# AshutoshNirkhe/KubernetesClusterCapacity

Measured on AMD Instinct MI355X. Metric: node×spec fit evals/sec at 1M nodes × 4K specs; % of HBM roofline, higher is better.
Workload: dtype int64; 1 GPU; C4: 1000000 nodes x 20000000 pods x 4096 specs; reduce + fit prepare + fit + finalize; nodes=1000000, pods=20000000, containers_rank0=39602467, nodes_rank0=1000000, pods_rank0=19801877, pods_per_node=poisson, mean 20, specs=4096, parallelism=node-sharded x1

## Files before the change

### include/kcc.h

```cpp
#ifndef KCC_H
#define KCC_H

#include <stdint.h>

#ifdef __cplusplus
extern "C" {
#endif

#define KCC_ABI_VERSION 2

enum {
  KCC_OK = 0,
  KCC_EINVAL = -1,
  KCC_ENOMEM = -2,
  KCC_EHIP = -3,
  KCC_ENODEV = -4,
  KCC_ERCCL = -5,
  KCC_EFAULT = -6
};

enum {
  KCC_SPEC_OK = 0,
  KCC_SPEC_DIVZERO = 1,
  KCC_SPEC_FAULT = 2
// ... 56 lines not shown
int kcc_fit_run_async(kcc_ctx* ctx, int64_t n_nodes, int64_t n_specs, int64_t* d_partial,
                      void* stream);

int kcc_fit_async(kcc_ctx* ctx, int64_t n_nodes, const uint64_t* d_alloc_cpu,
                  const int64_t* d_alloc_mem, const int64_t* d_alloc_pods,
                  const int64_t* d_pod_count, const uint64_t* d_used_cpu,
                  const int64_t* d_used_mem, int64_t n_specs, const uint64_t* d_spec_cpu,
                  const int64_t* d_spec_mem, int64_t* d_totals, int32_t* d_spec_err,
                  void* stream);

int kcc_capacity_partial_async(kcc_ctx* ctx, int64_t n_nodes, int64_t n_containers,
                               const int64_t* h_node_ptr, const int64_t* d_node_ptr,
                               const uint64_t* d_cpu_req, const int64_t* d_mem_req,
                               const uint64_t* d_alloc_cpu, const int64_t* d_alloc_mem,
                               const int64_t* d_alloc_pods, const int64_t* d_pod_count,
                               uint64_t* d_used_cpu, int64_t* d_used_mem, int64_t n_specs,
                               const uint64_t* d_spec_cpu, const int64_t* d_spec_mem,
                               int64_t* d_partial, int n_chunks, void* stream);
int kcc_capacity_async(kcc_ctx* ctx, int64_t n_nodes, int64_t n_containers,
                       const int64_t* h_node_ptr, const int64_t* d_node_ptr,
                       const uint64_t* d_cpu_req, const int64_t* d_mem_req,
                       const uint64_t* d_alloc_cpu, const int64_t* d_alloc_mem,
                       const int64_t* d_alloc_pods, const int64_t* d_pod_count,
                       uint64_t* d_used_cpu, int64_t* d_used_mem, int64_t n_specs,
                       const uint64_t* d_spec_cpu, const int64_t* d_spec_mem, int64_t* d_totals,
                       int32_t* d_spec_err, void* stream);

#define KCC_COMM_ID_BYTES 128
int kcc_set_node_shards(kcc_ctx* ctx, int n_shards);
int kcc_comm_unique_id(uint8_t* id );
int kcc_comm_init(kcc_ctx* ctx, const uint8_t* id, int n_ranks, int rank);
int kcc_allreduce_partial_async(kcc_ctx* ctx, int64_t n_specs, int64_t* d_partial, void* stream);

#define KCC_P2P_HANDLE_BYTES 64
#define KCC_P2P_MAX_SPECS (1 << 20)
int kcc_p2p_export(kcc_ctx* ctx, int n_ranks, int64_t max_specs,
                   uint8_t* handle );
int kcc_p2p_open(kcc_ctx* ctx, int rank, const uint8_t* handles );
int kcc_exchange_finalize_async(kcc_ctx* ctx, int64_t n_specs, const int64_t* d_partial,
                                int64_t* d_totals, int32_t* d_spec_err, void* stream);
int kcc_p2p_faults(kcc_ctx* ctx, int64_t* faults);

int kcc_profile_enable(kcc_ctx* ctx, int on);
int kcc_profile_read(kcc_ctx* ctx, double* reduce_ms, int64_t* reduce_launches, double* fit_ms,
                     int64_t* fit_launches);

int kcc_reduce_faults(kcc_ctx* ctx, int64_t* faults);
int kcc_clear_faults(kcc_ctx* ctx);

int kcc_set_fit_dense(kcc_ctx* ctx, int dense);
int kcc_set_clamp_in_fit(kcc_ctx* ctx, int mode);
int kcc_clamp_in_fit_used(kcc_ctx* ctx, int* used);
int kcc_fit_stream_rows(kcc_ctx* ctx, int64_t* streamed);

double kcc_last_slow_fraction(const kcc_ctx* ctx);

int kcc_fit_slow_pairs(kcc_ctx* ctx, int64_t* slow_pairs, int64_t* pairs);

enum {
  KCC_PARSE_OK = 1,
  KCC_PARSE_ERR = 0,
  KCC_PARSE_UNSUPPORTED = -1,
  KCC_PARSE_BADOFF = -2
};
int kcc_parse_cpu_millis(kcc_ctx* ctx, int64_t n, const char* bytes, int64_t n_bytes,
                         const int64_t* offsets, uint64_t* out, int8_t* status);
int kcc_parse_bytes(kcc_ctx* ctx, int64_t n, const char* bytes, int64_t n_bytes,
                    const int64_t* offsets, int64_t* out, int8_t* status);
int kcc_parse_quantity(kcc_ctx* ctx, int64_t n, const char* bytes, int64_t n_bytes,
                       const int64_t* offsets, int64_t* out, int8_t* status);
int kcc_parse_quantity_async(kcc_ctx* ctx, int64_t n, const char* d_bytes, int64_t n_bytes,
                             const int64_t* d_offsets, int64_t* d_out, int8_t* d_status,
                             void* stream);
int kcc_parse_cpu_millis_async(kcc_ctx* ctx, int64_t n, const char* d_bytes, int64_t n_bytes,
                               const int64_t* d_offsets, uint64_t* d_out, int8_t* d_status,
                               void* stream);
int kcc_parse_bytes_async(kcc_ctx* ctx, int64_t n, const char* d_bytes, int64_t n_bytes,
                          const int64_t* d_offsets, int64_t* d_out, int8_t* d_status,
                          void* stream);

int kcc_reduce_requests_keyed(kcc_ctx* ctx, int64_t n_keys, int64_t n_containers,
                              const int32_t* key, const uint64_t* cpu_req, const int64_t* mem_req,
                              const uint64_t* cpu_lim, const int64_t* mem_lim,
                              uint64_t* used_cpu, int64_t* used_mem, uint64_t* lim_cpu,
                              int64_t* lim_mem);
int kcc_reduce_requests_keyed_async(kcc_ctx* ctx, int64_t n_keys, int64_t n_containers,
                                    const int32_t* d_key, const uint64_t* d_cpu_req,
                                    const int64_t* d_mem_req, const uint64_t* d_cpu_lim,
                                    const int64_t* d_mem_lim, uint64_t* d_used_cpu,
                                    int64_t* d_used_mem, uint64_t* d_lim_cpu, int64_t* d_lim_mem,
                                    void* stream);
int kcc_count_by_key(kcc_ctx* ctx, int64_t n_keys, int64_t n, const int32_t* key, int64_t* count);
int kcc_count_by_key_async(kcc_ctx* ctx, int64_t n_keys, int64_t n, const int32_t* d_key,
                           int64_t* d_count, void* stream);

int kcc_fit_rows(kcc_ctx* ctx, int64_t n_nodes, const uint64_t* alloc_cpu,
                 const int64_t* alloc_mem, const int64_t* alloc_pods, const int64_t* pod_count,
                 const uint64_t* used_cpu, const int64_t* used_mem, uint64_t spec_cpu,
                 int64_t spec_mem, int64_t* q, int32_t* row_err);

int kcc_fit_grouped(kcc_ctx* ctx, int64_t n_nodes, const uint64_t* alloc_cpu,
                    const int64_t* alloc_mem, const int64_t* alloc_pods, const int64_t* pod_count,
                    const uint64_t* used_cpu, const int64_t* used_mem, const int32_t* group,
                    int64_t n_groups, int64_t n_specs, const uint64_t* spec_cpu,
                    const int64_t* spec_mem, int64_t* totals ,
                    int32_t* spec_err );
// ... 49 lines not shown
```

### kubernetesclustercapacity_amd/_lib.py

```python
from __future__ import annotations

import ctypes as C
import os
import re

_HERE = os.path.dirname(os.path.abspath(__file__))
LIB_PATH = os.path.join(_HERE, "libkcc.so")
HEADER_PATH = os.path.join(os.path.dirname(_HERE), "include", "kcc.h")

KCC_OK = 0
KCC_EINVAL = -1
KCC_ENOMEM = -2
KCC_EHIP = -3
KCC_ENODEV = -4
KCC_ERCCL = -5
KCC_EFAULT = -6
ERROR_NAMES = {
    KCC_EINVAL: "KCC_EINVAL", KCC_ENOMEM: "KCC_ENOMEM", KCC_EHIP: "KCC_EHIP",
    KCC_ENODEV: "KCC_ENODEV", KCC_ERCCL: "KCC_ERCCL", KCC_EFAULT: "KCC_EFAULT",
}
KCC_SPEC_OK = 0
KCC_SPEC_DIVZERO = 1
KCC_SPEC_FAULT = 2
KCC_EXT_MAX = 4

_i64, _i32, _int, _vp, _dbl = C.c_int64, C.c_int32, C.c_int, C.c_void_p, C.c_double

SIGNATURES = {
    "kcc_abi_version": (_int, []),
    "kcc_set_allreduce_verify": (_int, [_vp, _int]),
    "kcc_build_info": (C.c_char_p, []),
    "kcc_create": (_int, [C.POINTER(_vp), _int, _int]),
    "kcc_destroy": (None, [_vp]),
    "kcc_last_error": (C.c_char_p, [_vp]),
    "kcc_create_error": (C.c_char_p, []),
    "kcc_reserve": (_int, [_vp, _i64, _i64, _i64]),
    "kcc_reduce_requests": (_int, [_vp, _i64, _i64] + [_vp] * 9),
    "kcc_reduce_requests_async": (_int, [_vp, _i64, _i64] + [_vp] * 10),
    "kcc_fit": (_int, [_vp, _i64] + [_vp] * 6 + [_i64] + [_vp] * 4),
    "kcc_capacity": (_int, [_vp, _i64, _i64] + [_vp] * 7 + [_i64] + [_vp] * 4),
    "kcc_fit_partial_async": (_int, [_vp, _i64] + [_vp] * 6 + [_i64] + [_vp] * 4),
    "kcc_fit_prepare_async": (_int, [_vp, _i64] + [_vp] * 6 + [_i64] + [_vp] * 4),
    "kcc_fit_run_async": (_int, [_vp, _i64, _i64, _vp, _vp]),
    "kcc_fit_finalize_async": (_int, [_vp, _i64, _vp, _vp, _vp, _vp]),
    "kcc_fit_async": (_int, [_vp, _i64] + [_vp] * 6 + [_i64] + [_vp] * 5),
    "kcc_capacity_partial_async": (_int, [_vp, _i64, _i64] + [_vp] * 10 + [_i64] + [_vp] * 3
                                   + [_int, _vp]),
    "kcc_capacity_async": (_int, [_vp, _i64, _i64] + [_vp] * 10 + [_i64] + [_vp] * 5),
    "kcc_set_node_shards": (_int, [_vp, _int]),
    "kcc_set_fit_dense": (_int, [_vp, _int]),
    "kcc_set_clamp_in_fit": (_int, [_vp, _int]),
    "kcc_clamp_in_fit_used": (_int, [_vp, C.POINTER(C.c_int)]),
    "kcc_fit_stream_rows": (_int, [_vp, C.POINTER(_i64)]),
    "kcc_reduce_faults": (_int, [_vp, C.POINTER(_i64)]),
    "kcc_clear_faults": (_int, [_vp]),
    "kcc_comm_unique_id": (_int, [_vp]),
    "kcc_comm_init": (_int, [_vp, _vp, _int, _int]),
    "kcc_allreduce_partial_async": (_int, [_vp, _i64, _vp, _vp]),
    "kcc_p2p_export": (_int, [_vp, _int, _i64, _vp]),
    "kcc_p2p_open": (_int, [_vp, _int, _vp]),
    "kcc_exchange_finalize_async": (_int, [_vp, _i64, _vp, _vp, _vp, _vp]),
    "kcc_p2p_faults": (_int, [_vp, C.POINTER(_i64)]),
    "kcc_profile_enable": (_int, [_vp, _int]),
    "kcc_profile_read": (_int, [_vp] + [C.POINTER(_dbl), C.POINTER(_i64)] * 2),
    "kcc_last_slow_fraction": (_dbl, [_vp]),
    "kcc_fit_slow_pairs": (_int, [_vp, C.POINTER(_i64), C.POINTER(_i64)]),
    "kcc_parse_cpu_millis": (_int, [_vp, _i64, _vp, _i64, _vp, _vp, _vp]),
    "kcc_parse_bytes": (_int, [_vp, _i64, _vp, _i64, _vp, _vp, _vp]),
    "kcc_parse_quantity": (_int, [_vp, _i64, _vp, _i64, _vp, _vp, _vp]),
    "kcc_parse_quantity_async": (_int, [_vp, _i64, _vp, _i64, _vp, _vp, _vp, _vp]),
    "kcc_parse_cpu_millis_async": (_int, [_vp, _i64, _vp, _i64, _vp, _vp, _vp, _vp]),
    "kcc_parse_bytes_async": (_int, [_vp, _i64, _vp, _i64, _vp, _vp, _vp, _vp]),
    "kcc_reduce_requests_keyed": (_int, [_vp, _i64, _i64] + [_vp] * 9),
    "kcc_reduce_requests_keyed_async": (_int, [_vp, _i64, _i64] + [_vp] * 10),
    "kcc_count_by_key": (_int, [_vp, _i64, _i64, _vp, _vp]),
    "kcc_count_by_key_async": (_int, [_vp, _i64, _i64, _vp, _vp, _vp]),
    "kcc_fit_rows": (_int, [_vp, _i64] + [_vp] * 6 + [C.c_uint64, _i64, _vp, _vp]),
    "kcc_fit_grouped": (_int, [_vp, _i64] + [_vp] * 7 + [_i64, _i64] + [_vp] * 4),
    "kcc_fit_grouped_async": (_int, [_vp, _i64] + [_vp] * 7 + [_i64, _i64] + [_vp] * 5),
    "kcc_fit_ext": (_int, [_vp, _i64] + [_vp] * 6 + [_i64] + [_vp] * 3 + [_i64, _i64] + [_vp] * 5),
    "kcc_fit_ext_async": (_int, [_vp, _i64] + [_vp] * 6 + [_i64] + [_vp] * 3 + [_i64, _i64]
                          + [_vp] * 6),
    "kcc_pod_requests": (_int, [_vp, _i64, _i64, _i64] + [_vp] * 11),
    "kcc_pod_requests_async": (_int, [_vp, _i64, _i64, _i64] + [_vp] * 12),
    "kcc_reduce_requests_pods": (_int, [_vp, _i64, _i64, _i64, _i64] + [_vp] * 12),
}

KCC_PARSE_OK = 1
KCC_PARSE_ERR = 0
KCC_PARSE_UNSUPPORTED = -1
KCC_PARSE_BADOFF = -2


def header_symbols(path: str = HEADER_PATH) -> list[str]:
    text = open(path).read()
    text = re.sub(r"/\*.*?\*/", "", text, flags=re.S)
    return sorted(set(re.findall(r"\b(kcc_[a-z0-9_]+)\s*\(", text)))


def header_arities(path: str = HEADER_PATH) -> dict[str, int]:
    text = re.sub(r"/\*.*?\*/", "", open(path).read(), flags=re.S)
    out = {}
    for m in re.finditer(r"\b(kcc_[a-z0-9_]+)\s*\(([^;{]*?)\)\s*;", text, flags=re.S):
        params = m.group(2).strip()
        out[m.group(1)] = 0 if params in ("", "void") else params.count(",") + 1
    return out


def load(path: str = LIB_PATH) -> C.CDLL:
    if not os.path.exists(path):
        raise ImportError(
            f"libkcc.so not found at {path}: build it with "
            "`make -C kubernetesclustercapacity_amd/csrc` (or __graft_entry__.build()). "
            "There is no CPU fallback.")
    lib = C.CDLL(path)
    for name, (res, args) in SIGNATURES.items():
        fn = getattr(lib, name)
        fn.restype = res
        fn.argtypes = args
    return lib


_LIBS: dict[str, C.CDLL] = {}


def lib(path: str | None = None) -> C.CDLL:
    p = os.path.abspath(path or LIB_PATH)
    if p not in _LIBS:
        _LIBS[p] = load(p)
    return _LIBS[p]
```

### kubernetesclustercapacity_amd/csrc/kcc_abi.cpp

```cpp
#include "kcc.h"

#include <hip/hip_runtime.h>
#include <rccl/rccl.h>

#include <cstdio>
#include <cstdlib>
#include <cstring>
#include <string>
#include <vector>

#include "kcc_internal.h"

namespace {

struct DevBuf {
  void* p = nullptr;
  size_t bytes = 0;
};

hipError_t ensure(DevBuf& b, size_t bytes) {
  if (bytes == 0) bytes = 16;
  if (b.bytes >= bytes) return hipSuccess;
  if (b.p) (void)hipFree(b.p);
  b.p = nullptr;
  b.bytes = 0;
  hipError_t e = hipMalloc(&b.p, bytes);
  if (e == hipSuccess) b.bytes = bytes;
  return e;
}

hipError_t ensure_uncached(DevBuf& b, size_t bytes) {
  if (bytes == 0) bytes = 16;
  if (b.bytes >= bytes) return hipSuccess;
  if (b.p) (void)hipFree(b.p);
  b.p = nullptr;
  b.bytes = 0;
  hipError_t e = hipExtMallocWithFlags(&b.p, bytes, hipDeviceMallocUncached);
  if (e == hipSuccess) b.bytes = bytes;
  return e;
}

template <class T>
T* as(DevBuf& b) {
  return static_cast<T*>(b.p);
}

struct ProfPair {
  hipEvent_t a, b;
  int kind;
};

struct Dev {
  int device = 0;
  hipStream_t stream = nullptr;
  hipStream_t side = nullptr;
  hipEvent_t ev_fork = nullptr;
  hipEvent_t ev_red[kcc::FIT_MAX_CHUNKS] = {};
  bool prof_on = false;
  std::vector<ProfPair> prof_pending;
  std::vector<hipEvent_t> prof_free;
  double prof_ms[2] = {0.0, 0.0};
  int64_t prof_n[2] = {0, 0};
  DevBuf fast_a, fast_b, slow, slow_list, srec, sperm, counters;
  DevBuf red_tail;
  DevBuf faults;
  DevBuf rank_arrive;
  DevBuf fit_q;
  bool fitq_dirty = true;
  DevBuf c_rank, c_bcnt, c_cs, c_ms, c_mrc, c_crm, c_dperm;
  DevBuf c_C, c_H2, c_H3, c_Crow, c_rec, c_dir;
  bool clamp_dirty = true;
  int64_t last_pairs = 0;
  int64_t c_stride = 0;
  int64_t h_stride = 0;
  int64_t d_stride = 0;
  bool fit_dense = false;
  int clamp_in_fit = -1;
  bool last_nc = false;
  DevBuf fast_cl;
  int stream_chunks = 0;
  int64_t prep_nodes = -1, prep_specs = -1;
  DevBuf ptr, cpu, mem, cpul, meml, used_cpu, used_mem, lim_cpu, lim_mem;
  DevBuf alloc_cpu, alloc_mem, alloc_pods, pod_count, spec_cpu, spec_mem, partial, totals, err;
  DevBuf p_bytes, p_off, p_out, p_st;
  DevBuf k_key;
  DevBuf g_group;
  DevBuf g_count, g_cursor, g_total, g_rec, g_rg, g_acc;
  DevBuf x_alloc, x_used, x_spec;
  DevBuf x_rec;
  DevBuf kb_counts, kb_tot, kb_sr, kb_sv;
  DevBuf kb_part, kb_arrive;
  DevBuf kb_esc_n, kb_esc_row, kb_esc_cpu, kb_esc_mem;
  DevBuf q_ptr, q_iptr, q_icpu, q_imem, q_rst, q_ocpu, q_omem, q_pcpu, q_pmem;
  DevBuf p2p_mbox, p2p_arrive;
  DevBuf clamp_arrive;
  DevBuf np_sync;
  unsigned char* p2p_peer[kcc::P2P_MAX_RANKS] = {};
  int p2p_W = 0, p2p_rank = -1;
  int64_t p2p_smax = 0;
  bool p2p_ready = false;
};

}

struct kcc_ctx {
  std::vector<Dev> devs;
  std::vector<ncclComm_t> comms;
  ncclComm_t proc_comm = nullptr;
  int proc_ranks = 0, proc_rank = 0;
  int node_shards = 0;
  std::string err;
  double slow_frac = -1.0;
  unsigned long long* host_cnt = nullptr;
  size_t host_cnt_n = 0;
  int64_t host_stream_rows = -1;
  bool allreduce_verified = false;
  bool allreduce_verify_every = false;
};

namespace {

thread_local std::string g_create_error;

int fail(kcc_ctx* ctx, int code, const std::string& msg) {
  if (ctx) ctx->err = msg;
  return code;
}

#define KCC_HIP(ctx, expr)                                                              \
  do {                                                                                  \
// ... 71 lines not shown
    KCC_HIP(ctx, hipSetDevice(dv.device));
    KCC_HIP(ctx, hipMemcpy(f, dv.faults.p, sizeof(f), hipMemcpyDeviceToHost));
    red += f[kcc::FAULT_RED];
    p2p += f[kcc::FAULT_P2P];
  }
  if (red == 0 && p2p == 0) return KCC_OK;
  return fail(ctx, KCC_EFAULT,
              "device fault: " + std::to_string(red) + " reduce-side wait(s) (look-back, node prep, keyed gather) and " +
                  std::to_string(p2p) +
                  " exchange flag wait(s) gave up; results are not valid (every spec is marked "
                  "KCC_SPEC_FAULT) until kcc_clear_faults");
}

int reduce_async_dev(kcc_ctx* ctx, Dev& dv, int64_t n_nodes, int64_t n_cont, const int64_t* ptr,
                     const uint64_t* cpu, const int64_t* mem, const uint64_t* cpul,
                     const int64_t* meml, uint64_t* used_cpu, int64_t* used_mem,
                     uint64_t* lim_cpu, int64_t* lim_mem, hipStream_t s) {
  if (n_nodes < 0 || n_cont < 0) return fail(ctx, KCC_EINVAL, "negative size");
  if (n_nodes == 0) return n_cont == 0 ? KCC_OK : fail(ctx, KCC_EINVAL, "containers without nodes");
  if (n_nodes >= kcc::RED_MAX_NODES)
    return fail(ctx, KCC_EINVAL, "too many nodes per device (max 2^28 - 1)");
  if (!ptr || !used_cpu || !used_mem) return fail(ctx, KCC_EINVAL, "NULL node_ptr/output");
  if (n_cont > 0 && (!cpu || !mem)) return fail(ctx, KCC_EINVAL, "NULL cpu_req/mem_req");
  const bool lim = cpul != nullptr || meml != nullptr;
  if (lim && (!cpul || !meml || !lim_cpu || !lim_mem))
    return fail(ctx, KCC_EINVAL, "limits need cpu_lim, mem_lim, lim_cpu and lim_mem");
  if (!aligned16(cpu) || !aligned16(mem) || (lim && (!aligned16(cpul) || !aligned16(meml))))
    return fail(ctx, KCC_EINVAL, "container arrays must be 16-byte aligned");
  int rc = reduce_ws(ctx, dv, s);
  if (rc) return rc;
  KCC_HIP(ctx, kcc::launch_reduce(n_nodes, 0, n_cont, ptr, cpu, mem, lim ? cpul : nullptr,
                                  lim ? meml : nullptr, used_cpu, used_mem, lim ? lim_cpu : nullptr,
                                  lim ? lim_mem : nullptr, as<uint64_t>(dv.red_tail),
                                  as<unsigned long long>(dv.faults), s));
  return KCC_OK;
}

kcc::SpecPrep spec_prep_of(Dev& dv) {
  kcc::SpecPrep sp;
  sp.rec = as<kcc::SpecRec>(dv.srec);
  sp.perm = as<int32_t>(dv.sperm);
  return sp;
}

int reserve_dev(kcc_ctx* ctx, Dev& dv, int64_t n_nodes, int64_t n_cont, int64_t n_specs) {
  KCC_HIP(ctx, hipSetDevice(dv.device));
  const size_t N = (size_t)(n_nodes > 0 ? n_nodes : 1);
  const size_t S = (size_t)(n_specs > 0 ? n_specs : 1);
  (void)n_cont;
  {
    int rc = reduce_ws(ctx, dv, dv.stream);
    if (rc) return rc;
  }
  KCC_HIP(ctx, ensure(dv.fast_a, sizeof(kcc::FitGroupA) * (size_t)kcc::fit_groups((int64_t)N)));
  KCC_HIP(ctx, ensure(dv.fast_b, sizeof(kcc::FitGroup) * (size_t)kcc::fit_groups((int64_t)N)));
  KCC_HIP(ctx, ensure(dv.fast_cl, sizeof(int32_t) * kcc::FIT_GROUP * (size_t)kcc::fit_groups((int64_t)N)));
  KCC_HIP(ctx, ensure(dv.slow, sizeof(kcc::SlowNode) * N));
  KCC_HIP(ctx, ensure(dv.slow_list, sizeof(int64_t) * N));
  KCC_HIP(ctx, ensure(dv.srec, sizeof(kcc::SpecRec) * S));
  KCC_HIP(ctx, ensure(dv.sperm, 4 * S));
  KCC_HIP(ctx, ensure(dv.counters, sizeof(unsigned long long) * kcc::CNT_N));
  if (!dv.np_sync.p) {
    const size_t bytes = 4 * (kcc::NP_FLAGS + (size_t)kcc::reduce_tail_records());
    KCC_HIP(ctx, ensure(dv.np_sync, bytes));
    KCC_HIP(ctx, hipMemsetAsync(dv.np_sync.p, 0, bytes, dv.stream));
    KCC_HIP(ctx, hipStreamSynchronize(dv.stream));
  }
  if (!dv.clamp_arrive.p) {
    KCC_HIP(ctx, ensure(dv.clamp_arrive, 64));
    KCC_HIP(ctx, hipMemsetAsync(dv.clamp_arrive.p, 0, 64, dv.stream));
    KCC_HIP(ctx, hipStreamSynchronize(dv.stream));
  }
  const size_t q_before = dv.fit_q.bytes;
  KCC_HIP(ctx, ensure(dv.fit_q, 4 * (size_t)kcc::fit_queue_words((int64_t)S)));
  if (dv.fit_q.bytes != q_before) dv.fitq_dirty = true;
  const size_t S64 = (S + 63) / 64 * 64;
  KCC_HIP(ctx, ensure(dv.c_bcnt, 8 * (S64 / 64)));
  KCC_HIP(ctx, ensure(dv.c_cs, 8 * S));
  KCC_HIP(ctx, ensure(dv.c_ms, 8 * S));
  KCC_HIP(ctx, ensure(dv.c_mrc, 4 * S64));
  KCC_HIP(ctx, ensure(dv.c_crm, 4 * S64));
  KCC_HIP(ctx, ensure(dv.c_dperm, 4 * S));
  const int64_t cs_ = kcc::clamp_c_cells((int64_t)S), hs = kcc::clamp_h_cells((int64_t)S);
  const size_t before[3] = {dv.c_C.bytes, dv.c_H2.bytes, dv.c_H3.bytes};
  KCC_HIP(ctx, ensure(dv.c_rank, 4 * (size_t)kcc::rank_words((int64_t)S)));
  if (dv.rank_arrive.bytes < 4 * (S64 / 64)) {
    KCC_HIP(ctx, ensure(dv.rank_arrive, 4 * (S64 / 64)));
    KCC_HIP(ctx, hipMemsetAsync(dv.rank_arrive.p, 0, dv.rank_arrive.bytes, dv.stream));
    KCC_HIP(ctx, hipStreamSynchronize(dv.stream));
  }
  KCC_HIP(ctx, ensure(dv.c_C, 8 * (size_t)kcc::C_COPIES * (size_t)cs_));
  KCC_HIP(ctx, ensure(dv.c_H2, 8 * (size_t)kcc::H2_COPIES * (size_t)hs));
  KCC_HIP(ctx, ensure(dv.c_H3, 8 * (size_t)kcc::H2_COPIES * (size_t)hs));
  KCC_HIP(ctx, ensure(dv.c_Crow, 8 * (size_t)cs_));
  if (kcc::clamp_binned((int64_t)S)) {
    const size_t passes = (size_t)((N + kcc::CLAMP_PASS_ROWS_MIN - 1) / kcc::CLAMP_PASS_ROWS_MIN);
    const size_t recs = (size_t)((N + kcc::CLAMP_PASS_ROWS_MAX - 1) / kcc::CLAMP_PASS_ROWS_MAX) *
                        2 * kcc::CLAMP_PASS_ROWS_MAX;
    KCC_HIP(ctx, ensure(dv.c_rec, 8 * recs));
    KCC_HIP(ctx, ensure(dv.c_dir, 4 * (size_t)kcc::clamp_d_stride((int64_t)S) * passes));
  }
  if (dv.c_C.bytes != before[0] || dv.c_H2.bytes != before[1] || dv.c_H3.bytes != before[2] ||
      dv.c_stride != cs_ || dv.h_stride != hs)
    dv.clamp_dirty = true;
  dv.c_stride = cs_;
  dv.h_stride = hs;
  dv.d_stride = kcc::clamp_d_stride((int64_t)S);
  return KCC_OK;
}

int clamp_clean(kcc_ctx* ctx, Dev& dv, hipStream_t s) {
  if (dv.fitq_dirty) {
    KCC_HIP(ctx, hipMemsetAsync(dv.fit_q.p, 0, dv.fit_q.bytes, s));
    dv.fitq_dirty = false;
  }
  if (!dv.clamp_dirty) return KCC_OK;
  KCC_HIP(ctx, hipMemsetAsync(dv.c_C.p, 0, dv.c_C.bytes, s));
  KCC_HIP(ctx, hipMemsetAsync(dv.c_H2.p, 0, dv.c_H2.bytes, s));
  KCC_HIP(ctx, hipMemsetAsync(dv.c_H3.p, 0, dv.c_H3.bytes, s));
  dv.clamp_dirty = false;
  return KCC_OK;
}

kcc::ClampWork clamp_of(Dev& dv) {
  kcc::ClampWork cw;
  cw.rank = as<uint32_t>(dv.c_rank);
  cw.bcnt = as<uint32_t>(dv.c_bcnt);
  cw.cs = as<uint64_t>(dv.c_cs);
  cw.ms = as<int64_t>(dv.c_ms);
  cw.mr_c = as<uint32_t>(dv.c_mrc);
  cw.cr_m = as<uint32_t>(dv.c_crm);
  cw.dperm = as<int32_t>(dv.c_dperm);
  cw.C = as<int64_t>(dv.c_C);
  cw.H2 = as<int64_t>(dv.c_H2);
  cw.H3 = as<int64_t>(dv.c_H3);
  cw.Crow = as<int64_t>(dv.c_Crow);
  cw.rec = as<uint64_t>(dv.c_rec);
  cw.dir = as<uint32_t>(dv.c_dir);
  cw.c_stride = dv.c_stride;
  cw.h_stride = dv.h_stride;
  cw.d_stride = dv.d_stride;
  cw.n_pass = 0;
  return cw;
}

int check_spec_ws(kcc_ctx* ctx, Dev& dv, int64_t S) {
  const size_t S64 = (size_t)(S + 63) / 64 * 64;
  const bool ok = dv.c_rank.bytes >= 4 * (size_t)kcc::rank_words(S) &&
                  dv.c_bcnt.bytes >= 8 * (S64 / 64) && dv.c_mrc.bytes >= 4 * S64 &&
                  dv.rank_arrive.bytes >= 4 * (S64 / 64) &&
                  dv.c_crm.bytes >= 4 * S64 && dv.c_cs.bytes >= 8 * (size_t)S &&
                  dv.c_ms.bytes >= 8 * (size_t)S && dv.c_dperm.bytes >= 4 * (size_t)S &&
                  dv.srec.bytes >= sizeof(kcc::SpecRec) * (size_t)S &&
                  dv.sperm.bytes >= 4 * (size_t)S &&
                  dv.counters.bytes >= sizeof(unsigned long long) * kcc::CNT_N &&
                  dv.c_C.bytes >= 8 * (size_t)kcc::C_COPIES * (size_t)dv.c_stride &&
                  dv.c_stride >= kcc::clamp_c_cells(S);
  return ok ? KCC_OK : fail(ctx, KCC_EINVAL, "internal: spec workspace smaller than the call");
}

kcc::PlaceArgs place_args(Dev& dv, int64_t n_specs, const uint64_t* spec_cpu,
                          const int64_t* spec_mem, int64_t* partial) {
  return kcc::PlaceArgs{n_specs, spec_cpu, spec_mem, spec_prep_of(dv), clamp_of(dv), partial,
                        as<unsigned long long>(dv.counters), 0,
                        as<const unsigned long long>(dv.faults), 0};
}

int fit_prepare_dev(kcc_ctx* ctx, Dev& dv, int64_t n_nodes, const uint64_t* alloc_cpu,
                    const int64_t* alloc_mem, const int64_t* alloc_pods,
                    const int64_t* pod_count, const uint64_t* used_cpu,
                    const int64_t* used_mem, int64_t n_specs, const uint64_t* spec_cpu,
                    const int64_t* spec_mem, int64_t* partial, hipStream_t s) {
  ctx->host_stream_rows = -1;
  if (n_nodes < 0 || n_specs < 0) return fail(ctx, KCC_EINVAL, "negative size");
  if (n_specs >= kcc::MAX_SPECS) return fail(ctx, KCC_EINVAL, "too many specs (max 2^26 - 1)");
  if (n_specs > 0 && (!spec_cpu || !spec_mem || !partial))
    return fail(ctx, KCC_EINVAL, "NULL spec array / partial");
  if (n_nodes > 0 && (!alloc_cpu || !alloc_mem || !alloc_pods || !pod_count || !used_cpu || !used_mem))
    return fail(ctx, KCC_EINVAL, "NULL node array");
  int rc = reserve_dev(ctx, dv, n_nodes, 0, n_specs);
  if (rc) return rc;
  dv.last_pairs = n_nodes * n_specs;
  dv.prep_nodes = n_nodes;
  dv.prep_specs = n_specs;
  if (n_specs == 0) return KCC_OK;
  if ((rc = check_spec_ws(ctx, dv, n_specs))) return rc;
  rc = clamp_clean(ctx, dv, s);
  if (rc) return rc;
  dv.clamp_dirty = true;
  KCC_HIP(ctx, kcc::launch_spec_rank(kcc::rank_args(n_specs, spec_cpu, spec_mem, clamp_of(dv),
                                                    as<unsigned long long>(dv.counters),
                                                    as<uint32_t>(dv.rank_arrive)),
                                     s));
  const kcc::PlaceArgs pa = place_args(dv, n_specs, spec_cpu, spec_mem, partial);
  KCC_HIP(ctx, kcc::launch_node_prep(n_nodes, alloc_cpu, alloc_mem, alloc_pods, pod_count,
                                       used_cpu, used_mem, as<kcc::FitGroupA>(dv.fast_a),
                                       as<kcc::FitGroup>(dv.fast_b), as<kcc::SlowNode>(dv.slow),
                                       as<int64_t>(dv.slow_list), n_specs, clamp_of(dv),
                                       as<unsigned long long>(dv.counters), 0, 0,
                                       n_nodes, s, dv.fit_dense, &pa));
  if (n_nodes == 0) {
    dv.clamp_dirty = false;
    return KCC_OK;
  }
  dv.stream_chunks = 1;
  KCC_HIP(ctx, kcc::launch_clamp_apply(n_specs, n_nodes, clamp_of(dv),
                                       as<unsigned long long>(dv.counters), partial, s));
  dv.clamp_dirty = false;
  return KCC_OK;
}

int fit_run_dev(kcc_ctx* ctx, Dev& dv, int64_t n_nodes, int64_t n_specs, int64_t* partial,
                hipStream_t s) {
  if (n_nodes != dv.prep_nodes || n_specs != dv.prep_specs)
    return fail(ctx, KCC_EINVAL, "fit_run sizes differ from the preceding fit_prepare");
  if (n_nodes == 0 || n_specs == 0) return KCC_OK;
  if (!partial) return fail(ctx, KCC_EINVAL, "NULL partial");
  KCC_HIP(ctx, kcc::launch_fit(n_nodes, as<kcc::FitGroupA>(dv.fast_a), as<kcc::FitGroup>(dv.fast_b),
                               as<kcc::SlowNode>(dv.slow),
                               as<int64_t>(dv.slow_list), n_specs, spec_prep_of(dv), partial,
                               as<unsigned long long>(dv.counters), as<uint32_t>(dv.fit_q), 0,
                               n_nodes, s, as<const unsigned long long>(dv.faults)));
  return KCC_OK;
}

int fit_partial_dev(kcc_ctx* ctx, Dev& dv, int64_t n_nodes, const uint64_t* alloc_cpu,
                    const int64_t* alloc_mem, const int64_t* alloc_pods,
                    const int64_t* pod_count, const uint64_t* used_cpu,
                    const int64_t* used_mem, int64_t n_specs, const uint64_t* spec_cpu,
                    const int64_t* spec_mem, int64_t* partial, hipStream_t s) {
  int rc = fit_prepare_dev(ctx, dv, n_nodes, alloc_cpu, alloc_mem, alloc_pods, pod_count,
                           used_cpu, used_mem, n_specs, spec_cpu, spec_mem, partial, s);
  if (rc) return rc;
  return fit_run_dev(ctx, dv, n_nodes, n_specs, partial, s);
}

int fit_finalize_dev(kcc_ctx* ctx, Dev& dv, int64_t n_specs, const int64_t* partial,
                     int64_t* totals, int32_t* spec_err, hipStream_t s) {
  if (n_specs < 0) return fail(ctx, KCC_EINVAL, "negative size");
  if (n_specs == 0) return KCC_OK;
  if (!partial || !totals || !spec_err) return fail(ctx, KCC_EINVAL, "NULL partial/totals/err");
  if (dv.sperm.bytes < sizeof(int32_t) * (size_t)n_specs)
    return fail(ctx, KCC_EINVAL, "finalize without a matching fit_partial");
  KCC_HIP(ctx, kcc::launch_fit_finalize(n_specs, partial, as<int32_t>(dv.sperm), totals,
                                        spec_err, as<const unsigned long long>(dv.faults), s));
  return KCC_OK;
}



hipError_t prof_event(Dev& dv, hipEvent_t* ev) {
  if (!dv.prof_free.empty()) {
    *ev = dv.prof_free.back();
    dv.prof_free.pop_back();
    return hipSuccess;
  }
  return hipEventCreateWithFlags(ev, hipEventDisableSystemFence);
}

constexpr int64_t CHUNK_ALIGN = kcc::CLAMP_PASS_ROWS_MAX;
int plan_chunks(int64_t n_nodes, int want, int64_t min_nodes, std::vector<int64_t>& lo,
                std::vector<int64_t>& hi) {
  int k = want;
  if (k > kcc::FIT_MAX_CHUNKS) k = kcc::FIT_MAX_CHUNKS;
  while (k > 1 && n_nodes / k < min_nodes) --k;
  if (k < 1) k = 1;
  lo.assign(k, 0);
  hi.assign(k, 0);
  for (int c = 0; c < k; ++c) {
    lo[c] = c == 0 ? 0 : hi[c - 1];
    hi[c] = c == k - 1 ? n_nodes : (n_nodes * (c + 1) / k) / CHUNK_ALIGN * CHUNK_ALIGN;
    if (hi[c] < lo[c]) hi[c] = lo[c];
  }
  return k;
}
// ... 8 lines not shown
                         int64_t* used_mem, int64_t n_specs, const uint64_t* spec_cpu,
                         const int64_t* spec_mem, int64_t* partial, int n_chunks, hipStream_t s,
                         int64_t* totals = nullptr, int32_t* spec_err = nullptr) {
  ctx->host_stream_rows = -1;
  if (n_nodes < 0 || n_cont < 0 || n_specs < 0) return fail(ctx, KCC_EINVAL, "negative size");
  if (n_nodes >= kcc::RED_MAX_NODES)
    return fail(ctx, KCC_EINVAL, "too many nodes per device (max 2^28 - 1)");
  if (n_specs >= kcc::MAX_SPECS) return fail(ctx, KCC_EINVAL, "too many specs (max 2^26 - 1)");
  if (n_nodes == 0 && n_cont != 0) return fail(ctx, KCC_EINVAL, "containers without nodes");
  if (n_nodes > 0 && (!ptr || !used_cpu || !used_mem || !alloc_cpu || !alloc_mem || !alloc_pods ||
                      !pod_count))
    return fail(ctx, KCC_EINVAL, "NULL node array");
  if (n_cont > 0 && (!cpu || !mem)) return fail(ctx, KCC_EINVAL, "NULL cpu_req/mem_req");
  if (!aligned16(cpu) || !aligned16(mem))
    return fail(ctx, KCC_EINVAL, "container arrays must be 16-byte aligned");
  if (n_specs > 0 && (!spec_cpu || !spec_mem || !partial))
    return fail(ctx, KCC_EINVAL, "NULL spec array / partial");
  std::vector<int64_t> lo, hi;
  const int k = plan_chunks(n_nodes, h_ptr ? (n_chunks > 0 ? n_chunks : KCC_DEFAULT_CHUNKS) : 1,
                            KCC_MIN_CHUNK_NODES, lo, hi);
  std::vector<int64_t> c0(k), c1(k);
  for (int c = 0; c < k; ++c) {
    if (k == 1) {
      c0[c] = 0;
      c1[c] = n_cont;
    } else {
      c0[c] = h_ptr[lo[c]];
      c1[c] = h_ptr[hi[c]];
      if (c0[c] < 0 || c1[c] < c0[c] || c1[c] > n_cont)
        return fail(ctx, KCC_EINVAL, "h_node_ptr is not a CSR of n_containers");
    }
  }
  int rc = reserve_dev(ctx, dv, n_nodes, n_cont, n_specs);
  if (rc) return rc;
  if (n_specs > 0 && (rc = check_spec_ws(ctx, dv, n_specs))) return rc;
  for (int c = 0; c < k; ++c)
    if (!dv.ev_red[c]) KCC_HIP(ctx, hipEventCreateWithFlags(&dv.ev_red[c], hipEventDisableTiming));
  dv.last_pairs = n_nodes * n_specs;
  dv.stream_chunks = k;
  dv.prep_nodes = -1;
  dv.prep_specs = -1;
  hipStream_t rs = k > 1 ? dv.side : s;
  if (k > 1) {
    KCC_HIP(ctx, hipEventRecord(dv.ev_fork, s));
    KCC_HIP(ctx, hipStreamWaitEvent(dv.side, dv.ev_fork, 0));
  }
  const bool fuse_place = n_specs > 0;
  const bool fuse_rank = k == 1 && fuse_place && n_nodes > 0 && n_cont > 0;
  const bool nc = fuse_rank && n_specs <= kcc::CLAMP_LDS_SPECS && !dv.fit_dense &&
                  (dv.clamp_in_fit == 1 ||
                   (dv.clamp_in_fit < 0 && kcc::clamp_in_fit_auto(n_nodes, n_specs)));
  int32_t* const fast_cl = nc ? as<int32_t>(dv.fast_cl) : nullptr;
  dv.last_nc = nc;
  kcc::RankArgs ra = kcc::rank_args(n_specs, spec_cpu, spec_mem, clamp_of(dv),
                                    as<unsigned long long>(dv.counters),
                                    as<uint32_t>(dv.rank_arrive), nc);
  kcc::PlaceArgs pa = place_args(dv, n_specs, spec_cpu, spec_mem, partial);
  pa.no_ranks = nc ? 1 : 0;
  kcc::NpArgs np{};
  if (nc) {
    ra.done_flag = as<uint32_t>(dv.np_sync);
    np.n_place = (int32_t)((n_specs + 255) / 256);
    np.n_rows = (int32_t)((n_nodes + kcc::NP_ROWS_PER_WG - 1) / kcc::NP_ROWS_PER_WG);
    np.sync = as<uint32_t>(dv.np_sync);
    np.pa = pa;
    np.n = n_nodes;
    np.alloc_cpu = alloc_cpu;
    np.alloc_mem = alloc_mem;
    np.alloc_pods = alloc_pods;
    np.pod_count = pod_count;
    np.used_cpu = used_cpu;
    np.used_mem = used_mem;
    np.fast_a = as<kcc::FitGroupA>(dv.fast_a);
    np.fast_b = as<kcc::FitGroup>(dv.fast_b);
    np.slow = as<kcc::SlowNode>(dv.slow);
    np.slow_list = as<int64_t>(dv.slow_list);
    np.fast_cl = fast_cl;
    np.counters = as<unsigned long long>(dv.counters);
    np.bcnt = clamp_of(dv).bcnt;
    np.S = n_specs;
    np.faults = as<unsigned long long>(dv.faults);
  }
  if (n_specs > 0) {
    rc = clamp_clean(ctx, dv, s);
    if (rc) return rc;
    dv.clamp_dirty = true;
    if (!fuse_rank) KCC_HIP(ctx, kcc::launch_spec_rank(ra, s));
  }
  for (int c = 0; c < k; ++c) {
    const int64_t n = hi[c] - lo[c];
    ProfPair pp{};
    if (dv.prof_on) {
      KCC_HIP(ctx, prof_event(dv, &pp.a));
      KCC_HIP(ctx, prof_event(dv, &pp.b));
    }
    KCC_HIP(ctx, kcc::launch_reduce(n, c0[c], c1[c] - c0[c], ptr + lo[c], cpu, mem, nullptr, nullptr,
                                    used_cpu + lo[c], used_mem + lo[c], nullptr, nullptr,
                                    as<uint64_t>(dv.red_tail),
                                    as<unsigned long long>(dv.faults), rs,
                                    fuse_rank ? &ra : nullptr, nc ? &np : nullptr,
                                    dv.prof_on ? pp.a : nullptr, dv.prof_on ? pp.b : nullptr));
    if (dv.prof_on) {
      pp.kind = 0;
      dv.prof_pending.push_back(pp);
    }
    if (k > 1) KCC_HIP(ctx, hipEventRecord(dv.ev_red[c], dv.side));
  }
  const bool fuse_fin = totals && n_nodes > 0;
  const kcc::FinArgs fin{as<int32_t>(dv.sperm), totals, spec_err, as<uint32_t>(dv.clamp_arrive),
                         as<const unsigned long long>(dv.faults)};
  for (int c = 0; c < k; ++c) {
    if (k > 1) KCC_HIP(ctx, hipStreamWaitEvent(s, dv.ev_red[c], 0));
    const int64_t n = hi[c] - lo[c];
    const bool place_here = fuse_place && c == 0;
    if (n_specs == 0 || (n == 0 && !place_here)) continue;
    if (!nc)
    KCC_HIP(ctx, kcc::launch_node_prep(n, alloc_cpu + lo[c], alloc_mem + lo[c], alloc_pods + lo[c],
                                       pod_count + lo[c], used_cpu + lo[c], used_mem + lo[c],
                                       as<kcc::FitGroupA>(dv.fast_a) + lo[c] / kcc::FIT_GROUP,
                                       as<kcc::FitGroup>(dv.fast_b) + lo[c] / kcc::FIT_GROUP,
                                       as<kcc::SlowNode>(dv.slow) + lo[c],
                                       as<int64_t>(dv.slow_list) + lo[c], n_specs, clamp_of(dv),
                                       as<unsigned long long>(dv.counters),
                                       c, lo[c], n_nodes, s, dv.fit_dense,
                                       place_here ? &pa : nullptr));
    if (n == 0) continue;
    ProfPair pp{};
    if (dv.prof_on) {
      KCC_HIP(ctx, prof_event(dv, &pp.a));
      KCC_HIP(ctx, prof_event(dv, &pp.b));
    }
    KCC_HIP(ctx, kcc::launch_fit(n, as<kcc::FitGroupA>(dv.fast_a) + lo[c] / kcc::FIT_GROUP,
                                 as<kcc::FitGroup>(dv.fast_b) + lo[c] / kcc::FIT_GROUP,
                                 as<kcc::SlowNode>(dv.slow) + lo[c],
                                 as<int64_t>(dv.slow_list) + lo[c], n_specs, spec_prep_of(dv),
                                 partial, as<unsigned long long>(dv.counters),
                                 as<uint32_t>(dv.fit_q), c, n_nodes, s,
                                 as<const unsigned long long>(dv.faults), fast_cl,
                                 dv.prof_on ? pp.a : nullptr, dv.prof_on ? pp.b : nullptr));
    if (dv.prof_on) {
      pp.kind = 1;
      dv.prof_pending.push_back(pp);
    }
  }
  if (n_specs > 0 && nc) {
    dv.clamp_dirty = false;
    if (totals) return fit_finalize_dev(ctx, dv, n_specs, partial, totals, spec_err, s);
    return KCC_OK;
  }
  if (n_specs > 0) {
    if (n_nodes > 0)
      KCC_HIP(ctx, kcc::launch_clamp_apply(n_specs, n_nodes, clamp_of(dv),
                                           as<unsigned long long>(dv.counters), partial, s,
                                           fuse_fin ? &fin : nullptr));
    dv.clamp_dirty = false;
    if (totals && !fuse_fin)
      return fit_finalize_dev(ctx, dv, n_specs, partial, totals, spec_err, s);
  }
  return KCC_OK;
}

int run_host(kcc_ctx* ctx, bool with_reduce, int64_t n_nodes, int64_t n_cont,
             const int64_t* node_ptr, const uint64_t* cpu_req, const int64_t* mem_req,
             const uint64_t* alloc_cpu, const int64_t* alloc_mem, const int64_t* alloc_pods,
             const int64_t* pod_count, const uint64_t* used_cpu_in, const int64_t* used_mem_in,
             int64_t n_specs, const uint64_t* spec_cpu, const int64_t* spec_mem,
             int64_t* totals, int32_t* spec_err) {
  if (n_nodes < 0 || n_specs < 0) return fail(ctx, KCC_EINVAL, "negative size");
  if (n_specs > 0 && (!spec_cpu || !spec_mem || !totals || !spec_err))
    return fail(ctx, KCC_EINVAL, "NULL spec array / output");
  if (n_nodes > 0 && (!alloc_cpu || !alloc_mem || !alloc_pods || !pod_count))
    return fail(ctx, KCC_EINVAL, "NULL node array");
  if (with_reduce) {
    int rc = check_csr(ctx, n_nodes, n_cont, node_ptr);
    if (rc) return rc;
    if (n_cont > 0 && (!cpu_req || !mem_req)) return fail(ctx, KCC_EINVAL, "NULL container array");
  } else if (n_nodes > 0 && (!used_cpu_in || !used_mem_in)) {
    return fail(ctx, KCC_EINVAL, "NULL used array");
  }
  if (n_specs == 0) return KCC_OK;
  const int nd = (int)ctx->devs.size();
  const int ns = ctx->node_shards > nd ? ctx->node_shards : nd;
  const int slots = (ns + nd - 1) / nd;
  std::vector<int64_t> lo, hi;
  shard_nodes(n_nodes, ns, lo, hi);
  std::vector<std::vector<int64_t>> rebased(ns);
  if (ctx->host_cnt_n < (size_t)ns * kcc::CNT_N) {
    if (ctx->host_cnt) (void)hipHostFree(ctx->host_cnt);
    ctx->host_cnt = nullptr;
    ctx->host_cnt_n = 0;
    KCC_HIP(ctx, hipHostMalloc(reinterpret_cast<void**>(&ctx->host_cnt),
                               sizeof(unsigned long long) * (size_t)ns * kcc::CNT_N, hipHostMallocDefault));
// ... 66 lines not shown
    }
    KCC_NCCL(ctx, ncclGroupStart());
    for (int d = 0; d < nd; ++d) {
      Dev& dv = ctx->devs[d];
      KCC_NCCL(ctx, ncclAllReduce(dv.partial.p, dv.partial.p, words, ncclInt64,
                                  ncclSum, ctx->comms[d], dv.stream));
    }
    KCC_NCCL(ctx, ncclGroupEnd());
#ifdef KCC_DIAG_INLIB_COMM
    if (std::getenv("KCC_DRILL_CORRUPT_ALLREDUCE")) {
      Dev& dv = ctx->devs[nd - 1];
      KCC_HIP(ctx, hipSetDevice(dv.device));
      KCC_HIP(ctx, hipMemsetAsync(dv.partial.p, 0x5a, 8, dv.stream));
    }
#endif
    if (verify) {
      for (int d = 0; d < nd; ++d) {
        Dev& dv = ctx->devs[d];
        KCC_HIP(ctx, hipSetDevice(dv.device));
        KCC_HIP(ctx, hipMemcpyAsync(got.data(), dv.partial.p, 8 * words, hipMemcpyDeviceToHost,
                                    dv.stream));
        KCC_HIP(ctx, hipStreamSynchronize(dv.stream));
        for (size_t i = 0; i < words; ++i)
          if (got[i] != expect[i])
            return fail(ctx, KCC_ERCCL,
                        "in-library all-reduce verification failed on device " +
                            std::to_string(dv.device) + ": word " + std::to_string(i) + " is " +
                            std::to_string(got[i]) + ", the host sum of the devices' partials " +
                            std::to_string(expect[i]) + "; results not returned");
      }
      ctx->allreduce_verified = true;
    }
  }
  Dev& d0 = ctx->devs[0];
  KCC_HIP(ctx, hipSetDevice(d0.device));
  KCC_HIP(ctx, ensure(d0.totals, 8 * (size_t)n_specs));
  KCC_HIP(ctx, ensure(d0.err, 4 * (size_t)n_specs));
  int rc = fit_finalize_dev(ctx, d0, n_specs, as<int64_t>(d0.partial), as<int64_t>(d0.totals),
                            as<int32_t>(d0.err), d0.stream);
  if (rc) return rc;
  KCC_HIP(ctx, hipMemcpyAsync(totals, d0.totals.p, 8 * (size_t)n_specs, hipMemcpyDeviceToHost,
                              d0.stream));
  KCC_HIP(ctx, hipMemcpyAsync(spec_err, d0.err.p, 4 * (size_t)n_specs, hipMemcpyDeviceToHost,
                              d0.stream));
  unsigned long long slow_pairs = 0;
  for (int d = 0; d < nd; ++d) {
    Dev& dv = ctx->devs[d];
    KCC_HIP(ctx, hipSetDevice(dv.device));
    KCC_HIP(ctx, hipStreamSynchronize(dv.stream));
  }
  int64_t streamed = 0;
  for (int sh = 0; sh < ns; ++sh) {
    slow_pairs += ctx->host_cnt[(size_t)sh * kcc::CNT_N + kcc::CNT_SLOW_PAIRS];
    streamed += (int64_t)ctx->host_cnt[(size_t)sh * kcc::CNT_N + kcc::CNT_STREAM];
  }
  ctx->host_stream_rows = streamed;
  const double pairs = (double)n_nodes * (double)n_specs;
  ctx->slow_frac = pairs > 0 ? (double)slow_pairs / pairs : 0.0;
  return check_faults(ctx);
}

}

extern "C" {

int kcc_abi_version(void) { return KCC_ABI_VERSION; }

int kcc_set_allreduce_verify(kcc_ctx* ctx, int every_call) {
  if (!ctx) return KCC_EINVAL;
  ctx->allreduce_verify_every = every_call != 0;
  return KCC_OK;
}

#ifdef KCC_VARIANT_BUILD
const char* kcc_build_info(void) { return "variant: " KCC_VARIANT_FLAGS; }
#else
const char* kcc_build_info(void) { return "release"; }
#endif

const char* kcc_create_error(void) { return g_create_error.c_str(); }

int kcc_create(kcc_ctx** out, int first_device, int n_gpus) {
  g_create_error.clear();
  if (!out) { g_create_error = "out is NULL"; return KCC_EINVAL; }
  *out = nullptr;
  if (n_gpus <= 0 || first_device < 0) {
    g_create_error = "n_gpus must be >= 1 and first_device >= 0 (there is no CPU backend)";
    return KCC_EINVAL;
  }
  int count = 0;
  hipError_t e = hipGetDeviceCount(&count);
  if (e != hipSuccess || count <= 0) {
    g_create_error = std::string("no HIP device: ") + hipGetErrorString(e);
    return KCC_ENODEV;
  }
  if (first_device + n_gpus > count) {
    g_create_error = "requested devices [" + std::to_string(first_device) + ", " +
                     std::to_string(first_device + n_gpus) + ") but only " +
                     std::to_string(count) + " visible";
    return KCC_ENODEV;
  }
  kcc_ctx* ctx = new kcc_ctx();
  ctx->devs.resize(n_gpus);
  std::vector<int> ids(n_gpus);
  for (int d = 0; d < n_gpus; ++d) {
    Dev& dv = ctx->devs[d];
    dv.device = first_device + d;
// ... 7 lines not shown
                       "): libkcc is built for MI355X only";
      kcc_destroy(ctx);
      return KCC_ENODEV;
    }
    if ((e = hipSetDevice(dv.device)) != hipSuccess ||
        (e = hipStreamCreateWithFlags(&dv.stream, hipStreamNonBlocking)) != hipSuccess ||
        (e = hipStreamCreateWithFlags(&dv.side, hipStreamNonBlocking)) != hipSuccess ||
        (e = hipEventCreateWithFlags(&dv.ev_fork, hipEventDisableTiming)) != hipSuccess) {
      g_create_error = std::string("stream creation failed: ") + hipGetErrorString(e);
      kcc_destroy(ctx);
      return KCC_EHIP;
    }
  }
#ifdef KCC_DIAG_INLIB_COMM
  const bool inlib_comm = true;
#else
  const bool inlib_comm = n_gpus > 1;
#endif
  if (inlib_comm) {
    ctx->comms.resize(n_gpus);
    ncclResult_t r = ncclCommInitAll(ctx->comms.data(), n_gpus, ids.data());
    if (r != ncclSuccess) {
      ctx->comms.clear();
      g_create_error = std::string("ncclCommInitAll: ") + ncclGetErrorString(r);
      kcc_destroy(ctx);
      return KCC_ERCCL;
    }
  }
  *out = ctx;
  return KCC_OK;
}

void kcc_destroy(kcc_ctx* ctx) {
  if (!ctx) return;
  for (auto& c : ctx->comms) ncclCommDestroy(c);
  if (ctx->proc_comm) {
    (void)hipSetDevice(ctx->devs[0].device);
    (void)hipDeviceSynchronize();
    ncclCommDestroy(ctx->proc_comm);
  }
  for (Dev& dv : ctx->devs) {
    (void)hipSetDevice(dv.device);
    if (dv.stream) (void)hipStreamSynchronize(dv.stream);
    if (dv.p2p_W > 0) {
      (void)hipDeviceSynchronize();
      for (int p = 0; p < dv.p2p_W; ++p)
        if (p != dv.p2p_rank && dv.p2p_peer[p]) (void)hipIpcCloseMemHandle(dv.p2p_peer[p]);
      DevBuf* pb[] = {&dv.p2p_mbox, &dv.p2p_arrive};
      for (DevBuf* b : pb)
        if (b->p) (void)hipFree(b->p);
    }
    if (dv.clamp_arrive.p) (void)hipFree(dv.clamp_arrive.p);
    if (dv.np_sync.p) (void)hipFree(dv.np_sync.p);
    DevBuf* bufs[] = {&dv.c_rank, &dv.c_bcnt, &dv.c_cs, &dv.c_ms,
                      &dv.c_mrc, &dv.c_crm, &dv.c_dperm, &dv.c_C, &dv.c_H2, &dv.c_H3,
                      &dv.c_Crow, &dv.c_rec, &dv.c_dir,
                      &dv.red_tail,  &dv.faults, &dv.rank_arrive, &dv.fast_cl, &dv.slow_list, &dv.fast_a, &dv.fast_b, &dv.slow, &dv.srec,
                      &dv.sperm,     &dv.fit_q,
                      &dv.counters,  &dv.ptr,       &dv.cpu,       &dv.mem,       &dv.cpul,
                      &dv.meml,      &dv.used_cpu,  &dv.used_mem,  &dv.lim_cpu,   &dv.lim_mem,
                      &dv.alloc_cpu, &dv.alloc_mem, &dv.alloc_pods, &dv.pod_count, &dv.spec_cpu,
                      &dv.spec_mem,  &dv.partial,   &dv.totals,    &dv.err,
                      &dv.p_bytes,   &dv.p_off,     &dv.p_out,     &dv.p_st,      &dv.k_key,
                      &dv.kb_counts, &dv.kb_tot,    &dv.kb_sr,     &dv.kb_sv,     &dv.q_ptr,
                      &dv.kb_part,   &dv.kb_arrive,
                      &dv.kb_esc_n,  &dv.kb_esc_row, &dv.kb_esc_cpu, &dv.kb_esc_mem,
                      &dv.q_iptr,    &dv.q_icpu,    &dv.q_imem,    &dv.q_rst,     &dv.q_ocpu,
                      &dv.q_omem,    &dv.q_pcpu,    &dv.q_pmem,
                      &dv.g_group,   &dv.g_count,   &dv.g_cursor,  &dv.g_total,   &dv.g_rec,
                      &dv.g_rg,      &dv.g_acc,     &dv.x_alloc,   &dv.x_used,    &dv.x_spec,
                      &dv.x_rec};
    for (DevBuf* b : bufs)
      if (b->p) (void)hipFree(b->p);
    if (dv.stream) (void)hipStreamDestroy(dv.stream);
    if (dv.side) {
      (void)hipStreamSynchronize(dv.side);
      (void)hipStreamDestroy(dv.side);
    }
    if (dv.ev_fork) (void)hipEventDestroy(dv.ev_fork);
    for (hipEvent_t ev : dv.ev_red)
      if (ev) (void)hipEventDestroy(ev);
    for (const ProfPair& pp : dv.prof_pending) {
      (void)hipEventDestroy(pp.a);
      (void)hipEventDestroy(pp.b);
    }
    for (hipEvent_t ev : dv.prof_free) (void)hipEventDestroy(ev);
  }
  if (ctx->host_cnt) (void)hipHostFree(ctx->host_cnt);
  delete ctx;
}

const char* kcc_last_error(const kcc_ctx* ctx) { return ctx ? ctx->err.c_str() : "NULL context"; }

int kcc_reserve(kcc_ctx* ctx, int64_t max_nodes, int64_t max_containers, int64_t max_specs) {
  if (!ctx) return KCC_EINVAL;
  if (max_nodes < 0 || max_containers < 0 || max_specs < 0)
    return fail(ctx, KCC_EINVAL, "negative size");
  return reserve_dev(ctx, ctx->devs[0], max_nodes, max_containers, max_specs);
}

int kcc_reduce_requests_async(kcc_ctx* ctx, int64_t n_nodes, int64_t n_containers,
                              const int64_t* d_node_ptr, const uint64_t* d_cpu_req,
                              const int64_t* d_mem_req, const uint64_t* d_cpu_lim,
                              const int64_t* d_mem_lim, uint64_t* d_used_cpu,
                              int64_t* d_used_mem, uint64_t* d_lim_cpu, int64_t* d_lim_mem,
                              void* stream) {
  if (!ctx) return KCC_EINVAL;
// ... 206 lines not shown
  *reduce_launches = dv.prof_n[0];
  *fit_ms = dv.prof_ms[1];
  *fit_launches = dv.prof_n[1];
  return KCC_OK;
}

double kcc_last_slow_fraction(const kcc_ctx* ctx) { return ctx ? ctx->slow_frac : -1.0; }

int kcc_fit_slow_pairs(kcc_ctx* ctx, int64_t* slow_pairs, int64_t* pairs) {
  if (!ctx || !slow_pairs || !pairs) return ctx ? fail(ctx, KCC_EINVAL, "NULL output") : KCC_EINVAL;
  Dev& dv = ctx->devs[0];
  KCC_HIP(ctx, hipSetDevice(dv.device));
  KCC_HIP(ctx, hipDeviceSynchronize());
  unsigned long long c = 0;
  if (dv.counters.p) KCC_HIP(ctx, hipMemcpy(&c, dv.counters.p, sizeof(c), hipMemcpyDeviceToHost));
  *slow_pairs = (int64_t)c;
  *pairs = dv.last_pairs;
  return KCC_OK;
}

int kcc_set_fit_dense(kcc_ctx* ctx, int dense) {
  if (!ctx) return KCC_EINVAL;
  for (Dev& dv : ctx->devs) dv.fit_dense = dense != 0;
  return KCC_OK;
}

int kcc_clamp_in_fit_used(kcc_ctx* ctx, int* used) {
  if (!ctx || !used) return KCC_EINVAL;
  *used = 0;
  for (const Dev& dv : ctx->devs) *used |= dv.last_nc ? 1 : 0;
  return KCC_OK;
}

int kcc_set_clamp_in_fit(kcc_ctx* ctx, int mode) {
  if (!ctx) return KCC_EINVAL;
  if (mode < -1 || mode > 1) return fail(ctx, KCC_EINVAL, "mode: -1 (by size), 0 or 1");
  for (Dev& dv : ctx->devs) dv.clamp_in_fit = mode;
  return KCC_OK;
}

int kcc_fit_stream_rows(kcc_ctx* ctx, int64_t* streamed) {
  if (!ctx || !streamed) return ctx ? fail(ctx, KCC_EINVAL, "NULL output") : KCC_EINVAL;
  if (ctx->host_stream_rows >= 0) {
    *streamed = ctx->host_stream_rows;
    return KCC_OK;
  }
  Dev& dv = ctx->devs[0];
  KCC_HIP(ctx, hipSetDevice(dv.device));
  KCC_HIP(ctx, hipDeviceSynchronize());
  unsigned long long c[kcc::CNT_N] = {};
  if (dv.counters.p)
    KCC_HIP(ctx, hipMemcpy(c, dv.counters.p, sizeof(c), hipMemcpyDeviceToHost));
  int64_t t = 0;
  for (int k = 0; k < dv.stream_chunks && k < kcc::FIT_MAX_CHUNKS; ++k) t += (int64_t)c[kcc::CNT_STREAM + k];
  *streamed = t;
  return KCC_OK;
}

int kcc_reduce_faults(kcc_ctx* ctx, int64_t* faults) {
  if (!ctx || !faults) return ctx ? fail(ctx, KCC_EINVAL, "NULL output") : KCC_EINVAL;
  int64_t t = 0;
  for (Dev& dv : ctx->devs) {
    if (!dv.faults.p) continue;
    KCC_HIP(ctx, hipSetDevice(dv.device));
    KCC_HIP(ctx, hipDeviceSynchronize());
    unsigned long long f = 0;
    KCC_HIP(ctx, hipMemcpy(&f, as<unsigned long long>(dv.faults) + kcc::FAULT_RED, sizeof(f),
                           hipMemcpyDeviceToHost));
    t += (int64_t)f;
  }
  *faults = t;
  return KCC_OK;
}

int kcc_clear_faults(kcc_ctx* ctx) {
  if (!ctx) return KCC_EINVAL;
  for (Dev& dv : ctx->devs) {
    KCC_HIP(ctx, hipSetDevice(dv.device));
    KCC_HIP(ctx, hipDeviceSynchronize());
    if (dv.faults.p) KCC_HIP(ctx, hipMemset(dv.faults.p, 0, dv.faults.bytes));
    if (dv.red_tail.p) KCC_HIP(ctx, hipMemset(dv.red_tail.p, 0, dv.red_tail.bytes));
    for (DevBuf* b : {&dv.kb_arrive, &dv.rank_arrive, &dv.fit_q, &dv.clamp_arrive})
      if (b->p) KCC_HIP(ctx, hipMemset(b->p, 0, b->bytes));
    KCC_HIP(ctx, hipDeviceSynchronize());
  }
  return KCC_OK;
}

int kcc_set_node_shards(kcc_ctx* ctx, int n_shards) {
  if (!ctx) return KCC_EINVAL;
  if (n_shards < 0) return fail(ctx, KCC_EINVAL, "n_shards must be >= 0");
  ctx->node_shards = n_shards;
  return KCC_OK;
}


int kcc_comm_unique_id(uint8_t* id) {
  if (!id) return KCC_EINVAL;
  static_assert(sizeof(ncclUniqueId) == KCC_COMM_ID_BYTES, "ncclUniqueId size");
  ncclUniqueId u;
  if (ncclGetUniqueId(&u) != ncclSuccess) return KCC_ERCCL;
  std::memcpy(id, &u, sizeof(u));
  return KCC_OK;
}

int kcc_comm_init(kcc_ctx* ctx, const uint8_t* id, int n_ranks, int rank) {
  if (!ctx) return KCC_EINVAL;
  if (!id || n_ranks < 1 || rank < 0 || rank >= n_ranks)
// ... 842 lines not shown
```

### kubernetesclustercapacity_amd/csrc/kcc_internal.h

```cpp
#pragma once
#include <hip/hip_runtime.h>
#include <stdint.h>

#if !defined(KCC_VARIANT_BUILD) &&                                                       \
    (defined(KCC_DIAG_RED_NOSTORE) || defined(KCC_DIAG_RED_LOADONLY) ||                  \
     defined(KCC_TIMELINE) || defined(KCC_DIAG_RED_GIVEUP) || defined(KCC_DIAG_P2P_GIVEUP) || \
     defined(KCC_DIAG_INLIB_COMM) || defined(KCC_DIAG_GA_NOATOM) ||                     \
     defined(KCC_DIAG_NP_NOSC1))
#error "a diagnostic KCC_* knob in a release build: use `make variant` (KCC_VARIANT_BUILD)"
#endif

namespace kcc {

struct RankArgs;
struct NpArgs;

constexpr int RED_PREFETCH = 1;
constexpr int RED_IPL = 8;
constexpr int RED_TILE = 64 * RED_IPL;
constexpr int RED_WAVES_PER_BLOCK = 4;
constexpr int64_t RED_MAX_NODES = (int64_t)1 << 28;
constexpr int RED_TAIL_WORDS = 8;
constexpr int RED_TAIL_TAG = 7;
constexpr uint64_t RED_TAG_READY = 1;
// ... 22 lines not shown
};
hipError_t launch_reduce(int64_t n_nodes, int64_t c0, int64_t n_containers, const int64_t* node_ptr,
                         const uint64_t* cpu_req, const int64_t* mem_req,
                         const uint64_t* cpu_lim, const int64_t* mem_lim,
                         uint64_t* used_cpu, int64_t* used_mem, uint64_t* lim_cpu, int64_t* lim_mem,
                         uint64_t* tail, unsigned long long* faults, hipStream_t s,
                         const RankArgs* rank = nullptr, const NpArgs* np = nullptr,
                         hipEvent_t ev_start = nullptr, hipEvent_t ev_stop = nullptr);

constexpr int FIT_GROUP = 8;
struct __attribute__((aligned(32))) FitGroupA {
  uint64_t fm[FIT_GROUP];
  uint32_t fc[FIT_GROUP];
  uint32_t P[FIT_GROUP];
};
static_assert(sizeof(FitGroupA) == 128, "FitGroupA must be 128 B");
constexpr double FIT_BIAS = 4503599627370496.0;
struct __attribute__((aligned(32))) FitGroup {
  double fc[FIT_GROUP];
  double fm[FIT_GROUP];
  double Pb[FIT_GROUP];
};
static_assert(sizeof(FitGroup) == 192, "FitGroup must be 192 B");
__host__ __device__ inline int64_t fit_groups(int64_t n_nodes) { return (n_nodes + FIT_GROUP - 1) / FIT_GROUP; }

struct __attribute__((aligned(32))) SlowNode {
  uint64_t fc;
  int64_t fm;
  int64_t P;
  int64_t cl;
};
static_assert(sizeof(SlowNode) == 32, "SlowNode must be 32 B");

enum SpecClass : int32_t { SPEC_A = 0, SPEC_B = 1, SPEC_EXACT = 2 };
struct __attribute__((aligned(16))) SpecRec {
  uint64_t c;
  int64_t m;
  double rc;
  double rm;
  float rcf;
  int32_t cls;
  int64_t pad;
};
static_assert(sizeof(SpecRec) == 48, "SpecRec must be 48 B");

struct SpecPrep {
  SpecRec* rec;
  int32_t* perm;
};

struct ClampWork {
  uint32_t* rank;
  uint32_t* bcnt;
  uint64_t* cs;
  int64_t* ms;
  uint32_t* mr_c;
  uint32_t* cr_m;
  int32_t* dperm;
  int64_t* C;
  int64_t* H2;
  int64_t* H3;
  int64_t* Crow;
  uint64_t* rec;
  uint32_t* dir;
  int64_t c_stride;
  int64_t h_stride;
  int64_t d_stride;
  int64_t n_pass;
  int64_t pass_recs;
};
constexpr int64_t MAX_SPECS = (int64_t)1 << 26;
__host__ __device__ inline int64_t clamp_c_cells(int64_t S) { return (S / 64 + 3) * (S / 64 + 3); }
inline int64_t clamp_h_cells(int64_t S) { return (S / 64 + 1) * 65 * 64; }
constexpr int C_COPIES = 2;
constexpr int H2_COPIES = 2;
constexpr int CLAMP_PASS_ROWS_MIN = 1024;
constexpr int CLAMP_PASS_ROWS_MAX = 4096;
inline int64_t clamp_pass_rows(int64_t n_nodes) {
  return n_nodes >= (int64_t)200 * CLAMP_PASS_ROWS_MAX ? CLAMP_PASS_ROWS_MAX : CLAMP_PASS_ROWS_MIN;
}
constexpr int64_t CLAMP_BIN_T_MAX = 256;
__host__ __device__ inline bool clamp_binned(int64_t S) { return (S + 63) / 64 <= CLAMP_BIN_T_MAX; }
inline int64_t clamp_d_stride(int64_t S) { return 2 * ((S + 63) / 64) + 1; }
inline int64_t clamp_passes(int64_t n_nodes) {
  const int64_t pr = clamp_pass_rows(n_nodes);
  return (n_nodes + pr - 1) / pr;
}
constexpr int64_t CLAMP_LDS_SPECS = 4096;

constexpr int64_t RANK_L = 1024;
constexpr int64_t RANK_FULL_MAX = 4096;
__host__ __device__ inline int64_t rank_slices(int64_t S) { return (S + RANK_L - 1) / RANK_L; }
__host__ __device__ inline int64_t rank_words(int64_t S) { return 2 * S + 2 * S * rank_slices(S); }
struct RankArgs {
  int64_t S;
  const uint64_t* c_in;
  const int64_t* m_in;
  uint32_t* part;
  uint32_t* arrive;
  uint32_t* bcnt;
  uint64_t* cs;
  int64_t* ms;
  uint32_t* mr_c;
  uint32_t* cr_m;
  int64_t* C;
  int64_t c_stride, c_cells;
  unsigned long long* counters;
  int32_t n_blocks;
  int32_t zero_only;
  uint32_t* done_flag;
};
RankArgs rank_args(int64_t n_specs, const uint64_t* spec_cpu, const int64_t* spec_mem,
                   const ClampWork& cw, unsigned long long* counters, uint32_t* arrive,
                   bool zero_only = false);
hipError_t launch_spec_rank(const RankArgs& ra, hipStream_t s);

struct PlaceArgs {
  int64_t S;
  const uint64_t* c_in;
  const int64_t* m_in;
  SpecPrep sp;
  ClampWork cw;
  int64_t* partial;
  unsigned long long* counters;
  int32_t n_blocks;
  const unsigned long long* faults;
  int32_t no_ranks;
};


struct NpArgs {
  int32_t n_place, n_rows;
  uint32_t* sync;
  const int64_t* ptr;
  int64_t c0;
  int32_t range, red_waves;
  PlaceArgs pa;
  int64_t n;
  const uint64_t* alloc_cpu;
  const int64_t* alloc_mem;
  const int64_t* alloc_pods;
  const int64_t* pod_count;
  const uint64_t* used_cpu;
  const int64_t* used_mem;
  FitGroupA* fast_a;
  FitGroup* fast_b;
  SlowNode* slow;
  int64_t* slow_list;
  int32_t* fast_cl;
  unsigned long long* counters;
  const uint32_t* bcnt;
  int64_t S;
  unsigned long long* faults;
};
constexpr int NP_ROWS_PER_WG = 1024;
constexpr int NP_EPOCH = 0, NP_DONE = 16, NP_ARRIVE = 32, NP_FLAGS = 64;

constexpr int FIT_MAX_CHUNKS = 16;
enum {
  CNT_SLOW_PAIRS = 0,
  CNT_SPECS_A = 1,
  CNT_SPECS_B = 2,
  CNT_CLAMP_ALL = 3,
  CNT_SLOW_ROWS = 4,
  CNT_STREAM = 4 + FIT_MAX_CHUNKS,
  CNT_N = 4 + 2 * FIT_MAX_CHUNKS
};
struct FinArgs {
  const int32_t* perm;
  int64_t* totals;
  int32_t* spec_err;
  uint32_t* arrive;
  const unsigned long long* faults;
};
hipError_t launch_clamp_apply(int64_t n_specs, int64_t n_nodes, ClampWork cw,
                              const unsigned long long* counters, int64_t* partial, hipStream_t s,
                              const FinArgs* fin = nullptr);
int64_t clamp_apply_blocks(int64_t n_specs);
constexpr int64_t RED_RANKS_LAST_MIN = (int64_t)16 << 20;

hipError_t launch_node_prep(int64_t n_nodes, const uint64_t* alloc_cpu,
                            const int64_t* alloc_mem, const int64_t* alloc_pods,
                            const int64_t* pod_count, const uint64_t* used_cpu,
                            const int64_t* used_mem, FitGroupA* fast_a, FitGroup* fast_b,
                            SlowNode* slow, int64_t* slow_list, int64_t n_specs, ClampWork cw,
                            unsigned long long* counters, int chunk, int64_t row0,
                            int64_t call_nodes, hipStream_t s, bool dense = false,
                            const PlaceArgs* place = nullptr);
constexpr int64_t CLAMP_IN_FIT_PAIRS = 1100000000LL;
inline bool clamp_in_fit_auto(int64_t n_nodes, int64_t n_specs) {
  return n_specs <= CLAMP_LDS_SPECS && n_nodes * n_specs <= CLAMP_IN_FIT_PAIRS;
}

hipError_t launch_fit(int64_t n_nodes, const FitGroupA* fast_a, const FitGroup* fast_b,
                      const SlowNode* slow,
                      const int64_t* slow_list, int64_t n_specs, SpecPrep sp, int64_t* partial,
                      unsigned long long* counters, uint32_t* queue, int chunk,
                      int64_t grid_nodes, hipStream_t s, const unsigned long long* faults,
                      const int32_t* fast_cl = nullptr, hipEvent_t ev_start = nullptr,
                      hipEvent_t ev_stop = nullptr);
constexpr int64_t FIT_QSUBS_MAX = 32;
inline int64_t fit_queue_words(int64_t S) { return (S + 255) / 256 * FIT_QSUBS_MAX * 16; }

hipError_t launch_fit_finalize(int64_t n_specs, const int64_t* partial,
                               const int32_t* perm, int64_t* totals, int32_t* spec_err,
                               const unsigned long long* faults, hipStream_t s);
hipError_t launch_partial_add(int64_t n, int64_t* dst, const int64_t* src, hipStream_t s);

constexpr int P2P_MAX_RANKS = 8;
__host__ __device__ inline size_t p2p_flag_words(int W) { return (size_t)2 * W * 8; }
inline size_t p2p_mbox_bytes(int W, int64_t smax) {
  return 8 * (p2p_flag_words(W) + (size_t)2 * W * 2 * (size_t)smax);
}
struct P2PArgs {
  int64_t S, smax;
  int32_t W, rank;
  uint64_t* epoch;
  const int64_t* partial;
  unsigned char* mbox[P2P_MAX_RANKS];
  const int32_t* perm;
  int64_t* totals;
  int32_t* spec_err;
  uint32_t* arrive;
  unsigned long long* faults;
};
hipError_t launch_exchange_finalize(const P2PArgs& a, hipStream_t s);

enum ParseMode : int { PARSE_MODE_CPU_MILLIS = 0, PARSE_MODE_BYTES = 1, PARSE_MODE_QUANTITY = 2 };
enum ParseStatus : int8_t {
  PARSE_OK = 1,
  PARSE_ERR = 0,
  PARSE_UNSUPPORTED = -1,
  PARSE_BADOFF = -2
};
int64_t parse_grid(int64_t n);
hipError_t launch_parse(int mode, int64_t n, const uint8_t* bytes, int64_t n_bytes,
                        const int64_t* offsets, int64_t* out, int8_t* status, hipStream_t s);

constexpr int KB_SHIFT = 12;
constexpr int KB_ROWS = 1 << KB_SHIFT;
constexpr int KB_TILE = 65536;
constexpr int64_t KB_NB_MAX = 4096;
struct KeyedWork {
  uint32_t* counts;
  uint32_t* tot;
  uint64_t* sr;
  uint64_t* sv;
  uint32_t* esc_n;
  int32_t* esc_row;
  uint64_t* esc_cpu;
  uint64_t* esc_mem;
  uint64_t* part_acc;
  uint32_t* arrive;
  unsigned long long* faults;
};
// ... 111 lines not shown
```

### kubernetesclustercapacity_amd/csrc/kcc_kernels.hip

```cpp

#include <hip/hip_ext.h>
#include <hip/hip_runtime.h>
#include <stdint.h>

#include <atomic>

#include "kcc_internal.h"

namespace kcc {

namespace {

#ifdef KCC_TIMELINE
__device__ uint64_t kcc_tl[8192][8];
#define KCC_TL(slot, k) \
  do { if (threadIdx.x == 0) kcc_tl[(slot)][(k)] = __builtin_amdgcn_s_memrealtime(); } while (0)
#define KCC_TLV(slot, k, v) \
  do { if (threadIdx.x == 0) kcc_tl[(slot)][(k)] = (v); } while (0)
#else
#define KCC_TL(slot, k) do { } while (0)
#define KCC_TLV(slot, k, v) do { } while (0)
#endif

typedef __attribute__((address_space(3))) unsigned long long lds_ull;
// ... 735 lines not shown
    if (a[mid] <= v) lo = mid + 1;
    else hi = mid;
  }
  return (uint32_t)lo;
}

__device__ __forceinline__ uint32_t count_lt64(const uint32_t* __restrict__ a, uint32_t v, uint32_t lim) {
  const uint4* q = reinterpret_cast<const uint4*>(a);
  uint32_t n = 0;
#pragma unroll 4
  for (uint32_t u = 0; u < 16; ++u) {
    const uint4 w = q[u];
    n += (w.x < v && 4 * u + 0 < lim ? 1u : 0u) + (w.y < v && 4 * u + 1 < lim ? 1u : 0u) +
         (w.z < v && 4 * u + 2 < lim ? 1u : 0u) + (w.w < v && 4 * u + 3 < lim ? 1u : 0u);
  }
  return n;
}

#define KCC_NODE_PREP_BLOCK 1024
static_assert(CLAMP_PASS_ROWS_MIN == KCC_NODE_PREP_BLOCK, "a pass is 1, 2 or 4 rows per thread");
static_assert(2 * CLAMP_PASS_ROWS_MAX <= 0xffff, "record ranks packed in 16 bits");
__device__ __forceinline__ void np_atomic(int64_t* p, int64_t w) {
  atomic_add_u64(reinterpret_cast<uint64_t*>(p), (uint64_t)w);
}
static_assert(CLAMP_LDS_SPECS % KCC_NODE_PREP_BLOCK == 0, "node_prep table fill");
constexpr int64_t NODE_PREP_GRID = 1024;
constexpr int NP_C_CELLS = (int)((CLAMP_LDS_SPECS / 64 + 2) * (CLAMP_LDS_SPECS / 64 + 2));
static_assert(CLAMP_LDS_SPECS == 4096, "node_prep's LDS member tables are 64 x 64");
constexpr size_t NP_OFF_CS = 8 * (size_t)CLAMP_LDS_SPECS;
constexpr size_t NP_OFF_MK = NP_OFF_CS + 4 * (size_t)CLAMP_LDS_SPECS;
constexpr size_t NP_OFF_CK = NP_OFF_MK + 8 * 64 * 64;
constexpr size_t NP_OFF_CJ = NP_OFF_CK + 64 * 65;
constexpr size_t NP_OFF_C = (NP_OFF_CJ + 64 * 65 + 15) / 16 * 16;
constexpr size_t NODE_PREP_LDS = NP_OFF_C + 8 * (size_t)NP_C_CELLS;
constexpr int NP_BINS = 2 * (int)CLAMP_BIN_T_MAX;
constexpr uint32_t NP_ST_MAX = 16;
constexpr size_t NODE_PREP_LDS_SRCH = NP_OFF_MK;
__host__ __device__ inline uint32_t np_stride(int64_t S) {
  uint32_t st = 1;
  while (st < NP_ST_MAX && (int64_t)st * CLAMP_LDS_SPECS < S) st *= 2;
  return st;
}
template <int MODE, int SUB>
__global__ __launch_bounds__(KCC_NODE_PREP_BLOCK) void node_prep_kernel(int64_t n, const uint64_t* __restrict__ alloc_cpu,
                                 const int64_t* __restrict__ alloc_mem,
                                 const int64_t* __restrict__ alloc_pods,
                                 const int64_t* __restrict__ pod_count,
                                 const uint64_t* __restrict__ used_cpu,
                                 const int64_t* __restrict__ used_mem,
                                 FitGroupA* __restrict__ fast_a, FitGroup* __restrict__ fast_b,
                                 SlowNode* __restrict__ slow, int64_t* __restrict__ slow_list,
                                 int64_t S, ClampWork cw,
                                 unsigned long long* __restrict__ counters,
                                 int32_t chunk, int32_t dense, int64_t pass0, PlaceArgs pa) {
  if ((int32_t)blockIdx.x < pa.n_blocks) {
    spec_place_body(pa, blockIdx.x);
    return;
  }
  const int32_t bid = (int32_t)blockIdx.x - pa.n_blocks, nbid = (int32_t)gridDim.x - pa.n_blocks;
  KCC_TL(bid % 1024, 2);
  constexpr int64_t PR = (int64_t)KCC_NODE_PREP_BLOCK * SUB;
  const int lane = threadIdx.x & 63, wv = threadIdx.x >> 6;
  const int64_t stride = (int64_t)nbid * PR;
  uint64_t ld_ac, ld_uc;
  int64_t ld_am, ld_um, ld_P, ld_pc;
  auto load_row = [&](int64_t i) {
    ld_ac = ld_uc = 0;
    ld_am = ld_um = ld_P = ld_pc = 0;
    if (i < n) {
      ld_ac = alloc_cpu[i];
      ld_uc = used_cpu[i];
      ld_am = alloc_mem[i];
      ld_um = used_mem[i];
      ld_P = alloc_pods[i];
      ld_pc = pod_count[i];
    }
  };
  load_row((int64_t)bid * PR + threadIdx.x);
  __shared__ uint32_t np_wc[KCC_NODE_PREP_BLOCK / 64];
  __shared__ uint64_t np_base;
  __shared__ uint32_t np_tot;
  __shared__ uint32_t np_bcnt[NP_BINS];
  __shared__ uint32_t np_bstart[NP_BINS];
  const NpClasses cls = np_classes<false>(cw.bcnt, S, lane);
  const bool want_b = cls.want_b, slow_all = cls.slow_all;
  const int64_t nN = cls.nN;
  const int64_t T = (nN + 63) / 64, W = T + 2;
  const bool binned = MODE == 2 || clamp_binned(S);
  const int NB = (int)(2 * T);
  int64_t* Cc = cw.C + (int64_t)(bid % C_COPIES) * cw.c_stride;
  int64_t* H2c = cw.H2 + (int64_t)(bid % H2_COPIES) * cw.h_stride;
  int64_t* H3c = cw.H3 + (int64_t)(bid % H2_COPIES) * cw.h_stride;
  extern __shared__ __attribute__((aligned(16))) unsigned char np_lds[];
  int64_t* ms_l = reinterpret_cast<int64_t*>(np_lds);
  uint32_t* cs_l = reinterpret_cast<uint32_t*>(np_lds + NP_OFF_CS);
  unsigned long long* mk_l = reinterpret_cast<unsigned long long*>(np_lds + NP_OFF_MK);
  uint8_t* ck_l = np_lds + NP_OFF_CK;
  uint8_t* cj_l = np_lds + NP_OFF_CJ;
  unsigned long long* c_l = reinterpret_cast<unsigned long long*>(np_lds + NP_OFF_C);
  constexpr bool lds = MODE == 2;
  constexpr bool cpriv = lds;
  constexpr bool srch = MODE >= 1;
  const uint32_t st = lds ? 1u : np_stride(S);
  for (int b = threadIdx.x; b < NP_BINS; b += KCC_NODE_PREP_BLOCK) np_bcnt[b] = 0;
  constexpr int PER = (int)(CLAMP_LDS_SPECS / KCC_NODE_PREP_BLOCK);
  uint32_t yv[PER];
  if (srch) {
    uint64_t cv[PER], mv[PER];
#pragma unroll
    for (int u = 0; u < PER; ++u) {
      const int64_t k = threadIdx.x + (int64_t)KCC_NODE_PREP_BLOCK * u;
      const int64_t e = (k + 1) * st - 1;
      cv[u] = e < S ? cw.cs[e] : ~0ull;
      mv[u] = e < S ? (uint64_t)cw.ms[e] : (uint64_t)INT64_MAX;
      yv[u] = lds && k < S ? cw.mr_c[k] : 0xffffffffu;
    }
#pragma unroll
    for (int u = 0; u < PER; ++u) {
      const int64_t k = threadIdx.x + (int64_t)KCC_NODE_PREP_BLOCK * u;
      const bool in = (k + 1) * st - 1 < nN;
      cs_l[np_slot((uint32_t)k)] = in && cv[u] < FAST_FC_MAX ? (uint32_t)cv[u] : 0xffffffffu;
      ms_l[np_slot((uint32_t)k)] = in ? (int64_t)mv[u] : INT64_MAX;
      if (!in) yv[u] = 0xffffffffu;
      if (lds) mk_l[k] = 0ull;
    }
    if (cpriv)
      for (int64_t e = threadIdx.x; e < W * W; e += KCC_NODE_PREP_BLOCK) c_l[e] = 0ull;
  }
  __syncthreads();
  KCC_TL(bid % 1024, 6);
  if (lds) {
#pragma unroll
    for (int u = 0; u < PER; ++u) {
      const int64_t x = threadIdx.x + (int64_t)KCC_NODE_PREP_BLOCK * u;
      if (x < nN)
        __hip_atomic_fetch_or((lds_ull*)(mk_l + mk_at((uint32_t)x >> 6, yv[u] >> 6)), 1ull << (yv[u] & 63),
                              __ATOMIC_RELAXED, __HIP_MEMORY_SCOPE_WORKGROUP);
    }
  }
  __syncthreads();
  KCC_TL(bid % 1024, 7);
  const uint32_t cmin = lds ? cs_l[np_slot(0u)]
                            : (nN > 0 ? (cw.cs[0] < FAST_FC_MAX ? (uint32_t)cw.cs[0] : 0xffffffffu)
                                      : 0xffffffffu);
  const int64_t mmin = lds ? ms_l[np_slot(0u)] : (nN > 0 ? cw.ms[0] : INT64_MAX);
  if (lds) {
    static_assert(KCC_NODE_PREP_BLOCK == 1024, "16 waves: rows wv, wv + 16, wv + 32, wv + 48");
    for (int g = wv; g < 64; g += 32) {
      const uint32_t pk = (uint32_t)__popcll(mk_l[mk_at(g, lane)]) |
                          (uint32_t)__popcll(mk_l[mk_at(lane, g)]) << 8 |
                          (uint32_t)__popcll(mk_l[mk_at(g + 16, lane)]) << 16 |
                          (uint32_t)__popcll(mk_l[mk_at(lane, g + 16)]) << 24;
      const uint32_t inc = wave_incl_scan_u32(pk), exc = inc - pk;
      ck_l[g * 65 + lane] = (uint8_t)exc;
      cj_l[g * 65 + lane] = (uint8_t)(exc >> 8);
      ck_l[(g + 16) * 65 + lane] = (uint8_t)(exc >> 16);
      cj_l[(g + 16) * 65 + lane] = (uint8_t)(exc >> 24);
      if (lane == 63) {
        ck_l[g * 65 + 64] = (uint8_t)inc;
        cj_l[g * 65 + 64] = (uint8_t)(inc >> 8);
        ck_l[(g + 16) * 65 + 64] = (uint8_t)(inc >> 16);
        cj_l[(g + 16) * 65 + 64] = (uint8_t)(inc >> 24);
      }
    }
  }
  auto c_add = [&](int64_t cell, int64_t w) {
    if (cpriv) lds_add_u64(c_l + cell, (uint64_t)w);
    else np_atomic(&Cc[cell], w);
  };
  __syncthreads();
  KCC_TL(bid % 1024, 0);
  for (int64_t i0 = (int64_t)bid * PR; i0 < n; i0 += stride) {
    const int64_t pass = pass0 + i0 / PR;
    uint64_t r_fm[SUB];
    uint32_t r_fc[SUB];
    int32_t r_P[SUB];
    unsigned long long sbal[SUB];
    uint32_t pk1[SUB], pk2[SUB], pk3[SUB];
    uint64_t always_sum = 0;
    uint64_t base_ret = 0;
    uint32_t t_pass = 0;
#pragma unroll
    for (int q = 0; q < SUB; ++q) {
      const int64_t i = i0 + q * KCC_NODE_PREP_BLOCK + threadIdx.x;
      const bool valid = i < n;
      int32_t cl_q;
      const bool ok = np_classify(valid, i, ld_ac, ld_uc, ld_am, ld_um, ld_P, ld_pc, slow_all, slow,
                                  r_fm[q], r_fc[q], r_P[q], cl_q);
      np_slow_append(valid && !ok, i, lane, &counters[CNT_SLOW_ROWS + chunk], slow_list);
      load_row(q + 1 < SUB ? i + KCC_NODE_PREP_BLOCK : i0 + stride + threadIdx.x);
      sbal[q] = __ballot(dense ? valid : (r_fc[q] > 0 && r_fm[q] > 0 && r_P[q] > 0));
      if (q == SUB - 1) {
        if (lane == 0) np_wc[wv] = np_wave_streamed(sbal);
        __syncthreads();
        if (threadIdx.x == 0) {
          t_pass = np_wc_sum(np_wc, KCC_NODE_PREP_BLOCK / 64);
          base_ret = np_stream_claim(t_pass, &counters[CNT_STREAM + chunk]);
        }
        KCC_TL(bid % 1024, 3);
      }
      const int64_t P = r_P[q], Penc = P > 0 ? P : 0;
      const int64_t wfull = Penc - (int64_t)cl_q;
      if (ok && nN > 0 && P <= 0) always_sum += (uint64_t)wfull;
      const double rP = recip_up_f64(P > 0 ? (uint64_t)P : 1ull);
      const int64_t V0 = (int64_t)((double)r_fm[q] * rP);
      const uint32_t U0 = (uint32_t)((double)r_fc[q] * rP);
      const bool act = ok && nN > 0 && P > 0 && wfull != 0 && U0 >= cmin && V0 >= mmin;
      const int64_t w = act ? wfull : 0;
      const uint32_t U = act ? U0 : 0u;
      const int64_t V = act ? V0 : 0;
      uint32_t L = 0, b = 0;
      if (srch) {
        uint32_t iL = 1, ib = 1;
#pragma unroll
        for (int lv = 0; lv < 12; ++lv) {
          iL = 2 * iL + (cs_l[iL] <= U ? 1u : 0u);
          ib = 2 * ib + (ms_l[ib] <= V ? 1u : 0u);
        }
        L = iL - 4096u;
        b = ib - 4096u;
        L += L == 4095u && cs_l[0] <= U ? 1u : 0u;
        b += b == 4095u && ms_l[0] <= V ? 1u : 0u;
        if (!lds) {
          L *= st;
          b *= st;
          uint32_t addL = 0, addb = 0;
#pragma unroll 4
          for (uint32_t j = 0; j + 1 < st; ++j) {
            addL += w && L + j < (uint64_t)nN && cw.cs[L + j] <= (uint64_t)U ? 1u : 0u;
            addb += w && b + j < (uint64_t)nN && cw.ms[b + j] <= V ? 1u : 0u;
          }
          L += addL;
          b += addb;
        }
      } else {
        L = w ? upper_bound_count(cw.cs, nN, (uint64_t)U) : 0u;
        b = w ? upper_bound_count(cw.ms, nN, V) : 0u;
      }
      const uint32_t GX = L >> 6, rx = L & 63u, GY = b >> 6, ry = b & 63u;
      uint32_t k, j;
      if (lds) {
        const uint32_t gx = GX < 63u ? GX : 63u, yb = GY < 63u ? GY : 63u;
        const uint64_t mk = mk_l[mk_at(gx, yb)];
        k = (uint32_t)ck_l[gx * 65 + GY] + (uint32_t)__popcll(mk & ((1ull << ry) - 1ull));
        j = cj_l[yb * 65 + GX];
      } else {
        const int64_t mx = nN - 64 * (int64_t)GX, my = nN - 64 * (int64_t)GY;
        k = w && rx ? count_lt64(cw.mr_c + 64 * GX, b, (uint32_t)(mx < 64 ? mx : 64)) : 0u;
        j = w && ry && GX > 0 ? count_lt64(cw.cr_m + 64 * GY, GX << 6, (uint32_t)(my < 64 ? my : 64)) : 0u;
      }
      if (w && GX > 0 && GY > 0) c_add((int64_t)GX * W + GY, w);
      const bool has2 = w && rx > 0 && k > 0;
      const bool has3 = w && ry > 0 && GX > 0 && j > 0;
      if (!binned) {
        if (has2) np_atomic(&H2c[((int64_t)GX * 65 + k) * 64 + rx], w);
        if (has3) np_atomic(&H3c[((int64_t)GY * 65 + j) * 64 + ry], w);
      }
      const bool rec2 = binned && has2, rec3 = binned && has3;
      const uint32_t bin2 = rec2 ? GX : 0u, bin3 = rec3 ? (uint32_t)T + GY : 0u;
      const uint32_t rk2 = rec2 ? atomicAdd(&np_bcnt[bin2], 1u) : 0u;
      const uint32_t rk3 = rec3 ? atomicAdd(&np_bcnt[bin3], 1u) : 0u;
      const uint32_t wu = (uint32_t)(int32_t)w;
      pk1[q] = (rec2 ? k * 64 + rx : 0u) | (rec3 ? j * 64 + ry : 0u) << 13 | (wu & 63u) << 26;
      pk2[q] = rk2 | rk3 << 13 | ((wu >> 6) & 63u) << 26;
      pk3[q] = bin2 | bin3 << 9 | (uint32_t)((int32_t)wu >> 12) << 18;
      __builtin_amdgcn_sched_barrier(0);
    }
    {
      const uint64_t v = np_always_sum(always_sum);
      if (lane == 0 && v) c_add((T + 1) * W + T + 1, (int64_t)v);
    }
    if (threadIdx.x == 0) {
      np_base = base_ret;
      np_tot = t_pass;
    }
    __syncthreads();
    KCC_TL(bid % 1024, 4);
    if (binned && wv == 1) {
      const int per = (NB + 63) / 64;
      const int b0 = lane * per, b1 = min(b0 + per, NB);
      uint32_t ls = 0;
      for (int bb = b0; bb < b1; ++bb) ls += np_bcnt[bb];
      uint32_t li = ls;
#pragma unroll
      for (int d = 1; d < 64; d <<= 1) {
        const uint32_t t = __shfl_up(li, d, 64);
        if (lane >= d) li += t;
      }
      uint32_t* drow = cw.dir + pass * cw.d_stride;
      uint32_t run = li - ls;
      for (int bb = b0; bb < b1; ++bb) {
        const uint32_t c = np_bcnt[bb];
        np_bstart[bb] = run;
        drow[bb] = run;
        np_bcnt[bb] = 0;
        run += c;
      }
      if (lane == 63) drow[NB] = li;
    }
    __syncthreads();
    {
      const uint64_t sb0 = np_base + np_wc_sum(np_wc, wv);
      const uint32_t tot = np_tot;
      uint32_t done = 0;
      uint64_t* prec = cw.rec + pass * (2 * PR);
#pragma unroll
      for (int q = 0; q < SUB; ++q) {
        if ((sbal[q] >> lane) & 1ull)
          np_put<false>(sb0 + done + (uint32_t)__popcll(sbal[q] & ((1ull << lane) - 1ull)), r_fm[q], r_fc[q],
                        r_P[q] > 0 ? (uint32_t)r_P[q] : 0u, 0, fast_a, fast_b, want_b, nullptr);
        done += (uint32_t)__popcll(sbal[q]);
        const uint32_t c2 = pk1[q] & 0x1fffu, c3 = (pk1[q] >> 13) & 0x1fffu;
        if (c2 | c3) {
          const int32_t wr = (int32_t)pk3[q] >> 18 << 12 | (int32_t)((pk2[q] >> 26) << 6 | pk1[q] >> 26);
          const uint64_t wbits = (uint64_t)(uint32_t)wr << 32;
          if (c2) NP_ST(prec[np_bstart[pk3[q] & 0x1ffu] + (pk2[q] & 0x1fffu)], wbits | c2);
          if (c3) NP_ST(prec[np_bstart[(pk3[q] >> 9) & 0x1ffu] + ((pk2[q] >> 13) & 0x1fffu)], wbits | c3);
        }
      }
      if (threadIdx.x < np_padded(tot) - tot)
        np_put<false>(np_base + tot + threadIdx.x, 0ull, 0u, 0u, 0, fast_a, fast_b, want_b, nullptr);
    }
    __syncthreads();
    KCC_TL(bid % 1024, 5);
  }
  if (cpriv) {
    for (int64_t e = threadIdx.x; e < W * W; e += KCC_NODE_PREP_BLOCK) {
      const unsigned long long v = c_l[e];
      if (v) np_atomic(&Cc[e], (int64_t)v);
    }
  }
  KCC_TL(bid % 1024, 1);
}

__device__ __forceinline__ float recip_up_f32(uint64_t v) {
  const double vd = (double)v;
  float r = (float)(1.0 / vd);
  if (fma((double)r, vd, -1.0) < 0.0) r = __uint_as_float(__float_as_uint(r) + 1u);
  return r;
}



__device__ void spec_rank_count(const RankArgs& ra, int64_t blk, uint64_t* lds) {
  const int64_t S = ra.S;
  const uint64_t* __restrict__ c_in = ra.c_in;
  const int64_t* __restrict__ m_in = ra.m_in;
  const int tid = threadIdx.x, lane = tid & 63, wv = tid >> 6;
  typedef uint64_t u64x2_t __attribute__((ext_vector_type(2)));
  u64x2_t* key_l = reinterpret_cast<u64x2_t*>(lds);
  uint32_t* part = reinterpret_cast<uint32_t*>(lds);
  const int64_t ns = rank_slices(S);
  const int64_t qb = blk / ns, sl = blk % ns;
  const int64_t i = qb * 64 + lane;
  const bool qv = i < S;
  const uint64_t c = qv ? c_in[i] : 0;
  const int64_t m = qv ? m_in[i] : 0;
  const int32_t ci = qv ? spec_class(c, m) : SPEC_EXACT;
  if (sl == 0 && wv == 0) {
    const uint32_t na = (uint32_t)__popcll(__ballot(ci == SPEC_A));
    const uint32_t nb = (uint32_t)__popcll(__ballot(ci == SPEC_B));
    if (lane == 0) {
      ra.bcnt[2 * qb] = na;
      ra.bcnt[2 * qb + 1] = nb;
    }
  }
  const int64_t j0 = sl * RANK_L, j1 = j0 + RANK_L < S ? j0 + RANK_L : S;
  for (int64_t j = j0 + tid; j < j1; j += 256) {
    const uint64_t cj = c_in[j];
    const int64_t mj = m_in[j];
    const bool nj = spec_class(cj, mj) != SPEC_EXACT;
    u64x2_t k;
    k.x = nj ? cj << 13 | (uint64_t)(j & 8191) : ~0ull;
    k.y = nj ? (uint64_t)mj << 13 | (uint64_t)(j & 8191) : ~0ull;
    key_l[j - j0] = k;
  }
  __syncthreads();
  const int64_t chq = i >> 13, chs = j0 >> 13;
  const uint64_t tc = chs < chq ? (c + 1) << 13 : (chs == chq ? c << 13 | (uint64_t)(i & 8191) : c << 13);
  const uint64_t tm = chs < chq ? ((uint64_t)m + 1) << 13
                                : (chs == chq ? (uint64_t)m << 13 | (uint64_t)(i & 8191) : (uint64_t)m << 13);
  const int n = (int)(j1 - j0);
  const int w0 = n * wv / 4, w1 = n * (wv + 1) / 4;
  uint32_t rc = 0, rm = 0;
#pragma unroll 4
  for (int j = w0; j < w1; ++j) {
    const u64x2_t k = key_l[j];
    rc += k.x < tc ? 1u : 0u;
    rm += k.y < tm ? 1u : 0u;
  }
  __syncthreads();
  part[(wv * 2 + 0) * 64 + lane] = rc;
  part[(wv * 2 + 1) * 64 + lane] = rm;
  __syncthreads();
  uint32_t* const slices = ra.part + 2 * S;
  if (wv < 2) {
    const uint32_t t = part[(0 * 2 + wv) * 64 + lane] + part[(1 * 2 + wv) * 64 + lane] +
                       part[(2 * 2 + wv) * 64 + lane] + part[(3 * 2 + wv) * 64 + lane];
    if (qv) __hip_atomic_store(slices + (sl * 2 + wv) * S + i, t, __ATOMIC_RELAXED, __HIP_MEMORY_SCOPE_AGENT);
    asm volatile("s_waitcnt vmcnt(0)" ::: "memory");
  }
  __syncthreads();
  uint32_t& last_s = rank_small(lds)[0];
  if (tid == 0)
    last_s = ns == 1 ? 1u
                     : (uint32_t)(__hip_atomic_fetch_add(ra.arrive + qb, 1u, __ATOMIC_RELAXED,
                                                         __HIP_MEMORY_SCOPE_AGENT) == (uint32_t)ns - 1u);
  __syncthreads();
  if (!last_s || wv != 0) return;
  asm volatile("" ::: "memory");
  if (ns > 1 && lane == 0) ra.arrive[qb] = 0;
  if (!qv || ci == SPEC_EXACT) return;
  uint32_t x = 0, y = 0;
  for (int64_t k = 0; k < ns; ++k) {
    x += __hip_atomic_load(slices + (k * 2 + 0) * S + i, __ATOMIC_RELAXED, __HIP_MEMORY_SCOPE_AGENT);
    y += __hip_atomic_load(slices + (k * 2 + 1) * S + i, __ATOMIC_RELAXED, __HIP_MEMORY_SCOPE_AGENT);
  }
  ra.cs[x] = c;
  ra.ms[y] = m;
  ra.mr_c[x] = y;
  ra.cr_m[y] = x;
  ra.part[i] = x;
  ra.part[S + i] = y;
}

__device__ void spec_rank_sort(const RankArgs& ra, int64_t blk, uint64_t* lds) {
  const int64_t S = ra.S;
  const uint64_t* __restrict__ c_in = ra.c_in;
  const int64_t* __restrict__ m_in = ra.m_in;
  const int tid = threadIdx.x, lane = tid & 63, wv = tid >> 6;
  const int64_t ns = rank_slices(S);
  const int64_t qb = blk / ns, sl = blk % ns;
  const int64_t j0 = sl * RANK_L;
  uint64_t kx[4], ky[4];
  uint32_t nrm = 0;
#pragma unroll
  for (int q = 0; q < 4; ++q) {
    const int64_t j = j0 + 4 * tid + q;
    const uint64_t cj = j < S ? c_in[j] : 0;
    const int64_t mj = j < S ? m_in[j] : 0;
    const bool nj = j < S && spec_class(cj, mj) != SPEC_EXACT;
    kx[q] = nj ? cj << 13 | (uint64_t)(j & 8191) : ~0ull;
    ky[q] = nj ? (uint64_t)mj << 13 | (uint64_t)(j & 8191) : ~0ull;
    nrm += nj ? 1u : 0u;
  }
  uint64_t* const lx = lds;
  uint64_t* const ly = lds + RANK_L;
  auto cx = [](uint64_t& a, uint64_t& b, bool asc) {
    const uint64_t lo = a < b ? a : b, hi = a < b ? b : a;
    a = asc ? lo : hi;
    b = asc ? hi : lo;
  };
  typedef uint64_t u64x2_t __attribute__((ext_vector_type(2)));
  auto xlane = [&](uint32_t v, int msk) -> uint32_t {
    switch (msk) {
      case 1: return (uint32_t)__builtin_amdgcn_mov_dpp((int)v, 0xB1, 0xf, 0xf, false);
      case 2: return (uint32_t)__builtin_amdgcn_mov_dpp((int)v, 0x4E, 0xf, 0xf, false);
      case 4: return (uint32_t)__builtin_amdgcn_ds_swizzle((int)v, 0x1F | (4 << 10));
      case 8: return (uint32_t)__builtin_amdgcn_ds_swizzle((int)v, 0x1F | (8 << 10));
      case 16: return (uint32_t)__builtin_amdgcn_ds_swizzle((int)v, 0x1F | (16 << 10));
      default: return (uint32_t)__builtin_amdgcn_ds_bpermute((lane ^ 32) << 2, (int)v);
    }
  };
  auto xlane64 = [&](uint64_t v, int msk) -> uint64_t {
    return (uint64_t)xlane((uint32_t)(v >> 32), msk) << 32 | xlane((uint32_t)v, msk);
  };
#pragma unroll
  for (int k = 2; k <= RANK_L; k <<= 1) {
#pragma unroll
    for (int jj = k >> 1; jj > 0; jj >>= 1) {
// ... 91 lines not shown
  for (int e = 0; e < 4; ++e) {
    const int64_t i = qb * RANK_L + 256 * e + tid;
    if (i >= S) continue;
    uint32_t rx = 0, ry = 0;
    if (ci[e] != SPEC_EXACT) {
      const uint64_t own = (uint64_t)(i & 8191);
      if (sl < qb) {
        rx = c[e] == V_TOP ? n_norm : lower_bound(lx, (c[e] + 1) << 13);
        ry = (uint64_t)m[e] == V_TOP ? n_norm : lower_bound(ly, ((uint64_t)m[e] + 1) << 13);
      } else if (sl > qb) {
        rx = lower_bound(lx, c[e] << 13);
        ry = lower_bound(ly, (uint64_t)m[e] << 13);
      } else {
        rx = lower_bound(lx, c[e] << 13 | own);
        ry = lower_bound(ly, (uint64_t)m[e] << 13 | own);
      }
    }
    __hip_atomic_store(slices + (sl * 2 + 0) * S + i, rx, __ATOMIC_RELAXED, __HIP_MEMORY_SCOPE_AGENT);
    __hip_atomic_store(slices + (sl * 2 + 1) * S + i, ry, __ATOMIC_RELAXED, __HIP_MEMORY_SCOPE_AGENT);
  }
  asm volatile("s_waitcnt vmcnt(0)" ::: "memory");
  __syncthreads();
  uint32_t& last_s = rank_small(lds)[0];
  if (tid == 0)
    last_s = ns == 1 ? 1u
                     : (uint32_t)(__hip_atomic_fetch_add(ra.arrive + qb, 1u, __ATOMIC_RELAXED,
                                                         __HIP_MEMORY_SCOPE_AGENT) == (uint32_t)ns - 1u);
  __syncthreads();
  if (!last_s) return;
  asm volatile("" ::: "memory");
  if (ns > 1 && tid == 0) ra.arrive[qb] = 0;
#pragma unroll
  for (int e = 0; e < 4; ++e) {
    const int64_t i = qb * RANK_L + 256 * e + tid;
    if (i >= S || ci[e] == SPEC_EXACT) continue;
    uint32_t x = 0, y = 0;
    for (int64_t k = 0; k < ns; ++k) {
      x += __hip_atomic_load(slices + (k * 2 + 0) * S + i, __ATOMIC_RELAXED, __HIP_MEMORY_SCOPE_AGENT);
      y += __hip_atomic_load(slices + (k * 2 + 1) * S + i, __ATOMIC_RELAXED, __HIP_MEMORY_SCOPE_AGENT);
    }
    ra.cs[x] = c[e];
    ra.ms[y] = m[e];
    ra.mr_c[x] = y;
    ra.cr_m[y] = x;
    ra.part[i] = x;
    ra.part[S + i] = y;
  }
}

__device__ void spec_rank_body(const RankArgs& ra, int64_t blk, uint64_t* lds) {
  const int tid = threadIdx.x;
  if (ra.zero_only) {
    const bool wt = ra.done_flag != nullptr;
    if (tid < CNT_N && tid != CNT_SPECS_A && tid != CNT_SPECS_B) {
      if (wt) __hip_atomic_store(ra.counters + tid, 0ull, __ATOMIC_RELAXED, __HIP_MEMORY_SCOPE_AGENT);
      else ra.counters[tid] = 0;
    }
    const int lane = tid & 63;
    const int64_t nqb = (ra.S + 63) / 64;
    int32_t cls[CLAMP_LDS_SPECS / 256];
#pragma unroll
    for (int u = 0; u < (int)(CLAMP_LDS_SPECS / 256); ++u) {
      const int64_t j = ((int64_t)(tid >> 6) + 4 * u) * 64 + lane;
      cls[u] = j < ra.S ? spec_class(ra.c_in[j], ra.m_in[j]) : SPEC_EXACT;
    }
#pragma unroll
    for (int u = 0; u < (int)(CLAMP_LDS_SPECS / 256); ++u) {
      const int64_t qb = (tid >> 6) + 4 * u;
      const uint32_t na = (uint32_t)__popcll(__ballot(cls[u] == SPEC_A));
      const uint32_t nb = (uint32_t)__popcll(__ballot(cls[u] == SPEC_B));
      if (qb < nqb && lane == 0) {
        if (wt) {
          __hip_atomic_store(ra.bcnt + 2 * qb, na, __ATOMIC_RELAXED, __HIP_MEMORY_SCOPE_AGENT);
          __hip_atomic_store(ra.bcnt + 2 * qb + 1, nb, __ATOMIC_RELAXED, __HIP_MEMORY_SCOPE_AGENT);
        } else {
          ra.bcnt[2 * qb] = na;
          ra.bcnt[2 * qb + 1] = nb;
        }
      }
    }
    if (wt) {
      asm volatile("s_waitcnt vmcnt(0)" ::: "memory");
      __syncthreads();
      if (tid == 0)
        __hip_atomic_store(ra.done_flag + NP_DONE,
                           __hip_atomic_load(ra.done_flag + NP_EPOCH, __ATOMIC_RELAXED, __HIP_MEMORY_SCOPE_AGENT) + 1u,
                           __ATOMIC_RELAXED, __HIP_MEMORY_SCOPE_AGENT);
    }
    return;
  }
  {
    const int64_t gt = blk * 256 + tid, nt = (int64_t)ra.n_blocks * 256;
    if (gt < CNT_N && gt != CNT_SPECS_A && gt != CNT_SPECS_B) ra.counters[gt] = 0;
    for (int64_t e = gt; e < C_COPIES * ra.c_cells; e += nt)
      ra.C[(e / ra.c_cells) * ra.c_stride + e % ra.c_cells] = 0;
  }
  if (ra.S <= RANK_FULL_MAX) spec_rank_count(ra, blk, lds);
  else spec_rank_sort(ra, blk, lds);
}

__global__ __launch_bounds__(256) void spec_rank_kernel(RankArgs ra) {
  __shared__ __attribute__((aligned(16))) uint64_t lds[RANK_LDS_WORDS];
  spec_rank_body(ra, blockIdx.x, lds);
}


__device__ void spec_place_body(const PlaceArgs& pa, int64_t blk) {
  const int64_t S = pa.S;
  const uint64_t* __restrict__ c_in = pa.c_in;
  const int64_t* __restrict__ m_in = pa.m_in;
  const SpecPrep& sp = pa.sp;
  const ClampWork& cw = pa.cw;
  int64_t* __restrict__ partial = pa.partial;
  unsigned long long* __restrict__ counters = pa.counters;
  const int64_t i = blk * blockDim.x + threadIdx.x;
  const int lane = threadIdx.x & 63;
  const int64_t nqb = (S + 63) / 64, qb = i >> 6;
  const bool in = i < S;
  const uint64_t c = in ? c_in[i] : 0;
  const int64_t m = in ? m_in[i] : 0;
  const int32_t cls = in ? spec_class(c, m) : SPEC_EXACT;
  const bool normal = cls != SPEC_EXACT;
  const uint32_t x = in && normal && !pa.no_ranks ? cw.rank[i] : 0u;
  uint64_t tot = 0, pre = 0;
  const unsigned long long* bc = reinterpret_cast<const unsigned long long*>(cw.bcnt);
  for (int64_t b = lane; b < nqb; b += 64) {
    const uint64_t v = __hip_atomic_load(bc + b, __ATOMIC_RELAXED, __HIP_MEMORY_SCOPE_AGENT);
    tot += v;
    pre += b < qb ? v : 0ull;
  }
  tot = readlane_u64(wave_incl_scan_u64(tot), 63);
  pre = readlane_u64(wave_incl_scan_u64(pre), 63);
  const uint32_t nA = (uint32_t)tot, nB = (uint32_t)(tot >> 32);
  const uint32_t pA = (uint32_t)pre, pB = (uint32_t)(pre >> 32);
  const int64_t nN = (int64_t)nA + nB;
  const unsigned long long mA = __ballot(cls == SPEC_A && in), mB = __ballot(cls == SPEC_B && in);
  const unsigned long long below = (1ull << lane) - 1ull;
  const uint32_t rA = (uint32_t)__popcll(mA & below), rB = (uint32_t)__popcll(mB & below);
  if (!pa.no_ranks && i >= nN && i < (nN + 63) / 64 * 64) {
    cw.mr_c[i] = 0xffffffffu;
    cw.cr_m[i] = 0xffffffffu;
  }
  if (i == 0) {
    counters[CNT_SPECS_A] = nA;
    counters[CNT_SPECS_B] = nB;
  }
  if (!in) return;
  const int64_t pos = cls == SPEC_A ? (int64_t)pA + rA
                    : cls == SPEC_B ? (int64_t)nA + pB + rB
                                    : nN + (qb * 64 - pA - pB) + (lane - rA - rB);
  SpecRec rec;
  rec.c = c;
  rec.m = m;
  rec.rc = normal ? recip_up_f64(c) : 0.0;
  rec.rm = normal ? recip_up_f64((uint64_t)m) : 0.0;
  rec.rcf = cls == SPEC_A ? recip_up_f32(c) : 0.0f;
  rec.cls = cls;
  rec.pad = 0;
  sp.rec[pos] = rec;
  sp.perm[pos] = (int32_t)i;
  partial[i] = 0;
  partial[S + i] = device_faulted(pa.faults) ? (int64_t)SPEC_FAULT_MARK : 0;
  if (!normal || pa.no_ranks) return;
  cw.dperm[x] = (int32_t)pos;
}


constexpr int CP_THREADS = 1024;
constexpr int CP_WAVES = CP_THREADS / 64;
constexpr int64_t C_FULL_CELLS = 4624;
constexpr int H_CELLS = 65 * 64;
__host__ __device__ inline bool clamp_c_full(int64_t T) { return (T + 2) * (T + 2) <= C_FULL_CELLS; }

constexpr int CP_PW = 4096;
constexpr int64_t CP_SPLIT = 4;
constexpr int CP_RB = 8;
__device__ __forceinline__ void clamp_consume_bin(const ClampWork& cw, int64_t bin, uint64_t* tab,
                                                  uint32_t* w_lo, uint32_t* w_off, uint64_t* scratch,
                                                  uint32_t h, uint32_t G) {
  constexpr int PPT = CP_PW / CP_THREADS;
  const int tid = threadIdx.x, lane = tid & 63, wv = tid >> 6;
  uint32_t* wsum = reinterpret_cast<uint32_t*>(scratch);
  for (int64_t p0 = 0; p0 < cw.n_pass; p0 += CP_PW) {
    const int np = (int)(cw.n_pass - p0 < CP_PW ? cw.n_pass - p0 : CP_PW);
    uint32_t lo[PPT], cnt[PPT];
#pragma unroll
    for (int u = 0; u < PPT; ++u) {
      const int p = tid * PPT + u;
      lo[u] = 0;
      cnt[u] = 0;
      if (p < np) {
        const uint32_t* d = cw.dir + (p0 + p) * cw.d_stride + bin;
        lo[u] = d[0];
        cnt[u] = d[1];
      }
    }
    uint32_t ts = 0;
#pragma unroll
    for (int u = 0; u < PPT; ++u) {
      cnt[u] -= lo[u];
      ts += cnt[u];
// ... 25 lines not shown
    __syncthreads();
    int top = 1;
    while (2 * top <= np) top *= 2;
    auto search = [&](uint32_t j) {
      int p = 0;
      for (int st = top; st >= 1; st >>= 1)
        if (w_off[p + st] <= j) p += st;
      return p;
    };
    const uint32_t s0 = (uint32_t)((uint64_t)total * h / G), s1 = (uint32_t)((uint64_t)total * (h + 1) / G);
    const uint32_t per_w = (s1 - s0 + CP_WAVES * 64 - 1) / (CP_WAVES * 64) * 64;
    const uint32_t J0 = s0 + (uint32_t)wv * per_w;
    const uint32_t J1 = J0 + per_w < s1 ? J0 + per_w : s1;
    int p = J0 + lane < J1 ? search(J0 + lane) : 0;
    uint32_t nxt = w_off[p + 1], gb = w_lo[p] - w_off[p];
    const uint64_t* rec0 = cw.rec + p0 * cw.pass_recs;
    auto load_batch = [&](uint64_t (&rv)[CP_RB], uint32_t jb) {
#pragma unroll
      for (int u = 0; u < CP_RB; ++u) {
        const uint32_t j = jb + (uint32_t)(64 * u + lane);
        rv[u] = 0;
        if (j < J1) {
          if (j >= nxt) {
            p = w_off[p + 2] <= j ? search(j) : p + 1;
            nxt = w_off[p + 1];
            gb = w_lo[p] - w_off[p];
          }
          rv[u] = rec0[(int64_t)p * cw.pass_recs + (uint32_t)(j + gb)];
        }
      }
    };
    auto add_batch = [&](const uint64_t (&rv)[CP_RB], uint32_t jb) {
#pragma unroll
      for (int u = 0; u < CP_RB; ++u)
        if (jb + (uint32_t)(64 * u + lane) < J1)
          atomicAdd(reinterpret_cast<unsigned long long*>(&tab[(uint32_t)rv[u]]),
                    (unsigned long long)(int64_t)(int32_t)(rv[u] >> 32));
    };
    const uint32_t step = 64u * CP_RB;
    uint64_t ra[CP_RB], rb[CP_RB];
    load_batch(ra, J0);
    for (uint32_t jb = J0; jb < J1; jb += 2 * step) {
      load_batch(rb, jb + step);
      add_batch(ra, jb);
      load_batch(ra, jb + 2 * step);
      add_batch(rb, jb + step);
    }
    __syncthreads();
  }
}

__device__ __forceinline__ void clamp_apply_bin(const ClampWork& cw, int64_t S,
                                                int64_t* __restrict__ partial, int64_t nN,
                                                int64_t u, uint32_t G, uint32_t h) {
  __shared__ uint64_t tab[H_CELLS];
  __shared__ uint64_t ctot[CP_WAVES][64];
  __shared__ uint64_t colsum[128];
  __shared__ uint32_t pos_s[64];
  __shared__ uint32_t cp_lo[CP_PW];
  __shared__ uint32_t cp_off[CP_PW + 1];
  const int64_t T = (nN + 63) / 64, W = T + 2;
  KCC_TL(1024 + blockIdx.x % 1024, 0);
  const int tid = threadIdx.x, lane = tid & 63, wv = tid >> 6;
  const bool x_side = u < T;
  const int64_t g = x_side ? u : u - T;
  const bool full = clamp_c_full(T);
  const int64_t q = 64 * g + lane;
  uint32_t other = 0xffffffffu;
  if (wv == 0 || wv == CP_WAVES - 1) other = (x_side ? cw.mr_c : cw.cr_m)[q];
  if (tid < 128) colsum[tid] = 0;
  const bool binned = clamp_binned(S);
  int64_t* H = (x_side ? cw.H2 : cw.H3) + g * H_CELLS;
  constexpr int PER = (H_CELLS + CP_THREADS - 1) / CP_THREADS;
  uint64_t v[PER];
#pragma unroll
  for (int k = 0; k < PER; ++k) {
    const int e = tid + CP_THREADS * k;
    v[k] = 0;
    if (!binned) {
#pragma unroll
      for (int c = 0; c < H2_COPIES; ++c) v[k] += e < H_CELLS ? (uint64_t)H[c * cw.h_stride + e] : 0ull;
    }
  }
  constexpr int CPER = (int)((C_FULL_CELLS + CP_THREADS - 1) / CP_THREADS);
  uint64_t cv[CPER];
  const int64_t c0 = (g + 1) * W, c1 = W * W;
  const bool do_c = x_side && full && h == 0;
#pragma unroll
  for (int k = 0; k < CPER; ++k) {
    const int64_t e = c0 + tid + CP_THREADS * k;
    cv[k] = 0;
    if (do_c && e < c1) {
#pragma unroll
      for (int c = 0; c < C_COPIES; ++c) cv[k] += (uint64_t)cw.C[c * cw.c_stride + e];
    }
  }
#pragma unroll
  for (int k = 0; k < PER; ++k) {
    const int e = tid + CP_THREADS * k;
    if (e < H_CELLS) {
      tab[e] = v[k];
      if (!binned) {
#pragma unroll
        for (int c = 0; c < H2_COPIES; ++c) H[c * cw.h_stride + e] = 0;
      }
    }
  }
// ... 10 lines not shown
  }
  int32_t p = 0x7fffffff;
  if (wv == 0 && q < nN) p = cw.dperm[x_side ? q : (int64_t)other];
  for (int k = wv; k < 65; k += CP_WAVES) {
    const uint64_t sr = wave_incl_scan_u64(tab[k * 64 + 63 - lane]);
    tab[k * 64 + 63 - lane] = sr;
  }
  if (wv == CP_WAVES - 1) {
    uint32_t pos = 0;
    for (int l = 0; l < 64; ++l) pos += (uint32_t)__builtin_amdgcn_readlane((int)other, l) < other ? 1u : 0u;
    pos_s[lane] = pos;
  }
  __syncthreads();
  constexpr int KCH = (65 + CP_WAVES - 1) / CP_WAVES;
  const int k0 = wv * KCH, k1 = k0 + KCH < 65 ? k0 + KCH : 65;
  {
    const uint32_t posl = pos_s[lane];
    uint64_t part = 0;
    for (int k = k0; k < k1; ++k)
      part += (lane < 63 && (uint32_t)k > posl) ? tab[k * 64 + lane + 1] : 0ull;
    ctot[wv][lane] = part;
  }
  __syncthreads();
  if (wv != 0) return;
  KCC_TL(1024 + blockIdx.x % 1024, 3);
  uint64_t csuf = 0;
  if (do_c) {
    uint64_t carry = 0;
    for (int ch = 1; ch >= 0; --ch) {
      const int col = ch * 64 + 63 - lane;
      uint64_t sv = col < W ? colsum[col] : 0ull;
      sv = wave_incl_scan_u64(sv) + carry;
      carry = readlane_u64(sv, 63);
      if (col < W) colsum[col] = sv;
    }
    const uint32_t gy1 = other == 0xffffffffu ? 0xffffffffu : (other >> 6) + 1;
    csuf = gy1 < W ? colsum[gy1] : 0ull;
  }
  if (q >= nN) return;
  uint64_t d = csuf;
#pragma unroll
  for (int w2 = 0; w2 < CP_WAVES; ++w2) d += ctot[w2][lane];
  if (x_side && !full && h == 0) {
    const int64_t gy = other >> 6;
    uint64_t part[8] = {};
    for (int64_t G = g + 1; G <= T + 1; G += 8) {
#pragma unroll
      for (int r = 0; r < 8; ++r)
        part[r] += G + r <= T + 1 ? (uint64_t)cw.Crow[(G + r) * W + gy + 1] : 0ull;
    }
#pragma unroll
    for (int r = 0; r < 8; ++r) d += part[r];
  }
  if (d && p < clamp_n_pure(nN, S)) atomic_add_u64(reinterpret_cast<uint64_t*>(&partial[p]), 0ull - d);
  KCC_TL(1024 + blockIdx.x % 1024, 4);
}

__device__ void fused_finalize(const FinArgs& fin, int64_t S, const int64_t* partial,
                               uint32_t* ctr, uint32_t expect, int64_t s0, int64_t s1) {
  asm volatile("s_waitcnt vmcnt(0)" ::: "memory");
  __syncthreads();
  __shared__ uint32_t last_s;
  if (threadIdx.x == 0) {
    last_s = __hip_atomic_fetch_add(ctr, 1u, __ATOMIC_RELAXED, __HIP_MEMORY_SCOPE_AGENT) ==
             expect - 1u;
    if (last_s) __hip_atomic_store(ctr, 0u, __ATOMIC_RELAXED, __HIP_MEMORY_SCOPE_AGENT);
  }
  __syncthreads();
  if (!last_s) return;
  const bool faulted = device_faulted(fin.faults);
  constexpr int FIN_PER = 4;
  const int64_t nt = blockDim.x;
  for (int64_t i0 = s0 + threadIdx.x; i0 < s1; i0 += (int64_t)FIN_PER * nt) {
    int64_t t[FIN_PER], e[FIN_PER];
    int32_t dst[FIN_PER];
#pragma unroll
    for (int k = 0; k < FIN_PER; ++k) {
      const int64_t i = min(i0 + (int64_t)k * nt, s1 - 1);
      t[k] = __hip_atomic_load(partial + i, __ATOMIC_RELAXED, __HIP_MEMORY_SCOPE_AGENT);
      e[k] = __hip_atomic_load(partial + S + i, __ATOMIC_RELAXED, __HIP_MEMORY_SCOPE_AGENT);
      dst[k] = fin.perm[i];
    }
#pragma unroll
    for (int k = 0; k < FIN_PER; ++k) {
      if (i0 + (int64_t)k * nt >= s1) break;
      const bool fk = faulted || (uint64_t)e[k] >= SPEC_FAULT_MARK;
      fin.totals[dst[k]] = e[k] != 0 || fk ? 0 : t[k];
      fin.spec_err[dst[k]] = fk ? SPEC_ERR_FAULT : e[k] != 0 ? SPEC_ERR_DIV0 : 0;
    }
  }
}

__global__ __launch_bounds__(CP_THREADS) void clamp_apply_kernel(ClampWork cw,
                                                                 const unsigned long long* __restrict__ counters,
                                                                 int64_t S, int64_t* __restrict__ partial,
                                                                 FinArgs fin) {
  const int64_t nN = clamp_n_normal(counters);
  const int64_t T = (nN + 63) / 64;
  const int64_t Tm = (S + 63) / 64;
  const uint32_t G = gridDim.x / (uint32_t)(2 * Tm), h = blockIdx.x / (uint32_t)(2 * Tm);
  const int64_t u = blockIdx.x % (uint32_t)(2 * Tm);
  if (u < 2 * T) clamp_apply_bin(cw, S, partial, nN, u, G, h);
  if (fin.totals) fused_finalize(fin, S, partial, fin.arrive, gridDim.x, 0, S);
}

__global__ __launch_bounds__(256) void clamp_crows_kernel(ClampWork cw,
                                                          const unsigned long long* __restrict__ counters) {
  const int64_t nN = clamp_n_normal(counters);
  const int64_t T = (nN + 63) / 64, W = T + 2;
  const int64_t G = (int64_t)blockIdx.x * 4 + (threadIdx.x >> 6);
  const int lane = threadIdx.x & 63;
  if (nN == 0 || clamp_c_full(T) || G >= W) return;
  uint64_t carry = 0;
  for (int64_t ch = (W + 63) / 64 - 1; ch >= 0; --ch) {
    const int64_t gy = ch * 64 + 63 - lane;
    uint64_t v = 0;
#pragma unroll
    for (int c = 0; c < C_COPIES; ++c) v += gy < W ? (uint64_t)cw.C[c * cw.c_stride + G * W + gy] : 0ull;
    v = wave_incl_scan_u64(v) + carry;
    carry = readlane_u64(v, 63);
    if (gy < W) cw.Crow[G * W + gy] = (int64_t)v;
  }
}

typedef int32_t i32x4 __attribute__((ext_vector_type(4)));
typedef int32_t i32x8 __attribute__((ext_vector_type(8)));
typedef int32_t i32x16 __attribute__((ext_vector_type(16)));
typedef float f32x2 __attribute__((ext_vector_type(2)));

__device__ __forceinline__ void set_round_down() {
  asm volatile("s_setreg_imm32_b32 hwreg(HW_REG_MODE, 0, 4), 10\n\ts_nop 1" ::: "memory");
}
__device__ __forceinline__ void set_round_nearest() {
  asm volatile("s_setreg_imm32_b32 hwreg(HW_REG_MODE, 0, 4), 0\n\ts_nop 1" ::: "memory");
}
__device__ __forceinline__ double min_f64_s(double x, double p) {
  double d;
  asm("v_min_f64 %0, %1, %2" : "=v"(d) : "v"(x), "s"(p));
  return d;
}

constexpr int FIT_SPW = 256;
constexpr int FIT_CHUNK_GROUPS = 128;
constexpr uint32_t FIT_QCHUNK = 32;
static_assert(FIT_QCHUNK >= 2 && FIT_QCHUNK <= FIT_CHUNK_GROUPS, "claims sum in i32");
constexpr uint32_t FIT_QDIV = 2;
constexpr uint32_t FIT_QMIN = 2;
constexpr uint32_t FIT_Q1_DIV = 8;
constexpr uint32_t FIT_Q_HALVE = 128;
constexpr uint32_t FIT_WG_PER_SUB = 24;
constexpr uint32_t FIT_QSUBS = (uint32_t)FIT_QSUBS_MAX;

__device__ __forceinline__ double f64_at(const i32x16& v, int k) {
  return __longlong_as_double(((int64_t)(uint32_t)v[2 * k + 1] << 32) | (uint32_t)v[2 * k]);
}

#define KCC_FIT_ATTR __attribute__((amdgpu_waves_per_eu(8)))
template <bool CL>
__device__ __forceinline__ void fit_body(
    int64_t n_nodes, uint32_t* __restrict__ queue, const FitGroupA* __restrict__ fast_a,
    const FitGroup* __restrict__ fast_b, const SlowNode* __restrict__ slow,
    const int64_t* __restrict__ slow_list, int64_t S, const SpecRec* __restrict__ specs,
    int64_t* __restrict__ partial, unsigned long long* __restrict__ counters, int32_t chunk,
    int32_t gx, int32_t gy, const int32_t* __restrict__ fast_cl,
    const unsigned long long* __restrict__ faults, const int32_t b, uint32_t* q_slot) {
  const int32_t xcd = b & 7, r = b >> 3;
  const int32_t bx = r % gx, by = (r / gx) * 8 + xcd;
  if (by >= gy) return;
  __builtin_amdgcn_s_setprio(3);
  KCC_TL(2048 + b % 4096, 0);
  const int32_t wv = __builtin_amdgcn_readfirstlane((int32_t)(threadIdx.x >> 6));
  const int lane = threadIdx.x & 63;
  const int64_t s = (int64_t)bx * FIT_SPW + threadIdx.x;
  const bool active = s < S;
  const bool idle = !__any(active);
  SpecRec sr;
  if (active) {
    sr = specs[s];
  } else {
    sr.c = 1;
    sr.m = CLASS_A_M_MIN;
    sr.rc = 1.0;
    sr.rm = 1.0 / (double)CLASS_A_M_MIN;
    sr.rcf = 1.0f;
    sr.cls = SPEC_A;
  }
  const uint64_t c = sr.c;
  const int64_t m = sr.m;
  const double rm = sr.rm, rc = sr.rc;
  const bool wave_exact = __any(sr.cls == SPEC_EXACT);
  const bool wave_b = __any(sr.cls == SPEC_B);
  const bool wave_fast = !wave_exact && !idle;
  KCC_TL(2048 + b % 4096, 5);

  const uint32_t n_groups = (uint32_t)(counters[CNT_STREAM + chunk] / FIT_GROUP);
  uint32_t lim = n_groups;
  uint32_t base = 0;
  uint32_t nxt = 0;
  uint32_t nsub = (uint32_t)gy / FIT_WG_PER_SUB;
  nsub = nsub <= 8u ? 8u : (nsub >= FIT_QSUBS ? FIT_QSUBS : 1u << (31 - __builtin_clz(nsub)));
  if ((uint32_t)gy < nsub) nsub = (uint32_t)gy;
  const uint32_t sub = (uint32_t)by % nsub;
  uint32_t* const qp = queue + ((uint32_t)bx * FIT_QSUBS + sub) * 16u;
  const uint32_t qsz = n_groups / (uint32_t)gy < FIT_Q_HALVE ? FIT_QCHUNK / 2u : FIT_QCHUNK;
  uint32_t q1 = qsz;
  {
    const uint32_t sh = n_groups / (uint32_t)gy / FIT_Q1_DIV;
    q1 = sh < q1 ? (sh > FIT_QMIN ? sh : FIT_QMIN) : q1;
  }

  auto claim_issue = [&](uint32_t sz) {
    if (wv == 0 && lane == 0)
      asm volatile("global_atomic_add %0, %1, %2, off sc0"
                   : "=v"(nxt) : "v"(qp), "v"(sz) : "memory");
  };
  const uint32_t wps = ((uint32_t)gy + nsub - 1u) / nsub;
  const uint32_t wseg = ((uint32_t)gy - sub + nsub - 1u) / nsub;
  const uint32_t dyn0 = wseg * q1;
  uint32_t qcur = q1;
  auto claim_publish = [&](uint32_t slot) {
    if (wv == 0) {
      asm volatile("s_waitcnt vmcnt(0)" : "+v"(nxt) : : "memory");
      if (lane == 0) q_slot[slot] = dyn0 + nxt;
    }
    __syncthreads();
  };
  {
    const uint32_t seg = ((n_groups + nsub - 1u) / nsub + 7u) / 8u * 8u;
    base = sub * seg < n_groups ? sub * seg : n_groups;
    lim = base + seg < n_groups ? base + seg : n_groups;
    KCC_TL(2048 + b % 4096, 1);
  }
  const uint32_t first = ((uint32_t)by / nsub) * q1;
  uint32_t pr_done = 0;
  const uint32_t pr_share = (lim - base) / wseg > 0 ? (lim - base) / wseg : 1u;
#ifdef KCC_TIMELINE
  uint32_t tl_done = 0;
#endif
  uint64_t acc = 0;
  uint64_t errs = 0;
  uint32_t slow_iters = 0;

  auto eval_slow = [&](int64_t i) {
    ++slow_iters;
    const SlowNode sn = slow[i];
    int64_t qc = 0, qm = 0;
    bool z = false;
    if (sn.fc != 0) {
      if (c == 0) z = true;
      else qc = (int64_t)(sn.fc / c);
    }
    if (sn.fm != 0) {
      if (m == 0) z = true;
      else if (m == -1) qm = (int64_t)(0ull - (uint64_t)sn.fm);
      else qm = sn.fm / m;
    }
    int64_t q = qc <= qm ? qc : qm;
    if (q >= sn.P) q = sn.cl;
    errs += z ? 1u : 0u;
    acc += z ? 0ull : (uint64_t)q;
  };

  auto sum_a = [&](uint32_t g0, int cnt) {
    cnt = __builtin_amdgcn_readfirstlane(cnt);
    const FitGroupA* gbase = fast_a + g0;
    const f32x2 rcf2 = {sr.rcf, sr.rcf};
    int32_t acc32 = 0;
    set_round_down();
    for (int gi = 0; gi < cnt; ++gi) {
      int io = gi;
      asm volatile("" : "+s"(io));
      const FitGroupA* g = gbase + io;
      const i32x16 fmv = *reinterpret_cast<const i32x16*>(g->fm);
      const i32x8 fcv = *reinterpret_cast<const i32x8*>(g->fc);
      const i32x8 Pv = *reinterpret_cast<const i32x8*>(g->P);
#pragma unroll
      for (int u = 0; u < FIT_GROUP / 2; ++u) {
        const f32x2 fcp = {__int_as_float(fcv[2 * u]), __int_as_float(fcv[2 * u + 1])};
        const f32x2 q = fcp * rcf2;
        uint32_t m3[2];
#pragma unroll
        for (int h = 0; h < 2; ++h) {
          const int k = 2 * u + h;
          const uint32_t qm = (uint32_t)__double_as_longlong(f64_at(fmv, k) * rm);
          const uint32_t qc = __float_as_uint(h ? q.y : q.x);
          m3[h] = min(min(qc, qm), (uint32_t)Pv[k]);
        }
        acc32 += (int32_t)(m3[0] + m3[1]);
// ... 58 lines not shown
      const i32x16 fmv = *reinterpret_cast<const i32x16*>(g->fm);
      const i32x16 Pv = *reinterpret_cast<const i32x16*>(g->Pb);
      const i32x8 clv = *reinterpret_cast<const i32x8*>(cbase + (size_t)io * FIT_GROUP);
#pragma unroll
      for (int u = 0; u < FIT_GROUP / 2; ++u) {
        int32_t x[2];
#pragma unroll
        for (int h = 0; h < 2; ++h) {
          const int k = 2 * u + h;
          const double qc = __builtin_fma(f64_at(fcv, k), rc, bias);
          const double qm = __builtin_fma(f64_at(fmv, k), rm, bias);
          const double xb = __builtin_fmin(qc, qm);
          const int32_t xi = (int32_t)(uint32_t)__double_as_longlong(xb);
          x[h] = xb >= f64_at(Pv, k) ? clv[k] : xi;
        }
        acc32 += x[0] + x[1];
      }
    }
    set_round_nearest();
    acc += (uint64_t)(int64_t)acc32;
  };
  auto sum_b = [&](uint32_t g0, int cnt) {
    cnt = __builtin_amdgcn_readfirstlane(cnt);
    const FitGroup* gbase = fast_b + g0;
    const double bias = FIT_BIAS;
    int32_t acc32 = 0;
    set_round_down();
    for (int gi = 0; gi < cnt; ++gi) {
      int io = gi;
      asm volatile("" : "+s"(io));
      const FitGroup* g = gbase + io;
      const i32x16 fcv = *reinterpret_cast<const i32x16*>(g->fc);
      const i32x16 fmv = *reinterpret_cast<const i32x16*>(g->fm);
      const i32x16 Pv = *reinterpret_cast<const i32x16*>(g->Pb);
#pragma unroll
      for (int u = 0; u < FIT_GROUP / 2; ++u) {
        int32_t x[2];
#pragma unroll
        for (int h = 0; h < 2; ++h) {
          const int k = 2 * u + h;
          const double qc = __builtin_fma(f64_at(fcv, k), rc, bias);
          const double qm = __builtin_fma(f64_at(fmv, k), rm, bias);
          const double xb = min_f64_s(__builtin_fmin(qc, qm), f64_at(Pv, k));
          x[h] = (int32_t)(uint32_t)__double_as_longlong(xb);
        }
        acc32 += x[0] + x[1];
      }
    }
    set_round_nearest();
    acc += (uint64_t)(int64_t)acc32;
  };

  {
    for (uint32_t k = 0;; ++k) {
      const uint32_t cur = base + (k == 0 ? first : __builtin_amdgcn_readfirstlane(q_slot[k & 1u]));
      if (cur >= lim) break;
      const uint32_t rem = lim - cur;
      uint32_t qn = rem / (FIT_QDIV * wps);
      qn = qn < FIT_QMIN ? FIT_QMIN : (qn > qsz ? qsz : qn);

      claim_issue(qn);
      const int cnt = (int)((cur + qcur < lim ? cur + qcur : lim) - cur);
      qcur = qn;
      if (wave_fast) {
        if constexpr (CL) {
          if (!wave_b) sum_a_nc(cur, cnt);
          else sum_b_nc(cur, cnt);
        } else {
          if (!wave_b) sum_a(cur, cnt);
          else sum_b(cur, cnt);
        }
      }
      claim_publish((k + 1u) & 1u);
      {
        pr_done += (uint32_t)cnt;
        const uint32_t lv = (4u * pr_done) / pr_share;
        if (lv == 0) __builtin_amdgcn_s_setprio(3);
        else if (lv == 1) __builtin_amdgcn_s_setprio(2);
        else if (lv == 2) __builtin_amdgcn_s_setprio(1);
        else __builtin_amdgcn_s_setprio(0);
      }
      KCC_TLV(2048 + b % 4096, 4, (uint64_t)k + 1);
#ifdef KCC_TIMELINE
      tl_done += (uint32_t)cnt;
      if (k == 0) KCC_TL(2048 + b % 4096, 6);
#endif
    }
    if (wv == 0 && lane == 0) {
      const uint32_t d = atomicAdd(qp + 1, 1u);
      if (d == wseg - 1u) {
        qp[0] = 0;
        qp[1] = 0;
      }
    }
  }
  KCC_TL(2048 + b % 4096, 2);
#ifdef KCC_TIMELINE
  KCC_TLV(2048 + b % 4096, 7, tl_done);
#endif
  if (idle) return;
  if (wave_exact) {
    const uint32_t nn = (uint32_t)n_nodes;
    const uint32_t pn = (nn + (uint32_t)gy - 1u) / (uint32_t)gy;
    const uint32_t a0 = (uint32_t)by * pn < nn ? (uint32_t)by * pn : nn;
    const int64_t i1 = a0 + pn < nn ? a0 + pn : nn;
    for (int64_t i = a0; i < i1; ++i) eval_slow(i);
  } else {
    const int64_t n_slow = (int64_t)counters[CNT_SLOW_ROWS + chunk];
    for (int64_t j = by; j < n_slow; j += gy) eval_slow(slow_list[j]);
  }

  {
    const unsigned long long act = __ballot(active);
    if (slow_iters && lane == 0)
      atomicAdd(&counters[CNT_SLOW_PAIRS], (unsigned long long)slow_iters * (unsigned long long)__popcll(act));
  }
  if (CL && by == 0 && wave_fast) acc -= (uint64_t)counters[CNT_CLAMP_ALL];
  if (by == 0 && device_faulted(faults)) errs += SPEC_FAULT_MARK;
  if (active) {
    atomic_add_u64(reinterpret_cast<uint64_t*>(&partial[s]), acc);
    if (errs) atomic_add_u64(reinterpret_cast<uint64_t*>(&partial[S + s]), errs);
  }
  KCC_TL(2048 + b % 4096, 3);
}

template <bool CL>
__global__ __launch_bounds__(256) KCC_FIT_ATTR void fit_kernel(
    int64_t n_nodes, uint32_t* __restrict__ queue, const FitGroupA* __restrict__ fast_a,
    const FitGroup* __restrict__ fast_b, const SlowNode* __restrict__ slow,
    const int64_t* __restrict__ slow_list, int64_t S, const SpecRec* __restrict__ specs,
    int64_t* __restrict__ partial, unsigned long long* __restrict__ counters, int32_t chunk,
    int32_t gx, int32_t gy, const int32_t* __restrict__ fast_cl,
    const unsigned long long* __restrict__ faults) {
  __shared__ uint32_t q_slot[2];
  fit_body<CL>(n_nodes, queue, fast_a, fast_b, slow, slow_list, S, specs, partial, counters, chunk,
               gx, gy, fast_cl, faults, (int32_t)blockIdx.x, q_slot);
}

__global__ void fit_finalize_kernel(int64_t S, const int64_t* __restrict__ partial,
                                    const int32_t* __restrict__ perm, int64_t* __restrict__ totals,
                                    int32_t* __restrict__ spec_err,
                                    const unsigned long long* __restrict__ faults) {
  const int64_t i = (int64_t)blockIdx.x * blockDim.x + threadIdx.x;
  if (i >= S) return;
  const int32_t dst = perm[i];
  const bool err = partial[S + i] != 0;
  const bool faulted = device_faulted(faults) || (uint64_t)partial[S + i] >= SPEC_FAULT_MARK;
  totals[dst] = err || faulted ? 0 : partial[i];
  spec_err[dst] = faulted ? SPEC_ERR_FAULT : err ? SPEC_ERR_DIV0 : 0;
}

[[maybe_unused]] constexpr uint32_t P2P_SPIN_MAX = 1u << 21;
constexpr int64_t P2P_MAX_WG = 256;
__global__ __launch_bounds__(256) void exchange_finalize_kernel(P2PArgs a) {
  const int64_t S = a.S, smax = a.smax, i0 = (int64_t)blockIdx.x * 256 + threadIdx.x;
  const int64_t gs = (int64_t)gridDim.x * 256;
  const uint64_t epoch = __hip_atomic_load(a.epoch, __ATOMIC_RELAXED, __HIP_MEMORY_SCOPE_AGENT) + 1;
  const bool faulted_in = device_faulted(a.faults);
  const int W = a.W, par = (int)(epoch & 1u);
  const int64_t slot = ((int64_t)par * W + a.rank) * 2 * smax;
  const size_t fw = p2p_flag_words(W);
  for (int64_t i = i0; i < S; i += gs) {
    const int64_t v0 = a.partial[i], v1 = a.partial[S + i];
    for (int p = 0; p < W; ++p) {
      int64_t* d = reinterpret_cast<int64_t*>(a.mbox[p]) + fw + slot;
      d[i] = v0;
      d[smax + i] = v1;
    }
  }
  __builtin_amdgcn_fence(__ATOMIC_RELEASE, "");
  __syncthreads();
  if (threadIdx.x == 0) {
    const uint32_t old = __hip_atomic_fetch_add(a.arrive, 1u, __ATOMIC_ACQ_REL, __HIP_MEMORY_SCOPE_AGENT);
    if (old == gridDim.x - 1u) {
      __hip_atomic_store(a.arrive, 0u, __ATOMIC_RELAXED, __HIP_MEMORY_SCOPE_AGENT);
      __hip_atomic_store(a.epoch, epoch, __ATOMIC_RELAXED, __HIP_MEMORY_SCOPE_AGENT);
      for (int p = 0; p < W; ++p)
        __hip_atomic_store(reinterpret_cast<uint64_t*>(a.mbox[p]) + ((int64_t)par * W + a.rank) * 8,
                           epoch, __ATOMIC_RELEASE, __HIP_MEMORY_SCOPE_SYSTEM);
    }
  }
  __shared__ uint32_t gave_up;
  if (threadIdx.x == 0) gave_up = 0;
  __syncthreads();
  if (threadIdx.x < (unsigned)W) {
#ifdef KCC_DIAG_P2P_GIVEUP
    atomicAdd(&a.faults[FAULT_P2P], 1ull);
    gave_up = 1;
#else
// ... 108 lines not shown
    if ((e = hipMemsetAsync(used_cpu, 0, 8 * (size_t)n_nodes, s)) != hipSuccess ||
        (e = hipMemsetAsync(used_mem, 0, 8 * (size_t)n_nodes, s)) != hipSuccess)
      return e;
    if (limits && ((e = hipMemsetAsync(lim_cpu, 0, 8 * (size_t)n_nodes, s)) != hipSuccess ||
                   (e = hipMemsetAsync(lim_mem, 0, 8 * (size_t)n_nodes, s)) != hipSuccess))
      return e;
  }
  if (!red && ra.n_blocks == 0 && npb == 0) return hipSuccess;
  if (limits && (ra.n_blocks > 0 || npb > 0)) return hipErrorInvalidValue;
  if (npb > 0 && (ra.n_blocks != 1 || !ra.zero_only || !ra.done_flag)) return hipErrorInvalidValue;
  const bool ranks_last = n_containers >= RED_RANKS_LAST_MIN;
  const int64_t reserve = ranks_last ? 0 : (int64_t)RED_WAVES_PER_BLOCK * ra.n_blocks;
  const int32_t range = red ? reduce_range(n_containers, limits, reserve) : RED_TILE;
  const int64_t waves = red ? (n_containers + range - 1) / range : 0;
  if (waves > reduce_tail_records()) return hipErrorInvalidValue;
  const int64_t red_blocks = (waves + RED_WAVES_PER_BLOCK - 1) / RED_WAVES_PER_BLOCK;
  const unsigned blocks = (unsigned)(red_blocks + ra.n_blocks + npb);
  np.ptr = node_ptr;
  np.c0 = c0;
  np.range = range;
  np.red_waves = (int32_t)waves;
  RedArgs a{};
  a.n_nodes = n_nodes;
  a.c0 = c0;
  a.c_end = c0 + n_containers;
  a.range = range;
  a.ptr = node_ptr;
  a.in[0] = cpu_req;
  a.in[1] = reinterpret_cast<const uint64_t*>(mem_req);
  a.in[2] = limits ? cpu_lim : nullptr;
  a.in[3] = limits ? reinterpret_cast<const uint64_t*>(mem_lim) : nullptr;
  a.out[0] = used_cpu;
  a.out[1] = reinterpret_cast<uint64_t*>(used_mem);
  a.out[2] = limits ? lim_cpu : nullptr;
  a.out[3] = limits ? reinterpret_cast<uint64_t*>(lim_mem) : nullptr;
  a.tail = tail;
  a.faults = faults;
  a.ranks_last = ranks_last ? 1 : 0;
  auto kern = limits ? reduce_kernel<4, false> : npb > 0 ? reduce_kernel<2, true> : reduce_kernel<2, false>;
  if (ev_start || ev_stop)
    hipExtLaunchKernelGGL(kern, dim3(blocks), dim3(256), 0, s, ev_start, ev_stop, 0, a, ra, np);
  else
    hipLaunchKernelGGL(kern, dim3(blocks), dim3(256), 0, s, a, ra, np);
  return hipGetLastError();
}

hipError_t launch_node_prep(int64_t n_nodes, const uint64_t* alloc_cpu,
                            const int64_t* alloc_mem, const int64_t* alloc_pods,
                            const int64_t* pod_count, const uint64_t* used_cpu,
                            const int64_t* used_mem, FitGroupA* fast_a, FitGroup* fast_b,
                            SlowNode* slow, int64_t* slow_list, int64_t n_specs,
                            ClampWork cw, unsigned long long* counters, int chunk, int64_t row0,
                            int64_t call_nodes, hipStream_t s, bool dense,
                            const PlaceArgs* place) {
  if (n_nodes <= 0 && !place) return hipSuccess;
  const int64_t pr = clamp_pass_rows(call_nodes);
  if (row0 % pr != 0 || (pr != 1024 && pr != 4096)) return hipErrorInvalidValue;
  const int mode = n_specs <= CLAMP_LDS_SPECS ? 2 : n_specs <= (int64_t)NP_ST_MAX * CLAMP_LDS_SPECS ? 1 : 0;
  PlaceArgs pa{};
  if (place) {
    pa = *place;
    pa.n_blocks = (int32_t)((n_specs + KCC_NODE_PREP_BLOCK - 1) / KCC_NODE_PREP_BLOCK);
  }
  const size_t lds_bytes = mode == 2 ? NODE_PREP_LDS : mode == 1 ? NODE_PREP_LDS_SRCH : 0;
  auto kern = pr == 1024 ? (mode == 2 ? node_prep_kernel<2, 1> : mode == 1 ? node_prep_kernel<1, 1> : node_prep_kernel<0, 1>)
                         : (mode == 2 ? node_prep_kernel<2, 4> : mode == 1 ? node_prep_kernel<1, 4> : node_prep_kernel<0, 4>);
  static std::atomic<int64_t> resident[2][3][MAX_DEVS];
  const int64_t res = resident_blocks(resident[pr == 1024 ? 0 : 1][mode],
                                      reinterpret_cast<const void*>(kern), KCC_NODE_PREP_BLOCK,
                                      lds_bytes, 256);
  const int64_t cap = res < NODE_PREP_GRID ? res : NODE_PREP_GRID;
  const unsigned np_blocks = n_nodes > 0 ? grid_for(n_nodes, (int)pr, cap) : 0u;
  hipLaunchKernelGGL(kern, dim3(np_blocks + (unsigned)pa.n_blocks), dim3(KCC_NODE_PREP_BLOCK),
                     lds_bytes, s, n_nodes, alloc_cpu, alloc_mem, alloc_pods, pod_count, used_cpu,
                     used_mem, fast_a, fast_b, slow, slow_list, n_specs, cw,
                     counters, (int32_t)chunk, (int32_t)(dense ? 1 : 0), row0 / pr, pa);
  return hipGetLastError();
}

RankArgs rank_args(int64_t n_specs, const uint64_t* spec_cpu, const int64_t* spec_mem,
                   const ClampWork& cw, unsigned long long* counters, uint32_t* arrive,
                   bool zero_only) {
  RankArgs ra{};
  ra.S = n_specs;
  ra.c_in = spec_cpu;
  ra.m_in = spec_mem;
  ra.part = cw.rank;
  ra.arrive = arrive;
  ra.bcnt = cw.bcnt;
  ra.cs = cw.cs;
  ra.ms = cw.ms;
  ra.mr_c = cw.mr_c;
  ra.cr_m = cw.cr_m;
  ra.C = cw.C;
  ra.c_stride = cw.c_stride;
  const int64_t wmax = (n_specs + 63) / 64 + 2;
  ra.c_cells = wmax * wmax < cw.c_stride ? wmax * wmax : cw.c_stride;
  ra.counters = counters;
  ra.n_blocks = n_specs <= 0 ? 0
               : zero_only ? 1
               : n_specs <= RANK_FULL_MAX ? (int32_t)((n_specs + 63) / 64 * rank_slices(n_specs))
                                          : (int32_t)(rank_slices(n_specs) * rank_slices(n_specs));
  ra.zero_only = zero_only ? 1 : 0;
  return ra;
}

hipError_t launch_spec_rank(const RankArgs& ra, hipStream_t s) {
  if (ra.n_blocks <= 0) return hipSuccess;
  hipLaunchKernelGGL(spec_rank_kernel, dim3((unsigned)ra.n_blocks), dim3(256), 0, s, ra);
  return hipGetLastError();
}

hipError_t launch_clamp_apply(int64_t n_specs, int64_t n_nodes, ClampWork cw,
                              const unsigned long long* counters, int64_t* partial, hipStream_t s,
                              const FinArgs* fin) {
  if (n_specs <= 0) return hipSuccess;
  cw.n_pass = clamp_passes(n_nodes);
  cw.pass_recs = 2 * clamp_pass_rows(n_nodes);
  const int64_t T = (n_specs + 63) / 64;
  if (!clamp_c_full(T))
    hipLaunchKernelGGL(clamp_crows_kernel, dim3((unsigned)((T + 2 + 3) / 4)), dim3(256), 0, s, cw,
                       counters);
  const FinArgs f = fin ? *fin : FinArgs{};
  hipLaunchKernelGGL(clamp_apply_kernel, dim3((unsigned)clamp_apply_blocks(n_specs)), dim3(CP_THREADS),
                     0, s, cw, counters, n_specs, partial, f);
  return hipGetLastError();
}

int64_t clamp_apply_blocks(int64_t n_specs) {
  if (n_specs <= 0) return 0;
  const int64_t T = (n_specs + 63) / 64;
  static std::atomic<int64_t> cache[MAX_DEVS];
  const int64_t resident = resident_blocks(cache, reinterpret_cast<const void*>(clamp_apply_kernel),
                                           CP_THREADS, 0, 256);
  int64_t G = 1;
  if (clamp_binned(n_specs))
    while (G < CP_SPLIT && 2 * T * G * 2 <= resident) G *= 2;
  return 2 * T * G;
}

int64_t fit_resident_blocks() {
  static std::atomic<int64_t> cache[MAX_DEVS];
  return resident_blocks(cache, reinterpret_cast<const void*>(fit_kernel<false>), 256, 0, 2048);
}

static int64_t fit_grid_y(int64_t n_nodes, int64_t n_specs, int64_t grid_nodes) {
  const int64_t gx = (n_specs + FIT_SPW - 1) / FIT_SPW;
  const int64_t n_groups = fit_groups(n_nodes);
  int64_t gy = fit_resident_blocks() / gx;
  if (grid_nodes > n_nodes) gy = gy * n_nodes / grid_nodes;
  if (gy >= 16) gy = gy / 8 * 8;
  const int64_t claims = (n_groups + FIT_QCHUNK - 1) / FIT_QCHUNK;
  if (gy > claims) gy = claims;
  if (gy < 1) gy = 1;
  return gy;
}

hipError_t launch_fit(int64_t n_nodes, const FitGroupA* fast_a, const FitGroup* fast_b,
                      const SlowNode* slow,
                      const int64_t* slow_list, int64_t n_specs, SpecPrep sp, int64_t* partial,
                      unsigned long long* counters, uint32_t* queue, int chunk,
                      int64_t grid_nodes, hipStream_t s, const unsigned long long* faults,
                      const int32_t* fast_cl, hipEvent_t ev_start, hipEvent_t ev_stop) {
  if (n_nodes <= 0 || n_specs <= 0) return hipSuccess;
  const int64_t gx = (n_specs + FIT_SPW - 1) / FIT_SPW;
  const int64_t gy = fit_grid_y(n_nodes, n_specs, grid_nodes);
  const int64_t blocks = gx * ((gy + 7) / 8 * 8);
  if (blocks > 0x7fffffffLL || gy > 0x7fffffffLL) return hipErrorInvalidValue;
  auto kern = fast_cl ? fit_kernel<true> : fit_kernel<false>;
  if (ev_start || ev_stop)
    hipExtLaunchKernelGGL(kern, dim3((unsigned)blocks), dim3(256), 0, s, ev_start, ev_stop, 0, n_nodes,
                          queue, fast_a, fast_b, slow, slow_list, n_specs, sp.rec, partial, counters,
                          (int32_t)chunk, (int32_t)gx, (int32_t)gy, fast_cl, faults);
  else
    hipLaunchKernelGGL(kern, dim3((unsigned)blocks), dim3(256), 0, s, n_nodes, queue, fast_a,
                       fast_b, slow, slow_list, n_specs, sp.rec, partial, counters, (int32_t)chunk,
                       (int32_t)gx, (int32_t)gy, fast_cl, faults);
  return hipGetLastError();
}

hipError_t launch_fit_finalize(int64_t n_specs, const int64_t* partial, const int32_t* perm,
                               int64_t* totals, int32_t* spec_err,
                               const unsigned long long* faults, hipStream_t s) {
  if (n_specs <= 0) return hipSuccess;
  hipLaunchKernelGGL(fit_finalize_kernel, dim3(grid_for(n_specs, 256, 1 << 30)), dim3(256), 0, s,
                     n_specs, partial, perm, totals, spec_err, faults);
  return hipGetLastError();
}

hipError_t launch_exchange_finalize(const P2PArgs& a, hipStream_t s) {
  if (a.S <= 0) return hipSuccess;
  if (a.S > a.smax || a.W < 1 || a.W > P2P_MAX_RANKS || a.rank < 0 || a.rank >= a.W ||
      !a.epoch || !a.faults || !a.arrive)
    return hipErrorInvalidValue;
  hipLaunchKernelGGL(exchange_finalize_kernel, dim3(grid_for(a.S, 256, P2P_MAX_WG)), dim3(256), 0, s, a);
  return hipGetLastError();
}

hipError_t launch_partial_add(int64_t n, int64_t* dst, const int64_t* src, hipStream_t s) {
  if (n <= 0) return hipSuccess;
  hipLaunchKernelGGL(partial_add_kernel, dim3(grid_for(n, 256, 1 << 30)), dim3(256), 0, s, n, dst,
                     src);
  return hipGetLastError();
}

}

#ifdef KCC_TIMELINE
extern "C" int kcc_debug_timeline(void* host) {
  if (hipDeviceSynchronize() != hipSuccess) return -1;
  if (hipMemcpyFromSymbol(host, HIP_SYMBOL(kcc::kcc_tl), sizeof(uint64_t) * 8192 * 8) != hipSuccess)
    return -2;
  static uint64_t zero[8192][8];
  return hipMemcpyToSymbol(HIP_SYMBOL(kcc::kcc_tl), zero, sizeof(zero)) == hipSuccess ? 0 : -3;
}
#endif
```

### kubernetesclustercapacity_amd/engine.py

```python
from __future__ import annotations

import ctypes as C
from dataclasses import dataclass

import numpy as np

from . import _lib

COMM_ID_BYTES = 128
P2P_HANDLE_BYTES = 64


class KccError(RuntimeError):
    def __init__(self, code: int, msg: str):
        super().__init__(f"{_lib.ERROR_NAMES.get(code, code)}: {msg}")
        self.code = code


def _arr(x, dtype) -> np.ndarray:
    a = np.ascontiguousarray(x, dtype=dtype)
    return a


def _p(a) -> C.c_void_p | None:
# ... 408 lines not shown

    def allreduce_partial_async(self, n_specs, partial, stream=None):
        self._check(self._lib.kcc_allreduce_partial_async(self._h, n_specs, _dp(partial),
                                                          _stream(stream)))

    def p2p_export(self, n_ranks: int, max_specs: int) -> bytes:
        buf = C.create_string_buffer(P2P_HANDLE_BYTES)
        self._check(self._lib.kcc_p2p_export(self._h, int(n_ranks), int(max_specs),
                                             C.cast(buf, C.c_void_p)))
        return buf.raw

    def p2p_open(self, rank: int, handles):
        blob = b"".join(handles)
        if len(blob) != P2P_HANDLE_BYTES * len(handles):
            raise ValueError(f"each handle holds {P2P_HANDLE_BYTES} bytes")
        buf = C.create_string_buffer(blob, len(blob))
        self._check(self._lib.kcc_p2p_open(self._h, int(rank), C.cast(buf, C.c_void_p)))

    def exchange_finalize_async(self, n_specs, partial, totals, spec_err, stream=None):
        self._check(self._lib.kcc_exchange_finalize_async(self._h, n_specs, _dp(partial),
                                                          _dp(totals), _dp(spec_err),
                                                          _stream(stream)))

    def p2p_faults(self) -> int:
        v = C.c_int64()
        self._check(self._lib.kcc_p2p_faults(self._h, C.byref(v)))
        return v.value

    def profile_enable(self, on: bool = True):
        self._check(self._lib.kcc_profile_enable(self._h, 1 if on else 0))

    def profile_read(self):
        rm, rn, fm, fn = C.c_double(), C.c_int64(), C.c_double(), C.c_int64()
        self._check(self._lib.kcc_profile_read(self._h, C.byref(rm), C.byref(rn), C.byref(fm),
                                               C.byref(fn)))
        return rm.value, rn.value, fm.value, fn.value

    def set_fit_dense(self, dense: bool):
        self._check(self._lib.kcc_set_fit_dense(self._h, 1 if dense else 0))

    def set_clamp_in_fit(self, mode: int):
        self._check(self._lib.kcc_set_clamp_in_fit(self._h, int(mode)))

    def clamp_in_fit_used(self) -> bool:
        v = C.c_int()
        self._check(self._lib.kcc_clamp_in_fit_used(self._h, C.byref(v)))
        return bool(v.value)

    def fit_stream_rows(self) -> int:
        v = C.c_int64()
        self._check(self._lib.kcc_fit_stream_rows(self._h, C.byref(v)))
        return v.value

    def reduce_faults(self) -> int:
        v = C.c_int64()
        self._check(self._lib.kcc_reduce_faults(self._h, C.byref(v)))
        return v.value

    def clear_faults(self):
        self._check(self._lib.kcc_clear_faults(self._h))

    def fit_slow_pairs(self):
        a, b = C.c_int64(), C.c_int64()
        self._check(self._lib.kcc_fit_slow_pairs(self._h, C.byref(a), C.byref(b)))
        return a.value, b.value


def _key32(key) -> np.ndarray:
    k = np.asarray(key)
    if k.dtype != np.int32 and k.size and (k.max() > np.iinfo(np.int32).max or
                                           k.min() < np.iinfo(np.int32).min):
        raise ValueError("row keys must fit int32")
    return np.ascontiguousarray(k, np.int32)


def _stream(stream):
    if stream is None:
        return None
    h = getattr(stream, "cuda_stream", stream)
    return C.c_void_p(int(h)) if h else None


def select_groups(totals, err, eligible):
    t = np.asarray(totals, np.int64)
    e = np.asarray(err, np.int32)
    if t.ndim != 2 or e.shape != t.shape:
        raise ValueError("totals and err must both be [G, S]")
    m = np.asarray(eligible, bool)
    if m.shape == t.shape[:1]:
        m = np.broadcast_to(m[:, None], t.shape)
    if m.shape != t.shape:
        raise ValueError("eligible must be [G, S] or [G]")
    flagged = ((e != 0) & m).any(axis=0)
    s = np.where(m, t, 0).astype(np.int64).view(np.uint64).sum(axis=0, dtype=np.uint64)
    out = np.where(flagged, np.uint64(0), s).astype(np.uint64).view(np.int64)
    return out, flagged.astype(np.int32)


def verdict(totals, replicas):
    return np.asarray(totals, np.int64) >= np.asarray(replicas, np.int64)
```

Baseline: 14290 billion evals/s.

## Split fit stream into big-node region scanned only by large-spec column blocks

```diff
diff --git a/include/kcc.h b/include/kcc.h
--- a/include/kcc.h
+++ b/include/kcc.h
@@ -132,6 +132,8 @@
 int kcc_set_clamp_in_fit(kcc_ctx* ctx, int mode);
 int kcc_clamp_in_fit_used(kcc_ctx* ctx, int* used);
 int kcc_fit_stream_rows(kcc_ctx* ctx, int64_t* streamed);
+int kcc_set_fit_split(kcc_ctx* ctx, int mode);
+int kcc_fit_split_stats(kcc_ctx* ctx, int64_t* big_rows, int64_t* small_specs);
 
 double kcc_last_slow_fraction(const kcc_ctx* ctx);
 
diff --git a/kubernetesclustercapacity_amd/_lib.py b/kubernetesclustercapacity_amd/_lib.py
--- a/kubernetesclustercapacity_amd/_lib.py
+++ b/kubernetesclustercapacity_amd/_lib.py
@@ -52,6 +52,8 @@
     "kcc_set_clamp_in_fit": (_int, [_vp, _int]),
     "kcc_clamp_in_fit_used": (_int, [_vp, C.POINTER(C.c_int)]),
     "kcc_fit_stream_rows": (_int, [_vp, C.POINTER(_i64)]),
+    "kcc_set_fit_split": (_int, [_vp, _int]),
+    "kcc_fit_split_stats": (_int, [_vp, C.POINTER(_i64), C.POINTER(_i64)]),
     "kcc_reduce_faults": (_int, [_vp, C.POINTER(_i64)]),
     "kcc_clear_faults": (_int, [_vp]),
     "kcc_comm_unique_id": (_int, [_vp]),
@@ -114,8 +116,11 @@
             "`make -C kubernetesclustercapacity_amd/csrc` (or __graft_entry__.build()). "
             "There is no CPU fallback.")
     lib = C.CDLL(path)
+    release = os.path.abspath(path) == os.path.abspath(LIB_PATH)
     for name, (res, args) in SIGNATURES.items():
-        fn = getattr(lib, name)
+        fn = getattr(lib, name) if release else getattr(lib, name, None)
+        if fn is None:
+            continue
         fn.restype = res
         fn.argtypes = args
     return lib
diff --git a/kubernetesclustercapacity_amd/csrc/kcc_abi.cpp b/kubernetesclustercapacity_amd/csrc/kcc_abi.cpp
--- a/kubernetesclustercapacity_amd/csrc/kcc_abi.cpp
+++ b/kubernetesclustercapacity_amd/csrc/kcc_abi.cpp
@@ -67,7 +67,7 @@
   DevBuf rank_arrive;
   DevBuf fit_q;
   bool fitq_dirty = true;
-  DevBuf c_rank, c_bcnt, c_cs, c_ms, c_mrc, c_crm, c_dperm;
+  DevBuf c_rank, c_bcnt, c_scnt, c_cs, c_ms, c_mrc, c_crm, c_dperm;
   DevBuf c_C, c_H2, c_H3, c_Crow, c_rec, c_dir;
   bool clamp_dirty = true;
   int64_t last_pairs = 0;
@@ -76,6 +76,8 @@
   int64_t d_stride = 0;
   bool fit_dense = false;
   int clamp_in_fit = -1;
+  int fit_split = -1;
+  int64_t big_off = 0;
   bool last_nc = false;
   DevBuf fast_cl;
   int stream_chunks = 0;
@@ -253,8 +255,8 @@
     int rc = reduce_ws(ctx, dv, dv.stream);
     if (rc) return rc;
   }
-  KCC_HIP(ctx, ensure(dv.fast_a, sizeof(kcc::FitGroupA) * (size_t)kcc::fit_groups((int64_t)N)));
-  KCC_HIP(ctx, ensure(dv.fast_b, sizeof(kcc::FitGroup) * (size_t)kcc::fit_groups((int64_t)N)));
+  KCC_HIP(ctx, ensure(dv.fast_a, 2 * sizeof(kcc::FitGroupA) * (size_t)kcc::fit_groups((int64_t)N)));
+  KCC_HIP(ctx, ensure(dv.fast_b, 2 * sizeof(kcc::FitGroup) * (size_t)kcc::fit_groups((int64_t)N)));
   KCC_HIP(ctx, ensure(dv.fast_cl, sizeof(int32_t) * kcc::FIT_GROUP * (size_t)kcc::fit_groups((int64_t)N)));
   KCC_HIP(ctx, ensure(dv.slow, sizeof(kcc::SlowNode) * N));
   KCC_HIP(ctx, ensure(dv.slow_list, sizeof(int64_t) * N));
@@ -277,6 +279,7 @@
   if (dv.fit_q.bytes != q_before) dv.fitq_dirty = true;
   const size_t S64 = (S + 63) / 64 * 64;
   KCC_HIP(ctx, ensure(dv.c_bcnt, 8 * (S64 / 64)));
+  KCC_HIP(ctx, ensure(dv.c_scnt, 4 * (S64 / 64)));
   KCC_HIP(ctx, ensure(dv.c_cs, 8 * S));
   KCC_HIP(ctx, ensure(dv.c_ms, 8 * S));
   KCC_HIP(ctx, ensure(dv.c_mrc, 4 * S64));
@@ -327,6 +330,7 @@
   kcc::ClampWork cw;
   cw.rank = as<uint32_t>(dv.c_rank);
   cw.bcnt = as<uint32_t>(dv.c_bcnt);
+  cw.scnt = as<uint32_t>(dv.c_scnt);
   cw.cs = as<uint64_t>(dv.c_cs);
   cw.ms = as<int64_t>(dv.c_ms);
   cw.mr_c = as<uint32_t>(dv.c_mrc);
@@ -348,7 +352,8 @@
 int check_spec_ws(kcc_ctx* ctx, Dev& dv, int64_t S) {
   const size_t S64 = (size_t)(S + 63) / 64 * 64;
   const bool ok = dv.c_rank.bytes >= 4 * (size_t)kcc::rank_words(S) &&
-                  dv.c_bcnt.bytes >= 8 * (S64 / 64) && dv.c_mrc.bytes >= 4 * S64 &&
+                  dv.c_bcnt.bytes >= 8 * (S64 / 64) && dv.c_scnt.bytes >= 4 * (S64 / 64) &&
+                  dv.c_mrc.bytes >= 4 * S64 &&
                   dv.rank_arrive.bytes >= 4 * (S64 / 64) &&
                   dv.c_crm.bytes >= 4 * S64 && dv.c_cs.bytes >= 8 * (size_t)S &&
                   dv.c_ms.bytes >= 8 * (size_t)S && dv.c_dperm.bytes >= 4 * (size_t)S &&
@@ -361,10 +366,16 @@
 }
 
 kcc::PlaceArgs place_args(Dev& dv, int64_t n_specs, const uint64_t* spec_cpu,
-                          const int64_t* spec_mem, int64_t* partial) {
+                          const int64_t* spec_mem, int64_t* partial, bool split = false) {
   return kcc::PlaceArgs{n_specs, spec_cpu, spec_mem, spec_prep_of(dv), clamp_of(dv), partial,
                         as<unsigned long long>(dv.counters), 0,
-                        as<const unsigned long long>(dv.faults), 0};
+                        as<const unsigned long long>(dv.faults), 0, split ? 1 : 0};
+}
+
+int64_t fit_split_off(const Dev& dv, int64_t n_nodes, int64_t n_specs) {
+  const bool on = dv.fit_split != 0 && !dv.fit_dense && n_nodes > 0 && n_specs >= 2 * kcc::FIT_SPLIT_COL &&
+                  n_specs <= kcc::CLAMP_LDS_SPECS && n_specs <= kcc::RANK_FULL_MAX;
+  return on ? kcc::fit_groups(n_nodes) : 0;
 }
 
 int fit_prepare_dev(kcc_ctx* ctx, Dev& dv, int64_t n_nodes, const uint64_t* alloc_cpu,
@@ -389,17 +400,19 @@
   rc = clamp_clean(ctx, dv, s);
   if (rc) return rc;
   dv.clamp_dirty = true;
+  dv.big_off = fit_split_off(dv, n_nodes, n_specs);
   KCC_HIP(ctx, kcc::launch_spec_rank(kcc::rank_args(n_specs, spec_cpu, spec_mem, clamp_of(dv),
                                                     as<unsigned long long>(dv.counters),
-                                                    as<uint32_t>(dv.rank_arrive)),
+                                                    as<uint32_t>(dv.rank_arrive), false,
+                                                    dv.big_off > 0),
                                      s));
-  const kcc::PlaceArgs pa = place_args(dv, n_specs, spec_cpu, spec_mem, partial);
+  const kcc::PlaceArgs pa = place_args(dv, n_specs, spec_cpu, spec_mem, partial, dv.big_off > 0);
   KCC_HIP(ctx, kcc::launch_node_prep(n_nodes, alloc_cpu, alloc_mem, alloc_pods, pod_count,
                                        used_cpu, used_mem, as<kcc::FitGroupA>(dv.fast_a),
                                        as<kcc::FitGroup>(dv.fast_b), as<kcc::SlowNode>(dv.slow),
                                        as<int64_t>(dv.slow_list), n_specs, clamp_of(dv),
                                        as<unsigned long long>(dv.counters), 0, 0,
-                                       n_nodes, s, dv.fit_dense, &pa));
+                                       n_nodes, s, dv.fit_dense, &pa, dv.big_off));
   if (n_nodes == 0) {
     dv.clamp_dirty = false;
     return KCC_OK;
@@ -421,7 +434,8 @@
                                as<kcc::SlowNode>(dv.slow),
                                as<int64_t>(dv.slow_list), n_specs, spec_prep_of(dv), partial,
                                as<unsigned long long>(dv.counters), as<uint32_t>(dv.fit_q), 0,
-                               n_nodes, s, as<const unsigned long long>(dv.faults)));
+                               n_nodes, s, as<const unsigned long long>(dv.faults), nullptr, nullptr,
+                               nullptr, dv.big_off));
   return KCC_OK;
 }
 
@@ -536,10 +550,12 @@
                    (dv.clamp_in_fit < 0 && kcc::clamp_in_fit_auto(n_nodes, n_specs)));
   int32_t* const fast_cl = nc ? as<int32_t>(dv.fast_cl) : nullptr;
   dv.last_nc = nc;
+  dv.big_off = nc ? 0 : fit_split_off(dv, n_nodes, n_specs);
+  const bool split = dv.big_off > 0;
   kcc::RankArgs ra = kcc::rank_args(n_specs, spec_cpu, spec_mem, clamp_of(dv),
                                     as<unsigned long long>(dv.counters),
-                                    as<uint32_t>(dv.rank_arrive), nc);
-  kcc::PlaceArgs pa = place_args(dv, n_specs, spec_cpu, spec_mem, partial);
+                                    as<uint32_t>(dv.rank_arrive), nc, split);
+  kcc::PlaceArgs pa = place_args(dv, n_specs, spec_cpu, spec_mem, partial, split);
   pa.no_ranks = nc ? 1 : 0;
   kcc::NpArgs np{};
   if (nc) {
@@ -607,7 +623,7 @@
                                        as<int64_t>(dv.slow_list) + lo[c], n_specs, clamp_of(dv),
                                        as<unsigned long long>(dv.counters),
                                        c, lo[c], n_nodes, s, dv.fit_dense,
-                                       place_here ? &pa : nullptr));
+                                       place_here ? &pa : nullptr, dv.big_off));
     if (n == 0) continue;
     ProfPair pp{};
     if (dv.prof_on) {
@@ -621,7 +637,7 @@
                                  partial, as<unsigned long long>(dv.counters),
                                  as<uint32_t>(dv.fit_q), c, n_nodes, s,
                                  as<const unsigned long long>(dv.faults), fast_cl,
-                                 dv.prof_on ? pp.a : nullptr, dv.prof_on ? pp.b : nullptr));
+                                 dv.prof_on ? pp.a : nullptr, dv.prof_on ? pp.b : nullptr, dv.big_off));
     if (dv.prof_on) {
       pp.kind = 1;
       dv.prof_pending.push_back(pp);
@@ -794,7 +810,8 @@
   int64_t streamed = 0;
   for (int sh = 0; sh < ns; ++sh) {
     slow_pairs += ctx->host_cnt[(size_t)sh * kcc::CNT_N + kcc::CNT_SLOW_PAIRS];
-    streamed += (int64_t)ctx->host_cnt[(size_t)sh * kcc::CNT_N + kcc::CNT_STREAM];
+    streamed += (int64_t)ctx->host_cnt[(size_t)sh * kcc::CNT_N + kcc::CNT_STREAM] +
+                (int64_t)ctx->host_cnt[(size_t)sh * kcc::CNT_N + kcc::CNT_BIG];
   }
   ctx->host_stream_rows = streamed;
   const double pairs = (double)n_nodes * (double)n_specs;
@@ -908,7 +925,7 @@
     }
     if (dv.clamp_arrive.p) (void)hipFree(dv.clamp_arrive.p);
     if (dv.np_sync.p) (void)hipFree(dv.np_sync.p);
-    DevBuf* bufs[] = {&dv.c_rank, &dv.c_bcnt, &dv.c_cs, &dv.c_ms,
+    DevBuf* bufs[] = {&dv.c_rank, &dv.c_bcnt, &dv.c_scnt, &dv.c_cs, &dv.c_ms,
                       &dv.c_mrc, &dv.c_crm, &dv.c_dperm, &dv.c_C, &dv.c_H2, &dv.c_H3,
                       &dv.c_Crow, &dv.c_rec, &dv.c_dir,
                       &dv.red_tail,  &dv.faults, &dv.rank_arrive, &dv.fast_cl, &dv.slow_list, &dv.fast_a, &dv.fast_b, &dv.slow, &dv.srec,
@@ -1221,8 +1238,29 @@
   if (dv.counters.p)
     KCC_HIP(ctx, hipMemcpy(c, dv.counters.p, sizeof(c), hipMemcpyDeviceToHost));
   int64_t t = 0;
-  for (int k = 0; k < dv.stream_chunks && k < kcc::FIT_MAX_CHUNKS; ++k) t += (int64_t)c[kcc::CNT_STREAM + k];
+  for (int k = 0; k < dv.stream_chunks && k < kcc::FIT_MAX_CHUNKS; ++k)
+    t += (int64_t)(c[kcc::CNT_STREAM + k] + c[kcc::CNT_BIG + k]);
   *streamed = t;
+  return KCC_OK;
+}
+
+int kcc_set_fit_split(kcc_ctx* ctx, int mode) {
+  if (!ctx) return KCC_EINVAL;
+  if (mode < -1 || mode > 0) return fail(ctx, KCC_EINVAL, "mode: -1 (on where it applies) or 0 (off)");
+  for (Dev& dv : ctx->devs) dv.fit_split = mode;
+  return KCC_OK;
+}
+
+int kcc_fit_split_stats(kcc_ctx* ctx, int64_t* big_rows, int64_t* small_specs) {
+  if (!ctx || !big_rows || !small_specs) return ctx ? fail(ctx, KCC_EINVAL, "NULL output") : KCC_EINVAL;
+  Dev& dv = ctx->devs[0];
+  KCC_HIP(ctx, hipSetDevice(dv.device));
+  KCC_HIP(ctx, hipDeviceSynchronize());
+  unsigned long long c[kcc::CNT_N] = {};
+  if (dv.counters.p)
+    KCC_HIP(ctx, hipMemcpy(c, dv.counters.p, sizeof(c), hipMemcpyDeviceToHost));
+  *big_rows = (int64_t)c[kcc::CNT_BIG_ROWS];
+  *small_specs = (int64_t)c[kcc::CNT_SMALL];
   return KCC_OK;
 }
 
diff --git a/kubernetesclustercapacity_amd/csrc/kcc_internal.h b/kubernetesclustercapacity_amd/csrc/kcc_internal.h
--- a/kubernetesclustercapacity_amd/csrc/kcc_internal.h
+++ b/kubernetesclustercapacity_amd/csrc/kcc_internal.h
@@ -98,6 +98,7 @@
 struct ClampWork {
   uint32_t* rank;
   uint32_t* bcnt;
+  uint32_t* scnt;
   uint64_t* cs;
   int64_t* ms;
   uint32_t* mr_c;
@@ -137,7 +138,13 @@
 constexpr int64_t RANK_L = 1024;
 constexpr int64_t RANK_FULL_MAX = 4096;
 __host__ __device__ inline int64_t rank_slices(int64_t S) { return (S + RANK_L - 1) / RANK_L; }
-__host__ __device__ inline int64_t rank_words(int64_t S) { return 2 * S + 2 * S * rank_slices(S); }
+__host__ __device__ inline int64_t rank_words(int64_t S) {
+  return 2 * S + 2 * S * rank_slices(S) + (S + 63) / 64 * rank_slices(S);
+}
+constexpr int64_t FIT_SPLIT_X_NUM = 1, FIT_SPLIT_Y_NUM = 1, FIT_SPLIT_DEN = 2;
+constexpr int64_t FIT_SPLIT_COL = 256;
+__host__ __device__ inline int64_t fit_split_x(int64_t nN) { return nN * FIT_SPLIT_X_NUM / FIT_SPLIT_DEN; }
+__host__ __device__ inline int64_t fit_split_y(int64_t nN) { return nN * FIT_SPLIT_Y_NUM / FIT_SPLIT_DEN; }
 struct RankArgs {
   int64_t S;
   const uint64_t* c_in;
@@ -145,6 +152,8 @@
   uint32_t* part;
   uint32_t* arrive;
   uint32_t* bcnt;
+  uint32_t* scnt;
+  int32_t split;
   uint64_t* cs;
   int64_t* ms;
   uint32_t* mr_c;
@@ -158,7 +167,7 @@
 };
 RankArgs rank_args(int64_t n_specs, const uint64_t* spec_cpu, const int64_t* spec_mem,
                    const ClampWork& cw, unsigned long long* counters, uint32_t* arrive,
-                   bool zero_only = false);
+                   bool zero_only = false, bool split = false);
 hipError_t launch_spec_rank(const RankArgs& ra, hipStream_t s);
 
 struct PlaceArgs {
@@ -172,6 +181,7 @@
   int32_t n_blocks;
   const unsigned long long* faults;
   int32_t no_ranks;
+  int32_t split;
 };
 
 
@@ -210,7 +220,11 @@
   CNT_CLAMP_ALL = 3,
   CNT_SLOW_ROWS = 4,
   CNT_STREAM = 4 + FIT_MAX_CHUNKS,
-  CNT_N = 4 + 2 * FIT_MAX_CHUNKS
+  CNT_BIG = 4 + 2 * FIT_MAX_CHUNKS,
+  CNT_BIG_P = 4 + 3 * FIT_MAX_CHUNKS,
+  CNT_BIG_ROWS = 5 + 3 * FIT_MAX_CHUNKS,
+  CNT_SMALL = 6 + 3 * FIT_MAX_CHUNKS,
+  CNT_N = 7 + 3 * FIT_MAX_CHUNKS
 };
 struct FinArgs {
   const int32_t* perm;
@@ -232,7 +246,7 @@
                             SlowNode* slow, int64_t* slow_list, int64_t n_specs, ClampWork cw,
                             unsigned long long* counters, int chunk, int64_t row0,
                             int64_t call_nodes, hipStream_t s, bool dense = false,
-                            const PlaceArgs* place = nullptr);
+                            const PlaceArgs* place = nullptr, int64_t big_off = 0);
 constexpr int64_t CLAMP_IN_FIT_PAIRS = 1100000000LL;
 inline bool clamp_in_fit_auto(int64_t n_nodes, int64_t n_specs) {
   return n_specs <= CLAMP_LDS_SPECS && n_nodes * n_specs <= CLAMP_IN_FIT_PAIRS;
@@ -244,9 +258,9 @@
                       unsigned long long* counters, uint32_t* queue, int chunk,
                       int64_t grid_nodes, hipStream_t s, const unsigned long long* faults,
                       const int32_t* fast_cl = nullptr, hipEvent_t ev_start = nullptr,
-                      hipEvent_t ev_stop = nullptr);
+                      hipEvent_t ev_stop = nullptr, int64_t big_off = 0);
 constexpr int64_t FIT_QSUBS_MAX = 32;
-inline int64_t fit_queue_words(int64_t S) { return (S + 255) / 256 * FIT_QSUBS_MAX * 16; }
+inline int64_t fit_queue_words(int64_t S) { return 2 * ((S + 255) / 256 * FIT_QSUBS_MAX * 16); }
 
 hipError_t launch_fit_finalize(int64_t n_specs, const int64_t* partial,
                                const int32_t* perm, int64_t* totals, int32_t* spec_err,
diff --git a/kubernetesclustercapacity_amd/csrc/kcc_kernels.hip b/kubernetesclustercapacity_amd/csrc/kcc_kernels.hip
--- a/kubernetesclustercapacity_amd/csrc/kcc_kernels.hip
+++ b/kubernetesclustercapacity_amd/csrc/kcc_kernels.hip
@@ -811,7 +811,8 @@
                                  SlowNode* __restrict__ slow, int64_t* __restrict__ slow_list,
                                  int64_t S, ClampWork cw,
                                  unsigned long long* __restrict__ counters,
-                                 int32_t chunk, int32_t dense, int64_t pass0, PlaceArgs pa) {
+                                 int32_t chunk, int32_t dense, int64_t pass0, PlaceArgs pa,
+                                 int64_t big_off) {
   if ((int32_t)blockIdx.x < pa.n_blocks) {
     spec_place_body(pa, blockIdx.x);
     return;
@@ -836,15 +837,27 @@
     }
   };
   load_row((int64_t)bid * PR + threadIdx.x);
+  const uint32_t scnt_ld = MODE == 2 && big_off > 0 && !dense && (int64_t)lane < (S + 63) / 64 ? cw.scnt[lane] : 0u;
   __shared__ uint32_t np_wc[KCC_NODE_PREP_BLOCK / 64];
   __shared__ uint64_t np_base;
   __shared__ uint32_t np_tot;
   __shared__ uint32_t np_bcnt[NP_BINS];
   __shared__ uint32_t np_bstart[NP_BINS];
+  __shared__ uint32_t np_wcb[KCC_NODE_PREP_BLOCK / 64];
+  __shared__ uint64_t np_bbase;
+  __shared__ uint32_t np_btot;
+  __shared__ unsigned long long np_bigp[2];
   const NpClasses cls = np_classes<false>(cw.bcnt, S, lane);
   const bool want_b = cls.want_b, slow_all = cls.slow_all;
   const int64_t nN = cls.nN;
   const int64_t T = (nN + 63) / 64, W = T + 2;
+  bool split = false;
+  if (MODE == 2 && big_off > 0 && !dense) {
+    const uint32_t ns = (uint32_t)__builtin_amdgcn_readlane((int)wave_incl_scan_u32(scnt_ld), 63);
+    split = ns >= (uint32_t)FIT_SPLIT_COL;
+  }
+  const uint32_t split_x = (uint32_t)fit_split_x(nN), split_y = (uint32_t)fit_split_y(nN);
+  if (threadIdx.x < 2) np_bigp[threadIdx.x] = 0ull;
   const bool binned = MODE == 2 || clamp_binned(S);
   const int NB = (int)(2 * T);
   int64_t* Cc = cw.C + (int64_t)(bid % C_COPIES) * cw.c_stride;
@@ -935,10 +948,12 @@
     uint32_t r_fc[SUB];
     int32_t r_P[SUB];
     unsigned long long sbal[SUB];
+    unsigned long long bbal[SUB];
     uint32_t pk1[SUB], pk2[SUB], pk3[SUB];
     uint64_t always_sum = 0;
-    uint64_t base_ret = 0;
-    uint32_t t_pass = 0;
+    uint32_t big_p = 0;
+    uint64_t base_ret = 0, bbase_ret = 0;
+    uint32_t t_pass = 0, t_big = 0;
 #pragma unroll
     for (int q = 0; q < SUB; ++q) {
       const int64_t i = i0 + q * KCC_NODE_PREP_BLOCK + threadIdx.x;
@@ -949,7 +964,7 @@
       np_slow_append(valid && !ok, i, lane, &counters[CNT_SLOW_ROWS + chunk], slow_list);
       load_row(q + 1 < SUB ? i + KCC_NODE_PREP_BLOCK : i0 + stride + threadIdx.x);
       sbal[q] = __ballot(dense ? valid : (r_fc[q] > 0 && r_fm[q] > 0 && r_P[q] > 0));
-      if (q == SUB - 1) {
+      if (q == SUB - 1 && !split) {
         if (lane == 0) np_wc[wv] = np_wave_streamed(sbal);
         __syncthreads();
         if (threadIdx.x == 0) {
@@ -964,7 +979,7 @@
       const double rP = recip_up_f64(P > 0 ? (uint64_t)P : 1ull);
       const int64_t V0 = (int64_t)((double)r_fm[q] * rP);
       const uint32_t U0 = (uint32_t)((double)r_fc[q] * rP);
-      const bool act = ok && nN > 0 && P > 0 && wfull != 0 && U0 >= cmin && V0 >= mmin;
+      const bool act = ok && nN > 0 && P > 0 && (wfull != 0 || split) && U0 >= cmin && V0 >= mmin;
       const int64_t w = act ? wfull : 0;
       const uint32_t U = act ? U0 : 0u;
       const int64_t V = act ? V0 : 0;
@@ -996,6 +1011,33 @@
         L = w ? upper_bound_count(cw.cs, nN, (uint64_t)U) : 0u;
         b = w ? upper_bound_count(cw.ms, nN, V) : 0u;
       }
+      {
+        const bool big = split && act && L >= split_x && b >= split_y;
+        bbal[q] = __ballot(big);
+        sbal[q] &= ~bbal[q];
+        big_p += big ? (uint32_t)P : 0u;
+      }
+      if (q == SUB - 1 && split) {
+        const uint32_t nb = np_wave_streamed(bbal);
+        const uint32_t vp = (uint32_t)__builtin_amdgcn_readlane((int)wave_incl_scan_u32(big_p), 63);
+        if (lane == 0) {
+          np_wc[wv] = np_wave_streamed(sbal);
+          np_wcb[wv] = nb;
+          if (nb) {
+            lds_add_u64(&np_bigp[0], (uint64_t)vp);
+            lds_add_u64(&np_bigp[1], (uint64_t)nb);
+          }
+        }
+        __syncthreads();
+        if (threadIdx.x == 0) {
+          t_pass = np_wc_sum(np_wc, KCC_NODE_PREP_BLOCK / 64);
+          base_ret = np_stream_claim(t_pass, &counters[CNT_STREAM + chunk]);
+        }
+        if (threadIdx.x == 64) {
+          t_big = np_wc_sum(np_wcb, KCC_NODE_PREP_BLOCK / 64);
+          bbase_ret = np_stream_claim(t_big, &counters[CNT_BIG + chunk]);
+        }
+      }
       const uint32_t GX = L >> 6, rx = L & 63u, GY = b >> 6, ry = b & 63u;
       uint32_t k, j;
       if (lds) {
@@ -1032,6 +1074,10 @@
     if (threadIdx.x == 0) {
       np_base = base_ret;
       np_tot = t_pass;
+    }
+    if (split && threadIdx.x == 64) {
+      np_bbase = bbase_ret;
+      np_btot = t_big;
     }
     __syncthreads();
     KCC_TL(bid % 1024, 4);
@@ -1079,9 +1125,30 @@
       }
       if (threadIdx.x < np_padded(tot) - tot)
         np_put<false>(np_base + tot + threadIdx.x, 0ull, 0u, 0u, 0, fast_a, fast_b, want_b, nullptr);
+      if (split) {
+        const uint64_t bb0 = np_bbase + np_wc_sum(np_wcb, wv);
+        const uint32_t btot = np_btot;
+        uint32_t bdone = 0;
+#pragma unroll
+        for (int q = 0; q < SUB; ++q) {
+          if ((bbal[q] >> lane) & 1ull)
+            np_put<false>(bb0 + bdone + (uint32_t)__popcll(bbal[q] & ((1ull << lane) - 1ull)), r_fm[q], r_fc[q],
+                          (uint32_t)r_P[q], 0, fast_a + big_off, fast_b + big_off, want_b, nullptr);
+          bdone += (uint32_t)__popcll(bbal[q]);
+        }
+        if (threadIdx.x < np_padded(btot) - btot)
+          np_put<false>(np_bbase + btot + threadIdx.x, 0ull, 0u, 0u, 0, fast_a + big_off, fast_b + big_off,
+                        want_b, nullptr);
+      }
     }
     __syncthreads();
     KCC_TL(bid % 1024, 5);
+  }
+  if (split) {
+    if (threadIdx.x == 0 && np_bigp[1]) {
+      atomicAdd(&counters[CNT_BIG_P], np_bigp[0]);
+      atomicAdd(&counters[CNT_BIG_ROWS], np_bigp[1]);
+    }
   }
   if (cpriv) {
     for (int64_t e = threadIdx.x; e < W * W; e += KCC_NODE_PREP_BLOCK) {
@@ -1125,6 +1192,7 @@
     }
   }
   const int64_t j0 = sl * RANK_L, j1 = j0 + RANK_L < S ? j0 + RANK_L : S;
+  uint32_t n_norm = 0;
   for (int64_t j = j0 + tid; j < j1; j += 256) {
     const uint64_t cj = c_in[j];
     const int64_t mj = m_in[j];
@@ -1133,7 +1201,9 @@
     k.x = nj ? cj << 13 | (uint64_t)(j & 8191) : ~0ull;
     k.y = nj ? (uint64_t)mj << 13 | (uint64_t)(j & 8191) : ~0ull;
     key_l[j - j0] = k;
-  }
+    n_norm += (uint32_t)__popcll(__ballot(nj));
+  }
+  if (lane == 0) rank_small(lds)[4 + wv] = n_norm;
   __syncthreads();
   const int64_t chq = i >> 13, chs = j0 >> 13;
   const uint64_t tc = chs < chq ? (c + 1) << 13 : (chs == chq ? c << 13 | (uint64_t)(i & 8191) : c << 13);
@@ -1153,10 +1223,16 @@
   part[(wv * 2 + 1) * 64 + lane] = rm;
   __syncthreads();
   uint32_t* const slices = ra.part + 2 * S;
+  uint32_t* const norm = slices + 2 * S * ns;
   if (wv < 2) {
     const uint32_t t = part[(0 * 2 + wv) * 64 + lane] + part[(1 * 2 + wv) * 64 + lane] +
                        part[(2 * 2 + wv) * 64 + lane] + part[(3 * 2 + wv) * 64 + lane];
     if (qv) __hip_atomic_store(slices + (sl * 2 + wv) * S + i, t, __ATOMIC_RELAXED, __HIP_MEMORY_SCOPE_AGENT);
+    if (wv == 0 && lane == 0) {
+      const uint32_t* nw = rank_small(lds) + 4;
+      __hip_atomic_store(norm + qb * ns + sl, nw[0] + nw[1] + nw[2] + nw[3], __ATOMIC_RELAXED,
+                         __HIP_MEMORY_SCOPE_AGENT);
+    }
     asm volatile("s_waitcnt vmcnt(0)" ::: "memory");
   }
   __syncthreads();
@@ -1169,12 +1245,23 @@
   if (!last_s || wv != 0) return;
   asm volatile("" ::: "memory");
   if (ns > 1 && lane == 0) ra.arrive[qb] = 0;
-  if (!qv || ci == SPEC_EXACT) return;
+  const bool nq = qv && ci != SPEC_EXACT;
   uint32_t x = 0, y = 0;
+  int64_t nN = 0;
   for (int64_t k = 0; k < ns; ++k) {
-    x += __hip_atomic_load(slices + (k * 2 + 0) * S + i, __ATOMIC_RELAXED, __HIP_MEMORY_SCOPE_AGENT);
-    y += __hip_atomic_load(slices + (k * 2 + 1) * S + i, __ATOMIC_RELAXED, __HIP_MEMORY_SCOPE_AGENT);
-  }
+    if (nq) {
+      x += __hip_atomic_load(slices + (k * 2 + 0) * S + i, __ATOMIC_RELAXED, __HIP_MEMORY_SCOPE_AGENT);
+      y += __hip_atomic_load(slices + (k * 2 + 1) * S + i, __ATOMIC_RELAXED, __HIP_MEMORY_SCOPE_AGENT);
+    }
+    nN += __hip_atomic_load(norm + qb * ns + k, __ATOMIC_RELAXED, __HIP_MEMORY_SCOPE_AGENT);
+  }
+  {
+    const bool small = ra.split && nq && ci == SPEC_A && (int64_t)x < fit_split_x(nN) &&
+                       (int64_t)y < fit_split_y(nN);
+    const uint32_t n_small = (uint32_t)__popcll(__ballot(small));
+    if (lane == 0) ra.scnt[qb] = n_small;
+  }
+  if (!nq) return;
   ra.cs[x] = c;
   ra.ms[y] = m;
   ra.mr_c[x] = y;
@@ -1372,7 +1459,7 @@
   const int tid = threadIdx.x;
   if (ra.zero_only) {
     const bool wt = ra.done_flag != nullptr;
-    if (tid < CNT_N && tid != CNT_SPECS_A && tid != CNT_SPECS_B) {
+    if (tid < CNT_N && tid != CNT_SPECS_A && tid != CNT_SPECS_B && tid != CNT_SMALL) {
       if (wt) __hip_atomic_store(ra.counters + tid, 0ull, __ATOMIC_RELAXED, __HIP_MEMORY_SCOPE_AGENT);
       else ra.counters[tid] = 0;
     }
@@ -1411,7 +1498,7 @@
   }
   {
     const int64_t gt = blk * 256 + tid, nt = (int64_t)ra.n_blocks * 256;
-    if (gt < CNT_N && gt != CNT_SPECS_A && gt != CNT_SPECS_B) ra.counters[gt] = 0;
+    if (gt < CNT_N && gt != CNT_SPECS_A && gt != CNT_SPECS_B && gt != CNT_SMALL) ra.counters[gt] = 0;
     for (int64_t e = gt; e < C_COPIES * ra.c_cells; e += nt)
       ra.C[(e / ra.c_cells) * ra.c_stride + e % ra.c_cells] = 0;
   }
@@ -1442,18 +1529,30 @@
   const int32_t cls = in ? spec_class(c, m) : SPEC_EXACT;
   const bool normal = cls != SPEC_EXACT;
   const uint32_t x = in && normal && !pa.no_ranks ? cw.rank[i] : 0u;
+  const bool split = pa.split && !pa.no_ranks;
+  const uint32_t y = split && in && cls == SPEC_A ? cw.rank[S + i] : 0u;
   uint64_t tot = 0, pre = 0;
   const unsigned long long* bc = reinterpret_cast<const unsigned long long*>(cw.bcnt);
+  uint64_t stp = 0;
   for (int64_t b = lane; b < nqb; b += 64) {
     const uint64_t v = __hip_atomic_load(bc + b, __ATOMIC_RELAXED, __HIP_MEMORY_SCOPE_AGENT);
     tot += v;
     pre += b < qb ? v : 0ull;
+    if (split) {
+      const uint64_t sv = cw.scnt[b];
+      stp += sv | (b < qb ? sv << 32 : 0ull);
+    }
   }
   tot = readlane_u64(wave_incl_scan_u64(tot), 63);
   pre = readlane_u64(wave_incl_scan_u64(pre), 63);
+  stp = readlane_u64(wave_incl_scan_u64(stp), 63);
   const uint32_t nA = (uint32_t)tot, nB = (uint32_t)(tot >> 32);
   const uint32_t pA = (uint32_t)pre, pB = (uint32_t)(pre >> 32);
   const int64_t nN = (int64_t)nA + nB;
+  const uint32_t nS = (uint32_t)stp / (uint32_t)FIT_SPLIT_COL * (uint32_t)FIT_SPLIT_COL;
+  const bool small = split && in && cls == SPEC_A && (int64_t)x < fit_split_x(nN) &&
+                     (int64_t)y < fit_split_y(nN);
+  const unsigned long long mS = __ballot(small);
   const unsigned long long mA = __ballot(cls == SPEC_A && in), mB = __ballot(cls == SPEC_B && in);
   const unsigned long long below = (1ull << lane) - 1ull;
   const uint32_t rA = (uint32_t)__popcll(mA & below), rB = (uint32_t)__popcll(mB & below);
@@ -1464,9 +1563,12 @@
   if (i == 0) {
     counters[CNT_SPECS_A] = nA;
     counters[CNT_SPECS_B] = nB;
+    counters[CNT_SMALL] = nS;
   }
   if (!in) return;
-  const int64_t pos = cls == SPEC_A ? (int64_t)pA + rA
+  const uint32_t sb = (uint32_t)(stp >> 32) + (uint32_t)__popcll(mS & below);
+  const int64_t pos = cls == SPEC_A ? (small && sb < nS ? (int64_t)sb
+                                                        : (int64_t)nS + pA + rA - (sb < nS ? sb : nS))
                     : cls == SPEC_B ? (int64_t)nA + pB + rB
                                     : nN + (qb * 64 - pA - pB) + (lane - rA - rB);
   SpecRec rec;
@@ -1598,7 +1700,8 @@
 
 __device__ __forceinline__ void clamp_apply_bin(const ClampWork& cw, int64_t S,
                                                 int64_t* __restrict__ partial, int64_t nN,
-                                                int64_t u, uint32_t G, uint32_t h) {
+                                                int64_t u, uint32_t G, uint32_t h,
+                                                uint32_t small_n, uint64_t big_p) {
   __shared__ uint64_t tab[H_CELLS];
   __shared__ uint64_t ctot[CP_WAVES][64];
   __shared__ uint64_t colsum[128];
@@ -1715,6 +1818,7 @@
 #pragma unroll
     for (int r = 0; r < 8; ++r) d += part[r];
   }
+  if (x_side && h == 0 && (uint32_t)p < small_n) d -= big_p;
   if (d && p < clamp_n_pure(nN, S)) atomic_add_u64(reinterpret_cast<uint64_t*>(&partial[p]), 0ull - d);
   KCC_TL(1024 + blockIdx.x % 1024, 4);
 }
@@ -1763,7 +1867,9 @@
   const int64_t Tm = (S + 63) / 64;
   const uint32_t G = gridDim.x / (uint32_t)(2 * Tm), h = blockIdx.x / (uint32_t)(2 * Tm);
   const int64_t u = blockIdx.x % (uint32_t)(2 * Tm);
-  if (u < 2 * T) clamp_apply_bin(cw, S, partial, nN, u, G, h);
+  const uint32_t small_n = (uint32_t)counters[CNT_SMALL];
+  const uint64_t big_p = small_n ? (uint64_t)counters[CNT_BIG_P] : 0ull;
+  if (u < 2 * T) clamp_apply_bin(cw, S, partial, nN, u, G, h, small_n, big_p);
   if (fin.totals) fused_finalize(fin, S, partial, fin.arrive, gridDim.x, 0, S);
 }
 
@@ -1813,6 +1919,8 @@
 constexpr uint32_t FIT_Q_HALVE = 128;
 constexpr uint32_t FIT_WG_PER_SUB = 24;
 constexpr uint32_t FIT_QSUBS = (uint32_t)FIT_QSUBS_MAX;
+static_assert(FIT_SPLIT_COL == FIT_SPW, "the small specs fill whole fit columns");
+constexpr uint32_t FIT_SPLIT_SHARE = 4;
 
 __device__ __forceinline__ double f64_at(const i32x16& v, int k) {
   return __longlong_as_double(((int64_t)(uint32_t)v[2 * k + 1] << 32) | (uint32_t)v[2 * k]);
@@ -1825,10 +1933,31 @@
     const FitGroup* __restrict__ fast_b, const SlowNode* __restrict__ slow,
     const int64_t* __restrict__ slow_list, int64_t S, const SpecRec* __restrict__ specs,
     int64_t* __restrict__ partial, unsigned long long* __restrict__ counters, int32_t chunk,
-    int32_t gx, int32_t gy, const int32_t* __restrict__ fast_cl,
-    const unsigned long long* __restrict__ faults, const int32_t b, uint32_t* q_slot) {
+    int32_t gx, int32_t gy_all, const int32_t* __restrict__ fast_cl,
+    const unsigned long long* __restrict__ faults, const int32_t b, uint32_t* q_slot,
+    const uint32_t big_off) {
   const int32_t xcd = b & 7, r = b >> 3;
-  const int32_t bx = r % gx, by = (r / gx) * 8 + xcd;
+  int32_t bx = r % gx, by = (r / gx) * 8 + xcd;
+  int32_t gy = gy_all;
+  const uint32_t ncs = CL ? 0u : (uint32_t)counters[CNT_SMALL] / (uint32_t)FIT_SPW;
+  if (!CL && FIT_SPLIT_SHARE > 1 && ncs > 0 && ncs < (uint32_t)gx && gy_all % 8 == 0) {
+    const uint32_t nco = (uint32_t)gx - ncs, tot = (uint32_t)gx * ((uint32_t)gy_all / 8u);
+    uint32_t a = tot / (ncs + FIT_SPLIT_SHARE * nco);
+    a = a ? a : 1u;
+    const uint32_t o = (tot - ncs * a) / nco;
+    uint32_t j;
+    if ((uint32_t)r < ncs * a) {
+      bx = (int32_t)((uint32_t)r % ncs);
+      j = (uint32_t)r / ncs;
+      gy = (int32_t)(a * 8u);
+    } else {
+      const uint32_t r2 = (uint32_t)r - ncs * a;
+      bx = (int32_t)(ncs + r2 % nco);
+      j = r2 / nco;
+      gy = (int32_t)(o * 8u);
+    }
+    by = (int32_t)(j * 8u) + xcd;
+  }
   if (by >= gy) return;
   __builtin_amdgcn_s_setprio(3);
   KCC_TL(2048 + b % 4096, 0);
@@ -1856,7 +1985,9 @@
   const bool wave_fast = !wave_exact && !idle;
   KCC_TL(2048 + b % 4096, 5);
 
-  const uint32_t n_groups = (uint32_t)(counters[CNT_STREAM + chunk] / FIT_GROUP);
+  const uint32_t n_res = (uint32_t)(counters[CNT_STREAM + chunk] / FIT_GROUP);
+  const uint32_t n_big = CL || (uint32_t)bx < ncs ? 0u : (uint32_t)(counters[CNT_BIG + chunk] / FIT_GROUP);
+  uint32_t n_groups = n_res;
   uint32_t lim = n_groups;
   uint32_t base = 0;
   uint32_t nxt = 0;
@@ -1864,13 +1995,9 @@
   nsub = nsub <= 8u ? 8u : (nsub >= FIT_QSUBS ? FIT_QSUBS : 1u << (31 - __builtin_clz(nsub)));
   if ((uint32_t)gy < nsub) nsub = (uint32_t)gy;
   const uint32_t sub = (uint32_t)by % nsub;
-  uint32_t* const qp = queue + ((uint32_t)bx * FIT_QSUBS + sub) * 16u;
-  const uint32_t qsz = n_groups / (uint32_t)gy < FIT_Q_HALVE ? FIT_QCHUNK / 2u : FIT_QCHUNK;
+  uint32_t* qp = queue + ((uint32_t)bx * FIT_QSUBS + sub) * 16u;
+  uint32_t qsz = FIT_QCHUNK;
   uint32_t q1 = qsz;
-  {
-    const uint32_t sh = n_groups / (uint32_t)gy / FIT_Q1_DIV;
-    q1 = sh < q1 ? (sh > FIT_QMIN ? sh : FIT_QMIN) : q1;
-  }
 
   auto claim_issue = [&](uint32_t sz) {
     if (wv == 0 && lane == 0)
@@ -1879,7 +2006,7 @@
   };
   const uint32_t wps = ((uint32_t)gy + nsub - 1u) / nsub;
   const uint32_t wseg = ((uint32_t)gy - sub + nsub - 1u) / nsub;
-  const uint32_t dyn0 = wseg * q1;
+  uint32_t dyn0 = 0;
   uint32_t qcur = q1;
   auto claim_publish = [&](uint32_t slot) {
     if (wv == 0) {
@@ -1888,15 +2015,30 @@
     }
     __syncthreads();
   };
-  {
+  uint32_t first = 0;
+  auto region = [&](uint32_t reg) {
+    n_groups = reg ? n_big : n_res;
+    qp = queue + (((uint32_t)gx * reg + (uint32_t)bx) * FIT_QSUBS + sub) * 16u;
+    qsz = n_groups / (uint32_t)gy < FIT_Q_HALVE ? FIT_QCHUNK / 2u : FIT_QCHUNK;
+    q1 = qsz;
+    const uint32_t sh = n_groups / (uint32_t)gy / FIT_Q1_DIV;
+    q1 = sh < q1 ? (sh > FIT_QMIN ? sh : FIT_QMIN) : q1;
+    dyn0 = wseg * q1;
+    qcur = q1;
     const uint32_t seg = ((n_groups + nsub - 1u) / nsub + 7u) / 8u * 8u;
     base = sub * seg < n_groups ? sub * seg : n_groups;
     lim = base + seg < n_groups ? base + seg : n_groups;
-    KCC_TL(2048 + b % 4096, 1);
-  }
-  const uint32_t first = ((uint32_t)by / nsub) * q1;
+    first = ((uint32_t)by / nsub) * q1;
+  };
   uint32_t pr_done = 0;
-  const uint32_t pr_share = (lim - base) / wseg > 0 ? (lim - base) / wseg : 1u;
+  uint32_t pr_share = 0;
+  if (n_big) {
+    region(1u);
+    pr_share = lim - base;
+  }
+  region(0u);
+  KCC_TL(2048 + b % 4096, 1);
+  pr_share = (pr_share + lim - base) / wseg > 0 ? (pr_share + lim - base) / wseg : 1u;
 #ifdef KCC_TIMELINE
   uint32_t tl_done = 0;
 #endif
@@ -2061,8 +2203,15 @@
   };
 
   {
-    for (uint32_t k = 0;; ++k) {
-      const uint32_t cur = base + (k == 0 ? first : __builtin_amdgcn_readfirstlane(q_slot[k & 1u]));
+    uint32_t k = 0;
+#pragma nounroll
+    for (uint32_t reg = 0; reg < (n_big ? 2u : 1u); ++reg) {
+    if (reg) region(reg);
+    const uint32_t roff = reg ? big_off : 0u;
+    bool fst = true;
+    for (;; ++k) {
+      const uint32_t cur = base + (fst ? first : __builtin_amdgcn_readfirstlane(q_slot[k & 1u]));
+      fst = false;
       if (cur >= lim) break;
       const uint32_t rem = lim - cur;
       uint32_t qn = rem / (FIT_QDIV * wps);
@@ -2076,8 +2225,8 @@
           if (!wave_b) sum_a_nc(cur, cnt);
           else sum_b_nc(cur, cnt);
         } else {
-          if (!wave_b) sum_a(cur, cnt);
-          else sum_b(cur, cnt);
+          if (!wave_b) sum_a(roff + cur, cnt);
+          else sum_b(roff + cur, cnt);
         }
       }
       claim_publish((k + 1u) & 1u);
@@ -2101,6 +2250,7 @@
         qp[0] = 0;
         qp[1] = 0;
       }
+    }
     }
   }
   KCC_TL(2048 + b % 4096, 2);
@@ -2140,10 +2290,10 @@
     const int64_t* __restrict__ slow_list, int64_t S, const SpecRec* __restrict__ specs,
     int64_t* __restrict__ partial, unsigned long long* __restrict__ counters, int32_t chunk,
     int32_t gx, int32_t gy, const int32_t* __restrict__ fast_cl,
-    const unsigned long long* __restrict__ faults) {
+    const unsigned long long* __restrict__ faults, uint32_t big_off) {
   __shared__ uint32_t q_slot[2];
   fit_body<CL>(n_nodes, queue, fast_a, fast_b, slow, slow_list, S, specs, partial, counters, chunk,
-               gx, gy, fast_cl, faults, (int32_t)blockIdx.x, q_slot);
+               gx, gy, fast_cl, faults, (int32_t)blockIdx.x, q_slot, big_off);
 }
 
 __global__ void fit_finalize_kernel(int64_t S, const int64_t* __restrict__ partial,
@@ -2358,7 +2508,7 @@
                             SlowNode* slow, int64_t* slow_list, int64_t n_specs,
                             ClampWork cw, unsigned long long* counters, int chunk, int64_t row0,
                             int64_t call_nodes, hipStream_t s, bool dense,
-                            const PlaceArgs* place) {
+                            const PlaceArgs* place, int64_t big_off) {
   if (n_nodes <= 0 && !place) return hipSuccess;
   const int64_t pr = clamp_pass_rows(call_nodes);
   if (row0 % pr != 0 || (pr != 1024 && pr != 4096)) return hipErrorInvalidValue;
@@ -2380,13 +2530,14 @@
   hipLaunchKernelGGL(kern, dim3(np_blocks + (unsigned)pa.n_blocks), dim3(KCC_NODE_PREP_BLOCK),
                      lds_bytes, s, n_nodes, alloc_cpu, alloc_mem, alloc_pods, pod_count, used_cpu,
                      used_mem, fast_a, fast_b, slow, slow_list, n_specs, cw,
-                     counters, (int32_t)chunk, (int32_t)(dense ? 1 : 0), row0 / pr, pa);
+                     counters, (int32_t)chunk, (int32_t)(dense ? 1 : 0), row0 / pr, pa,
+                     mode == 2 && !dense ? big_off : (int64_t)0);
   return hipGetLastError();
 }
 
 RankArgs rank_args(int64_t n_specs, const uint64_t* spec_cpu, const int64_t* spec_mem,
                    const ClampWork& cw, unsigned long long* counters, uint32_t* arrive,
-                   bool zero_only) {
+                   bool zero_only, bool split) {
   RankArgs ra{};
   ra.S = n_specs;
   ra.c_in = spec_cpu;
@@ -2394,6 +2545,8 @@
   ra.part = cw.rank;
   ra.arrive = arrive;
   ra.bcnt = cw.bcnt;
+  ra.scnt = cw.scnt;
+  ra.split = split && !zero_only && n_specs <= RANK_FULL_MAX ? 1 : 0;
   ra.cs = cw.cs;
   ra.ms = cw.ms;
   ra.mr_c = cw.mr_c;
@@ -2467,8 +2620,10 @@
                       const int64_t* slow_list, int64_t n_specs, SpecPrep sp, int64_t* partial,
                       unsigned long long* counters, uint32_t* queue, int chunk,
                       int64_t grid_nodes, hipStream_t s, const unsigned long long* faults,
-                      const int32_t* fast_cl, hipEvent_t ev_start, hipEvent_t ev_stop) {
+                      const int32_t* fast_cl, hipEvent_t ev_start, hipEvent_t ev_stop,
+                      int64_t big_off) {
   if (n_nodes <= 0 || n_specs <= 0) return hipSuccess;
+  if (big_off < 0 || big_off > 0x7fffffffLL) return hipErrorInvalidValue;
   const int64_t gx = (n_specs + FIT_SPW - 1) / FIT_SPW;
   const int64_t gy = fit_grid_y(n_nodes, n_specs, grid_nodes);
   const int64_t blocks = gx * ((gy + 7) / 8 * 8);
@@ -2477,11 +2632,11 @@
   if (ev_start || ev_stop)
     hipExtLaunchKernelGGL(kern, dim3((unsigned)blocks), dim3(256), 0, s, ev_start, ev_stop, 0, n_nodes,
                           queue, fast_a, fast_b, slow, slow_list, n_specs, sp.rec, partial, counters,
-                          (int32_t)chunk, (int32_t)gx, (int32_t)gy, fast_cl, faults);
+                          (int32_t)chunk, (int32_t)gx, (int32_t)gy, fast_cl, faults, (uint32_t)big_off);
   else
     hipLaunchKernelGGL(kern, dim3((unsigned)blocks), dim3(256), 0, s, n_nodes, queue, fast_a,
                        fast_b, slow, slow_list, n_specs, sp.rec, partial, counters, (int32_t)chunk,
-                       (int32_t)gx, (int32_t)gy, fast_cl, faults);
+                       (int32_t)gx, (int32_t)gy, fast_cl, faults, (uint32_t)big_off);
   return hipGetLastError();
 }
 
diff --git a/kubernetesclustercapacity_amd/engine.py b/kubernetesclustercapacity_amd/engine.py
--- a/kubernetesclustercapacity_amd/engine.py
+++ b/kubernetesclustercapacity_amd/engine.py
@@ -484,6 +484,14 @@
         self._check(self._lib.kcc_fit_stream_rows(self._h, C.byref(v)))
         return v.value
 
+    def set_fit_split(self, mode: int):
+        self._check(self._lib.kcc_set_fit_split(self._h, int(mode)))
+
+    def fit_split_stats(self):
+        b, s = C.c_int64(), C.c_int64()
+        self._check(self._lib.kcc_fit_split_stats(self._h, C.byref(b), C.byref(s)))
+        return b.value, s.value
+
     def reduce_faults(self) -> int:
         v = C.c_int64()
         self._check(self._lib.kcc_reduce_faults(self._h, C.byref(v)))
```

Measured after the change: 14610 billion evals/s, median of 6. +2.3%, better.
